# Gancheekim/ATM-VFI

Measured on AMD Instinct MI355X. Metric: interpolated frames/s at 1080p (network_base, bs=1), higher is better.
Workload: dtype f32 (contractions as fp16 hi/lo split x3 MFMA, fp32 accumulate; ~22 significand bits)

## Files before the change

atm-vfi_amd/csrc/api.hip:

```cpp
#include "common.h"

#include <string.h>

#include <vector>

namespace atmvfi {

static thread_local char g_err[512] = "";

void set_error(const char* fmt, ...) {
    va_list ap;
    va_start(ap, fmt);
    vsnprintf(g_err, sizeof(g_err), fmt, ap);
    va_end(ap);
}

int check_launch(const char* what) {
    const hipError_t e = hipGetLastError();
    if (e != hipSuccess) {
        set_error("%s: launch failed: %s", what, hipGetErrorString(e));
        return ATMVFI_ELAUNCH;
    }
    return ATMVFI_OK;
}

#ifdef ATMVFI_RANGE_CHECK
static std::vector<RangeWordSetter>& range_registry() {
    static std::vector<RangeWordSetter> v;
    return v;
}
void range_registry_add(RangeWordSetter s) { range_registry().push_back(s); }
#endif

}

extern "C" int atmvfi_range_word_set(uint32_t* word, void* stream) {
#ifdef ATMVFI_RANGE_CHECK
    for (atmvfi::RangeWordSetter set : atmvfi::range_registry()) {
        const int e = set(reinterpret_cast<unsigned*>(word), (hipStream_t)stream);
        ATMVFI_REQUIRE(e == 0, ATMVFI_ELAUNCH, "range_word_set: hipMemcpyToSymbolAsync failed (%d)", e);
    }
    return ATMVFI_OK;
#else
    (void)word; (void)stream;
    atmvfi::set_error("range_word_set: this is the default build; the operand range check lives in libatmvfi_hip_checked.so (make checked)");
    return ATMVFI_EINVAL;
#endif
}
extern "C" int atmvfi_range_checked(void) {
#ifdef ATMVFI_RANGE_CHECK
    return 1;
#else
    return 0;
#endif
}

extern "C" int atmvfi_version(void) { return (0 << 16) | (26 << 8) | 0; }
extern "C" const char* atmvfi_last_error(void) { return atmvfi::g_err; }
#ifndef ATMVFI_SOURCE_DIGEST
#define ATMVFI_SOURCE_DIGEST "unknown (api.hip compiled outside the Makefile)"
#endif
extern "C" const char* atmvfi_source_digest(void) { return ATMVFI_SOURCE_DIGEST; }
```

atm-vfi_amd/csrc/conv3x3_f16x3.hip:

```cpp
#include "common.h"

#include "conv3_common.h"

#include <stdlib.h>

namespace {

__global__ void pack_split_kernel(int mode, const float* __restrict__ src, _Float16* __restrict__ hi, _Float16* __restrict__ lo,
                                  int Cout, int Cin, int kh, int kw, int rows, int cin_pad, int coutp) {
    fp16_saturate_on();
    const int taps = (mode == ATMVFI_GEMM_DECONV) ? 1 : kh * kw;
    const int cpt = cin_pad >> 5;
    const long long total = (long long)rows * taps * cin_pad;
    for (long long idx = (long long)blockIdx.x * blockDim.x + threadIdx.x; idx < total;
         idx += (long long)gridDim.x * blockDim.x) {
        const int e = (int)(idx & 31);
        const int row = (int)((idx >> 5) % rows);
        const int kstep = (int)((idx >> 5) / rows);
        const int tap = kstep / cpt;
        const int c = (kstep - tap * cpt) * 32 + e;
        float v = 0.f;
        if (c < Cin) {
            if (mode == ATMVFI_GEMM_DECONV) {
                const int q = row / coutp;
                const int co = row - q * coutp;
                if (q < 4 && co < Cout) v = src[(((long long)c * Cout + co) * 2 + (q >> 1)) * 2 + (q & 1)];
            } else if (row < Cout) {
                const int ky = tap / kw, kx = tap - ky * kw;
                v = src[(((long long)row * Cin + c) * kh + ky) * kw + kx];
            }
        }
        const _Float16 h = sat_half(v);
        hi[idx] = h;
        lo[idx] = sat_half((v - (float)h) * LO_SCALE);
    }
}

__global__ void pack_conv3x3_kernel(const float* __restrict__ src, _Float16* __restrict__ hi, _Float16* __restrict__ lo, int Cout, int Cin,
                                    int rows, int cf, int tail) {
    fp16_saturate_on();
    const int nsteps = 9 * (cf >> 5) + (tail ? 3 : 0);
    const long long total = (long long)nsteps * rows * 32;
    for (long long idx = (long long)blockIdx.x * blockDim.x + threadIdx.x; idx < total; idx += (long long)gridDim.x * blockDim.x) {
        const int e = (int)(idx & 31);
        const int row = (int)((idx >> 5) % rows);
        const int step = (int)((idx >> 5) / rows);
        int tap, c;
        if (step < 9 * (cf >> 5)) {
            tap = step % 9;
            c = (step / 9) * 32 + e;
        } else {
            const int t = step - 9 * (cf >> 5);
            tap = 4 * t + (e >> 3);
            c = (e & 7) < tail ? cf + (e & 7) : Cin;
        }
        float v = 0.f;
        if (row < Cout && tap < 9 && c < Cin) v = src[((long long)row * Cin + c) * 9 + tap];
        const _Float16 h = sat_half(v);
        hi[idx] = h;
        lo[idx] = sat_half((v - (float)h) * LO_SCALE);
    }
}

}

static void conv3_layout(int Cin, int& cf, int& tail) {
    const int t = Cin % 32;
    if (t >= 1 && t <= 8) { cf = Cin - t; tail = t; }
    else { cf = atmvfi::round_up(Cin, 32); tail = 0; }
}
static int split_rows(int mode, int Cout) {
    return (mode == ATMVFI_GEMM_DECONV) ? atmvfi::round_up(4 * atmvfi::round_up(Cout, 4), 16) : atmvfi::round_up(Cout, 16);
}

extern "C" int64_t atmvfi_split_weight_halves(int mode, int Cout, int Cin, int kh, int kw) {
    const int taps = (mode == ATMVFI_GEMM_DECONV) ? 1 : kh * kw;
    return (int64_t)split_rows(mode, Cout) * taps * atmvfi::round_up(Cin, 32);
}

extern "C" int atmvfi_pack_weight_split(int mode, const float* src, void* dst_hi, void* dst_lo, int Cout, int Cin, int kh,
                                         int kw, void* stream) {
    ATMVFI_REQUIRE(src && dst_hi && dst_lo && Cout > 0 && Cin > 0 && kh > 0 && kw > 0 && mode >= 0 && mode <= 2, ATMVFI_EINVAL,
                   "pack_weight_split: bad arguments");
    if (mode == ATMVFI_GEMM_DECONV) ATMVFI_REQUIRE(kh == 2 && kw == 2, ATMVFI_EINVAL, "pack_weight_split: deconv must be 2x2");
    const int64_t total = atmvfi_split_weight_halves(mode, Cout, Cin, kh, kw);
    const int blocks = (int)((total + 255) / 256 > 4096 ? 4096 : (total + 255) / 256);
    hipLaunchKernelGGL(pack_split_kernel, dim3(blocks), dim3(256), 0, (hipStream_t)stream, mode, src, (_Float16*)dst_hi,
                       (_Float16*)dst_lo, Cout, Cin, kh, kw, split_rows(mode, Cout), atmvfi::round_up(Cin, 32),
                       atmvfi::round_up(Cout, 4));
    return atmvfi::check_launch("pack_weight_split");
}

extern "C" int atmvfi_conv3x3_f16x3(const float* in, int in_ld, int N, int H, int W, int Cin, const void* w_hi,
                                     const void* w_lo, int Cout, float* out, int out_ld, const float* bias,
                                     const float* prelu, void* out_hi, void* out_lo, int64_t plane_rows,
                                     const float* plane_prelu, int schedule, int wn, void* stream) {
    ATMVFI_REQUIRE(in && w_hi && w_lo && out, ATMVFI_EINVAL, "conv3x3_f16x3: null pointer");
    ATMVFI_REQUIRE(schedule >= -1 && schedule <= 1 && wn >= 0 && wn <= 8, ATMVFI_EINVAL,
                   "conv3x3_f16x3: schedule -1 (auto), 0 (row) or 1 (half), wn 0 (auto) or 1..8; got %d, %d", schedule, wn);
    ATMVFI_REQUIRE(N > 0 && H > 0 && W > 0 && Cin > 0 && Cout > 0, ATMVFI_EINVAL, "conv3x3_f16x3: bad shape");
    ATMVFI_REQUIRE(in_ld % 4 == 0 && in_ld >= atmvfi::round_up(Cin, 4) && out_ld % 4 == 0 && out_ld >= atmvfi::round_up(Cout, 4),
                   ATMVFI_EALIGN, "conv3x3_f16x3: leading dimensions must be multiples of 4 and cover the channels");
    ATMVFI_REQUIRE(atmvfi::aligned16(in) && atmvfi::aligned16(out) && atmvfi::aligned16(w_hi) && atmvfi::aligned16(w_lo) &&
                       (!bias || atmvfi::aligned16(bias)) && (!prelu || atmvfi::aligned16(prelu)),
                   ATMVFI_EALIGN, "conv3x3_f16x3: pointers (incl. bias/prelu) must be 16-byte aligned");
    ATMVFI_REQUIRE((out_hi == nullptr) == (out_lo == nullptr), ATMVFI_EINVAL, "conv3x3_f16x3: plane sink needs both planes");
    if (out_hi) {
        ATMVFI_REQUIRE(plane_rows >= (int64_t)N * H * W, ATMVFI_EINVAL, "conv3x3_f16x3: plane_rows %lld < N*H*W", (long long)plane_rows);
        ATMVFI_REQUIRE(atmvfi::aligned16(out_hi) && atmvfi::aligned16(out_lo) && (!plane_prelu || atmvfi::aligned16(plane_prelu)),
                       ATMVFI_EALIGN, "conv3x3_f16x3: plane sink pointers must be 16-byte aligned");
    }
    Conv3Dev d;
    d.in = in; d.in_ld = in_ld; d.N = N; d.H = H; d.W = W; d.Cin = Cin;
    d.w_hi = (const _Float16*)w_hi; d.w_lo = (const _Float16*)w_lo;
    d.wrows = atmvfi::round_up(Cout, 16);
    conv3_layout(Cin, d.cf, d.tail);
    d.cs = 0;
    d.ktot = 0;
    d.Cout = Cout; d.out = out; d.out_ld = out_ld; d.bias = bias; d.prelu = prelu;
    d.out_hi = (_Float16*)out_hi; d.out_lo = (_Float16*)out_lo; d.plane_rows = plane_rows; d.plane_prelu = plane_prelu;
    d.stamp = nullptr;
    d.nblocks = 0;
    d.tchunk = 0;
    d.legacy_order = 0;
    d.force_schedule = schedule;
// ... 24 lines not shown
```

atm-vfi_amd/csrc/gemm_common.h:

```cpp
#pragma once
#include "common.h"

namespace atmvfi {

struct GemmDev {
    int mode;
    const float* in;
    int in_ld, H, W, Cin;
    long long in_gstride;
    int in_rpg;
    const float* weight;
    int wrows;
    int ktot;
    int cin_pad;
    int cpt;
    int nchunks;
    int Cout;
    int coutp;
    int kw, stride, pad, dil;
    int Ho, Wo;
    long long M;
    float* out;
    int out_ld;
    long long out_gstride;
// ... 3 lines not shown
    const float* prelu;
    const float* in_prelu;
    const float* residual;
    int res_ld;
    const _Float16* w_hi;
    const _Float16* w_lo;
    int cin_pad32;
    int cpt32;
    int nchunks32;
    int ktot32;
    const _Float16* a_hi;
    const _Float16* a_lo;
    const _Float16* a_hi2;
    const _Float16* a_lo2;
    int in_ld2, split_chunks;
    int in_N;
    unsigned long long* stamp;
    int dbg;
    int mchunk;
    int vblocks;
    int nblocks;
    _Float16* out_hi;
    _Float16* out_lo;
    long long out_plane_rows;
    int out_c0, out_gc;
    int force_wn;
    int ksplit;
    float* part;
    long long part_stride;
    int part_ld;
    int fit32;
    int pfit32;
    int terms;
};


__device__ __forceinline__ bool gemm_out_row(const GemmDev& a, long long m, float*& orow, const float*& rrow, long long& prow, int& pc0) {
    pc0 = a.out_c0;
    if (a.mode == ATMVFI_GEMM_DECONV) {
        const int hw = a.H * a.W;
        const int n = (m >> 31) ? (int)(m / hw) : (int)((unsigned)m / (unsigned)hw);
        const int rem = (int)(m - (long long)n * hw);
        const int y = rem / a.W;
        const int x = rem - y * a.W;
        prow = ((long long)n * a.Ho + 2 * y) * a.Wo + 2 * x;
        orow = a.out + prow * a.out_ld;
    } else {
        long long ro = m;
        if (a.out_row_map) ro = a.out_row_map[m];
        if (ro < 0) return false;
        prow = ro;
        long long off = ro * (long long)a.out_ld;
        if (a.out_rpg > 0) {
            const long long grp = ro / a.out_rpg;
            prow = ro - grp * a.out_rpg;
            off = grp * a.out_gstride + prow * (long long)a.out_ld;
            pc0 += (int)grp * a.out_gc;
        }
        orow = a.out + off;
    }
    rrow = a.residual ? a.residual + m * (long long)a.res_ld : nullptr;
    return true;
}
__device__ __forceinline__ void gemm_out_row_at(const GemmDev& a, long long m, long long ro, float*& orow, long long& prow, int& pc0) {
    pc0 = a.out_c0;
    if (a.mode == ATMVFI_GEMM_DECONV) {
        const int hw = a.H * a.W;
// ... 44 lines not shown
    if (c.nvalid >= 4) {
        if (a.bias) c.b = *reinterpret_cast<const f32x4*>(a.bias + c.co);
        if (a.prelu) c.p = *reinterpret_cast<const f32x4*>(a.prelu + c.co);
    } else if (c.nvalid > 0) {
        float bb[4] = {0.f, 0.f, 0.f, 0.f}, pp[4] = {1.f, 1.f, 1.f, 1.f};
        for (int e = 0; e < c.nvalid; ++e) {
            if (a.bias) bb[e] = a.bias[c.co + e];
            if (a.prelu) pp[e] = a.prelu[c.co + e];
        }
        c.b = (f32x4){bb[0], bb[1], bb[2], bb[3]};
        c.p = (f32x4){pp[0], pp[1], pp[2], pp[3]};
    }
    return c;
}

__device__ __forceinline__ void gemm_store4(const GemmDev& a, float* orow, const float* rrow, const ChanVec& c, f32x4 v) {
    if (c.co < 0) return;
    float* optr = orow;
    if (a.mode == ATMVFI_GEMM_DECONV) optr = orow + ((long long)(c.q >> 1) * a.Wo + (c.q & 1)) * a.out_ld;
    v += c.b;
    v.x = v.x > 0.f ? v.x : c.p.x * v.x;
    v.y = v.y > 0.f ? v.y : c.p.y * v.y;
    v.z = v.z > 0.f ? v.z : c.p.z * v.z;
    v.w = v.w > 0.f ? v.w : c.p.w * v.w;
    if (c.nvalid >= 4) {
        if (rrow) v += *reinterpret_cast<const f32x4*>(rrow + c.co);
        *reinterpret_cast<f32x4*>(optr + c.co) = v;
    } else {
        const float vv[4] = {v.x, v.y, v.z, v.w};
        for (int e = 0; e < c.nvalid; ++e) optr[c.co + e] = vv[e] + (rrow ? rrow[c.co + e] : 0.f);
    }
}

template <int BN>
__device__ __forceinline__ void gemm_dma_consts(const GemmDev& a, int n0, float* cst, int wave, int lane) {
    dma_epilogue_consts<BN>(a.bias, a.prelu, n0, cst, wave, lane, [&](int col) {
        int co = col;
        if (a.mode == ATMVFI_GEMM_DECONV) {
            const int q = col / a.coutp;
            co = q < 4 ? col - q * a.coutp : a.Cout;
        }
        return co < a.Cout ? co : -1;
    });
}
constexpr int gemm_const_floats(int BN) { return epilogue_const_floats(BN); }

struct ChanPos {
    int co;
    int q;
    int nvalid;
};
__device__ __forceinline__ ChanPos gemm_chan_pos(const GemmDev& a, int nb) {
    ChanPos c;
    c.q = 0;
    c.co = nb;
    if (a.mode == ATMVFI_GEMM_DECONV) {
        c.q = (nb >= a.coutp) + (nb >= 2 * a.coutp) + (nb >= 3 * a.coutp);
        c.co = nb - c.q * a.coutp;
        if (nb >= 4 * a.coutp) c.co = a.Cout;
    }
    c.nvalid = a.Cout - c.co;
    return c;
}
__device__ __forceinline__ void gemm_finish_store4(const GemmDev& a, float* orow, long long prow, int pc0, const ChanPos& c, f32x4 v,
                                                   const f32x4 b, const f32x4 p, const f32x4 res) {
    v += b;
    v.x = v.x > 0.f ? v.x : p.x * v.x;
    v.y = v.y > 0.f ? v.y : p.y * v.y;
    v.z = v.z > 0.f ? v.z : p.z * v.z;
    v.w = v.w > 0.f ? v.w : p.w * v.w;
    v += res;
// ... 1 lines not shown
        float* optr = orow;
        if (a.mode == ATMVFI_GEMM_DECONV) optr = orow + ((long long)(c.q >> 1) * a.Wo + (c.q & 1)) * a.out_ld;
        if (c.nvalid >= 4) {
            *reinterpret_cast<f32x4*>(optr + c.co) = v;
        } else if (c.nvalid > 0) {
            optr[c.co] = v.x;
            if (c.nvalid > 1) optr[c.co + 1] = v.y;
            if (c.nvalid > 2) optr[c.co + 2] = v.z;
        }
    }
    if (a.out_hi && c.nvalid > 0) {
        if (c.nvalid < 4) {
            v.y = c.nvalid > 1 ? v.y : 0.f;
            v.z = c.nvalid > 2 ? v.z : 0.f;
            v.w = 0.f;
        }
        if (a.mode == ATMVFI_GEMM_DECONV) prow += (long long)(c.q >> 1) * a.Wo + (c.q & 1);
        const RowSink sink{nullptr, 0, a.out_hi, a.out_lo, a.out_plane_rows};
        sink_store4(sink, prow, pc0 + c.co, v);
    }
}
__device__ __forceinline__ f32x4 gemm_load_residual4(const float* rrow, const ChanPos& c) {
    f32x4 r = (f32x4){0.f, 0.f, 0.f, 0.f};
    if (c.nvalid >= 4) {
        r = *reinterpret_cast<const f32x4*>(rrow + c.co);
    } else if (c.nvalid > 0) {
        r.x = rrow[c.co];
        if (c.nvalid > 1) r.y = rrow[c.co + 1];
        if (c.nvalid > 2) r.z = rrow[c.co + 2];
    }
    return r;
}

int launch_gemm_f16x3(const GemmDev& d, int ngemm, hipStream_t stream);
bool try_launch_conv3x3_small(const GemmDev& d, int kh, int* rc, hipStream_t stream);
int launch_gemm_split(const GemmDev& d, int ngemm, hipStream_t stream);
int launch_gemm_pp(const GemmDev& d, int ngemm, hipStream_t stream);
int launch_gemm_duo(const GemmDev& d, int ngemm, hipStream_t stream);

}
```

atm-vfi_amd/csrc/gemm_conv.hip:

```cpp
#include "common.h"
#include "gemm_common.h"

#include <algorithm>

namespace {

using atmvfi::GemmDev;

__device__ __forceinline__ int swz(int row) { return (0x1320 >> (((row >> 2) & 3) << 2)) & 3; }

template <int WM, int WN>
__global__ __launch_bounds__(256) void gemm_mfma_f32(const GemmDev a) {
    fp16_saturate_on();
    constexpr int BM = 64 * WM;
    constexpr int BN = 16 * WN;
    constexpr int NB = (BN * 4 + 255) / 256;
    __shared__ __attribute__((aligned(16))) float lds[2 * (BM + BN) * 16];
    float* As = lds;
    float* Bs = lds + 2 * BM * 16;

    const int t = threadIdx.x;
    const int lane = t & 63;
    const int wave = t >> 6;
    const int kq = t & 3;
// ... 169 lines not shown

int packed_rows(int mode, int Cout) {
    if (mode == ATMVFI_GEMM_DECONV) return atmvfi::round_up(4 * atmvfi::round_up(Cout, 4), 16);
    return atmvfi::round_up(Cout, 16);
}

template <int WM, int WN>
void launch(const GemmDev& d, int ntiles, hipStream_t s) {
    dim3 grid((unsigned)atmvfi::ceil_div64(d.M, 64 * WM), (unsigned)((ntiles + WN - 1) / WN));
    hipLaunchKernelGGL((gemm_mfma_f32<WM, WN>), grid, dim3(256), 0, s, d);
}

}

extern "C" int64_t atmvfi_packed_weight_floats(int mode, int Cout, int Cin, int kh, int kw) {
    const int taps = (mode == ATMVFI_GEMM_DECONV) ? 1 : kh * kw;
    return (int64_t)packed_rows(mode, Cout) * taps * atmvfi::round_up(Cin, 16);
}

extern "C" int atmvfi_pack_weight(int mode, const float* src, float* dst, int Cout, int Cin, int kh, int kw, void* stream) {
    ATMVFI_REQUIRE(src && dst, ATMVFI_EINVAL, "pack_weight: null pointer");
    ATMVFI_REQUIRE(mode >= 0 && mode <= 2 && Cout > 0 && Cin > 0, ATMVFI_EINVAL, "pack_weight: bad mode/shape");
    if (mode == ATMVFI_GEMM_DECONV) ATMVFI_REQUIRE(kh == 2 && kw == 2, ATMVFI_EINVAL, "pack_weight: deconv must be 2x2");
    if (mode == ATMVFI_GEMM_LINEAR) ATMVFI_REQUIRE(kh == 1 && kw == 1, ATMVFI_EINVAL, "pack_weight: linear must be 1x1");
    const int rows = packed_rows(mode, Cout);
    const int cin_pad = atmvfi::round_up(Cin, 16);
    const int64_t total = atmvfi_packed_weight_floats(mode, Cout, Cin, kh, kw);
    const int blocks = (int)std::min<int64_t>((total + 255) / 256, 4096);
    hipLaunchKernelGGL(pack_weight_kernel, dim3(blocks), dim3(256), 0, (hipStream_t)stream, mode, src, dst, Cout, Cin,
                       kh, kw, rows, cin_pad, atmvfi::round_up(Cout, 4));
    return atmvfi::check_launch("pack_weight");
}

extern "C" int atmvfi_gemm(const atmvfi_gemm_params* p, void* stream) {
    ATMVFI_REQUIRE(p, ATMVFI_EINVAL, "gemm: null params");
    const bool planes = p->in_hi || p->in_lo;
    const bool sink = p->out_hi || p->out_lo;
    ATMVFI_REQUIRE((p->in || planes) && p->weight && (p->out || sink), ATMVFI_EINVAL, "gemm: null tensor pointer");
    if (sink) {
        ATMVFI_REQUIRE(p->out_hi && p->out_lo && (p->precision == ATMVFI_PREC_F16X3 || p->precision == ATMVFI_PREC_F16), ATMVFI_EINVAL,
                       "gemm: the plane sink needs both planes and precision f16x3 (or f16)");
        ATMVFI_REQUIRE(atmvfi::aligned16(p->out_hi) && atmvfi::aligned16(p->out_lo) && p->out_plane_c0 >= 0 && p->out_plane_c0 % 4 == 0 &&
                           p->out_plane_gc % 4 == 0, ATMVFI_EALIGN, "gemm: plane sink: 16-byte aligned planes, channel offsets multiples of 4");
        const long long orows = p->mode == ATMVFI_GEMM_DECONV ? (long long)p->N * p->Ho * p->Wo
                                : p->out_rpg > 0 ? (long long)p->out_rpg : (p->mode == ATMVFI_GEMM_CONV ? (long long)p->N * p->Ho * p->Wo : (long long)p->M);
        ATMVFI_REQUIRE(p->out_row_map || p->out_plane_rows >= orows, ATMVFI_EINVAL, "gemm: plane sink rows %lld < output rows %lld",
                       (long long)p->out_plane_rows, orows);
        ATMVFI_REQUIRE(p->out_plane_rows > 0, ATMVFI_EINVAL, "gemm: plane sink needs out_plane_rows");
    }
    if (planes) {
        ATMVFI_REQUIRE(p->in_hi && p->in_lo && (p->precision == ATMVFI_PREC_F16X3 || p->precision == ATMVFI_PREC_F16) && !p->in_prelu,
                       ATMVFI_EINVAL, "gemm: split-plane input needs both planes, precision f16x3 (or f16) and no in_prelu");
        ATMVFI_REQUIRE(atmvfi::aligned16(p->in_hi) && atmvfi::aligned16(p->in_lo) && p->in_rpg == 0, ATMVFI_EALIGN,
                       "gemm: split planes need 16-byte aligned pointers and plain rows");
        const long long mrows = p->mode == ATMVFI_GEMM_LINEAR ? (long long)p->M : (long long)p->N * p->H * p->W;
        ATMVFI_REQUIRE(p->in_ld >= mrows + (p->mode == ATMVFI_GEMM_CONV ? 1 : 0), ATMVFI_EALIGN,
                       "gemm: with split planes in_ld is the plane row count and must cover the rows (+ the zero row in CONV mode): %lld > %d",
                       mrows, p->in_ld);
        if (p->in_hi2 || p->in_lo2) {
            ATMVFI_REQUIRE(p->mode == ATMVFI_GEMM_CONV && p->in_hi2 && p->in_lo2 && atmvfi::aligned16(p->in_hi2) && atmvfi::aligned16(p->in_lo2) &&
                               p->in_ld2 >= mrows + 1 && p->in_split_chunks > 0 && p->in_split_chunks * 32 < p->Cin, ATMVFI_EINVAL,
                           "gemm: a second plane source needs CONV mode, both planes, in_ld2 > N*H*W and 0 < 32 * in_split_chunks < Cin");
        }
    }
    ATMVFI_REQUIRE(p->precision >= ATMVFI_PREC_F32 && p->precision <= ATMVFI_PREC_F16, ATMVFI_EINVAL, "gemm: bad precision %d", p->precision);
    ATMVFI_REQUIRE(p->precision != ATMVFI_PREC_F16 || planes, ATMVFI_EINVAL,
                   "gemm: precision f16 needs split-plane input (in_hi / in_lo): the fp32-input engines have no single-pass instance");
    ATMVFI_REQUIRE(p->precision != ATMVFI_PREC_F16 || p->tile_wn != -1, ATMVFI_EINVAL,
                   "gemm: precision f16 has no instance of the reference schedule (tile_wn = -1): use 0 (auto), -2, -3 or -4");
    ATMVFI_REQUIRE(p->mode >= 0 && p->mode <= 2, ATMVFI_EINVAL, "gemm: bad mode %d", p->mode);
    ATMVFI_REQUIRE(p->Cin > 0 && p->Cout > 0, ATMVFI_EINVAL, "gemm: bad channel counts");
    ATMVFI_REQUIRE(planes || (p->in_ld >= atmvfi::round_up(p->Cin, 4) && p->in_ld % 4 == 0), ATMVFI_EALIGN,
                   "gemm: in_ld %d must be a multiple of 4 and >= Cin rounded to 4 (Cin %d)", p->in_ld, p->Cin);
    ATMVFI_REQUIRE(!p->out || (p->out_ld % 4 == 0 && p->out_ld >= atmvfi::round_up(p->Cout, 4)), ATMVFI_EALIGN,
                   "gemm: out_ld %d must be a multiple of 4 and >= Cout rounded to 4 (Cout %d)", p->out_ld, p->Cout);
    ATMVFI_REQUIRE((planes || atmvfi::aligned16(p->in)) && (!p->out || atmvfi::aligned16(p->out)) && atmvfi::aligned16(p->weight), ATMVFI_EALIGN,
                   "gemm: in/out/weight must be 16-byte aligned");
    ATMVFI_REQUIRE((planes || p->in_gstride % 4 == 0) && p->out_gstride % 4 == 0, ATMVFI_EALIGN, "gemm: group strides must be multiples of 4");
    if (p->residual)
        ATMVFI_REQUIRE(p->res_ld >= p->Cout, ATMVFI_EINVAL, "gemm: res_ld %d < Cout %d", p->res_ld, p->Cout);
    if (p->in_prelu) ATMVFI_REQUIRE(atmvfi::aligned16(p->in_prelu), ATMVFI_EALIGN, "gemm: in_prelu must be 16-byte aligned");
    ATMVFI_REQUIRE((!p->bias || atmvfi::aligned16(p->bias)) && (!p->prelu || atmvfi::aligned16(p->prelu)) &&
                       (!p->residual || (atmvfi::aligned16(p->residual) && p->res_ld % 4 == 0)),
                   ATMVFI_EALIGN, "gemm: bias/prelu/residual must be 16-byte aligned (res_ld a multiple of 4)");

    GemmDev d;
    d.mode = p->mode;
    d.in = p->in; d.in_ld = p->in_ld; d.H = p->H; d.W = p->W; d.Cin = p->Cin;
    d.in_gstride = p->in_gstride; d.in_rpg = p->in_rpg;
    d.weight = p->weight;
    d.cin_pad = atmvfi::round_up(p->Cin, 16);
    d.cpt = d.cin_pad / 16;
    d.Cout = p->Cout; d.coutp = atmvfi::round_up(p->Cout, 4);
    d.kw = 1; d.stride = 1; d.pad = 0; d.dil = 1; d.Ho = p->Ho; d.Wo = p->Wo;
    int taps = 1;
    int ngemm = p->Cout;
    if (p->mode == ATMVFI_GEMM_CONV) {
        ATMVFI_REQUIRE(p->N > 0 && p->H > 0 && p->W > 0, ATMVFI_EINVAL, "conv2d: bad input size");
        ATMVFI_REQUIRE((p->kh == 1 || p->kh == 3) && p->kh == p->kw, ATMVFI_EINVAL, "conv2d: kernel %dx%d unsupported", p->kh, p->kw);
        ATMVFI_REQUIRE(p->stride >= 1 && p->dil >= 1 && p->pad >= 0, ATMVFI_EINVAL, "conv2d: bad stride/dilation/pad");
        const int ho = (p->H + 2 * p->pad - p->dil * (p->kh - 1) - 1) / p->stride + 1;
        const int wo = (p->W + 2 * p->pad - p->dil * (p->kw - 1) - 1) / p->stride + 1;
        ATMVFI_REQUIRE(ho == p->Ho && wo == p->Wo, ATMVFI_EINVAL, "conv2d: Ho/Wo (%d,%d) do not match geometry (%d,%d)", p->Ho, p->Wo, ho, wo);
// ... 19 lines not shown
    d.out = p->out; d.out_ld = p->out_ld; d.out_gstride = p->out_gstride; d.out_rpg = p->out_rpg;
    d.out_row_map = p->out_row_map;
    d.bias = p->bias; d.prelu = p->prelu; d.in_prelu = p->in_prelu; d.residual = p->residual; d.res_ld = p->res_ld;
    ATMVFI_REQUIRE(d.M < (1ll << 40), ATMVFI_EINVAL, "gemm: M too large");
    d.a_hi = (const _Float16*)p->in_hi;
    d.a_lo = (const _Float16*)p->in_lo;
    d.a_hi2 = (const _Float16*)p->in_hi2;
    d.a_lo2 = (const _Float16*)p->in_lo2;
    d.in_ld2 = p->in_ld2;
    d.split_chunks = p->in_hi2 ? p->in_split_chunks : (1 << 30);
    d.in_N = p->N;
    d.out_hi = (_Float16*)p->out_hi;
    d.out_lo = (_Float16*)p->out_lo;
    d.out_plane_rows = p->out_plane_rows;
    d.out_c0 = p->out_plane_c0;
    d.out_gc = p->out_plane_gc;
    ATMVFI_REQUIRE(p->tile_wn >= -4 && p->tile_wn <= 8 && (p->tile_wn >= 0 || planes), ATMVFI_EINVAL,
                   "gemm: tile_wn 0 (auto), 1..8, or (split-plane input) -1 reference schedule / -2 gemm_duo (128-column tiles) / -3 gemm_pp / -4 gemm_duo (64-column tiles), got %d", p->tile_wn);
    d.force_wn = p->tile_wn;
    ATMVFI_REQUIRE(!p->workspace || (atmvfi::aligned16(p->workspace) && p->workspace_floats > 0), ATMVFI_EALIGN,
                   "gemm: the split-K workspace must be 16-byte aligned and non-empty");
    d.ksplit = 0;
    d.part = p->workspace;
    d.part_stride = p->workspace ? p->workspace_floats : 0;
    d.part_ld = 0;
    d.fit32 = 0;
    d.pfit32 = 0;
    d.nblocks = 0;
    d.dbg = 0;
    d.vblocks = 0;
    d.mchunk = 0;
    d.stamp = nullptr;
    d.terms = p->precision == ATMVFI_PREC_F16 ? 1 : 3;
    d.w_hi = (const _Float16*)p->weight_hi;
    d.w_lo = (const _Float16*)p->weight_lo;
    d.cin_pad32 = atmvfi::round_up(p->Cin, 32);
    d.cpt32 = d.cin_pad32 / 32;
    d.nchunks32 = taps * d.cpt32;
    d.ktot32 = taps * d.cin_pad32;
    if (p->precision == ATMVFI_PREC_F16X3 || p->precision == ATMVFI_PREC_F16) {
        ATMVFI_REQUIRE(p->weight_hi && p->weight_lo, ATMVFI_EINVAL, "gemm: precision f16x3 / f16 needs weight_hi/weight_lo");
        ATMVFI_REQUIRE(atmvfi::aligned16(p->weight_hi) && atmvfi::aligned16(p->weight_lo), ATMVFI_EALIGN,
                       "gemm: split weights must be 16-byte aligned");
        if (planes) return atmvfi::launch_gemm_split(d, ngemm, (hipStream_t)stream);
        return atmvfi::launch_gemm_f16x3(d, ngemm, (hipStream_t)stream);
    }

    {
        int rc = 0;
        if (atmvfi::try_launch_conv3x3_small(d, p->kh, &rc, (hipStream_t)stream)) return rc;
    }
    const int ntiles = (ngemm + 15) / 16;
    int best = 1;
    float best_cost = 1e30f;
    for (int wn = 1; wn <= 8; ++wn) {
        const int padded = (ntiles + wn - 1) / wn * wn;
        const float cost = (float)padded * (1.0f + 1.0f / (float)wn);
        if (cost <= best_cost) { best_cost = cost; best = wn; }
    }
    hipStream_t s = (hipStream_t)stream;
    switch (best) {
        case 1: launch<2, 1>(d, ntiles, s); break;
        case 2: launch<2, 2>(d, ntiles, s); break;
        case 3: launch<2, 3>(d, ntiles, s); break;
        case 4: launch<2, 4>(d, ntiles, s); break;
        case 5: launch<2, 5>(d, ntiles, s); break;
        case 6: launch<2, 6>(d, ntiles, s); break;
        case 7: launch<2, 7>(d, ntiles, s); break;
        default: launch<2, 8>(d, ntiles, s); break;
    }
    return atmvfi::check_launch("gemm");
}

extern "C" int atmvfi_conv2d(const atmvfi_gemm_params* p, void* stream) {
    ATMVFI_REQUIRE(p && p->mode == ATMVFI_GEMM_CONV, ATMVFI_EINVAL, "conv2d: params->mode must be ATMVFI_GEMM_CONV");
    return atmvfi_gemm(p, stream);
}
extern "C" int atmvfi_linear(const atmvfi_gemm_params* p, void* stream) {
    ATMVFI_REQUIRE(p && p->mode == ATMVFI_GEMM_LINEAR, ATMVFI_EINVAL, "linear: params->mode must be ATMVFI_GEMM_LINEAR");
    return atmvfi_gemm(p, stream);
}
extern "C" int atmvfi_deconv2x2(const atmvfi_gemm_params* p, void* stream) {
    ATMVFI_REQUIRE(p && p->mode == ATMVFI_GEMM_DECONV, ATMVFI_EINVAL, "deconv2x2: params->mode must be ATMVFI_GEMM_DECONV");
    return atmvfi_gemm(p, stream);
}
```

atm-vfi_amd/csrc/gemm_duo.hip:

```cpp
#include "gemm_plane.h"

namespace {

using atmvfi::GemmDev;

constexpr int BM = 128;
constexpr int stage_bytes(int BN) { return (2 * BM + 2 * BN) * 64; }
constexpr int A_LO = BM * 64, W_HI = 2 * BM * 64;
constexpr int cst_floats(int BN) { return atmvfi::gemm_const_floats(BN) + BM; }

#ifdef ATMVFI_STAMP
static unsigned long long* g_duo_stamp = nullptr;
extern "C" void atmvfi_debug_set_duo_stamp_buffer(void* p) { g_duo_stamp = (unsigned long long*)p; }
#define DUO_SUB(k) do { if (a.stamp) { __builtin_amdgcn_sched_barrier(0); const unsigned long long t_ = __builtin_amdgcn_s_memtime(); sub[k] += t_ - sub_t; sub_t = t_; __builtin_amdgcn_sched_barrier(0); } } while (0)
#else
#define DUO_SUB(k) do { } while (0)
#endif

template <bool CONVM, int BN, bool X3>
__global__ __launch_bounds__(256, 2) void gemm_duo_kernel(const GemmDev a) {
    constexpr int STAGE = stage_bytes(BN), W_LO = W_HI + BN * 64;
    constexpr int MI = BN == 128 ? 4 : 2;
    constexpr int NWN = BN / 64;
    constexpr int WROWS = 16 * MI;
// ... 247 lines not shown
        const f32x4 res = rrow ? atmvfi::gemm_load_residual4(rrow, cp) : (f32x4){0.f, 0.f, 0.f, 0.f};
        atmvfi::gemm_finish_store4(a, orow, prow, pc0, cp, v, vec4(a.bias, 0.f), vec4(a.prelu, 1.f), res);
    }
}

}

template <bool CONVM, int BN, bool X3>
static int launch_duo(const GemmDev& d, int ngemm, hipStream_t s) {
    const size_t lds = (size_t)2 * stage_bytes(BN) + cst_floats(BN) * sizeof(float);
    const hipError_t attr_err = atmvfi::allow_dynamic_lds<gemm_duo_kernel<CONVM, BN, X3>>(lds);
    ATMVFI_REQUIRE(attr_err == hipSuccess, ATMVFI_ELAUNCH, "gemm_duo: hipFuncSetAttribute: %s", hipGetErrorString(attr_err));
    GemmDev dd = d;
    const int prc = atmvfi::plane_gemm_prepare("gemm_duo", dd, ngemm, BM, BN);
    if (prc != ATMVFI_OK) return prc;
#ifdef ATMVFI_STAMP
    dd.stamp = g_duo_stamp;
#endif
    if (dd.ksplit > 1) {
        hipLaunchKernelGGL((gemm_duo_kernel<CONVM, BN, X3>), dim3((unsigned)dd.vblocks, (unsigned)dd.ksplit), dim3(256), lds, s, dd);
        const int rc = atmvfi::check_launch("gemm_duo (split-K)");
        if (rc != ATMVFI_OK) return rc;
        const int ngemm4 = (ngemm + 3) / 4;
        const long long groups = d.M * ngemm4;
        hipLaunchKernelGGL(gemm_splitk_reduce_kernel, dim3((unsigned)std::min<long long>((groups + 255) / 256, 8192)), dim3(256), 0, s, dd, ngemm4);
        return atmvfi::check_launch("gemm_duo (split-K reduce)");
    }
    hipLaunchKernelGGL((gemm_duo_kernel<CONVM, BN, X3>), dim3((unsigned)dd.vblocks), dim3(256), lds, s, dd);
    return atmvfi::check_launch("gemm_duo");
}

int atmvfi::launch_gemm_duo(const GemmDev& d, int ngemm, hipStream_t s) {
    const bool conv = d.mode == ATMVFI_GEMM_CONV;
    if ((ngemm <= 64 && d.force_wn != -2) || d.force_wn == -4) {
        if (d.terms == 1) return conv ? launch_duo<true, 64, false>(d, ngemm, s) : launch_duo<false, 64, false>(d, ngemm, s);
        return conv ? launch_duo<true, 64, true>(d, ngemm, s) : launch_duo<false, 64, true>(d, ngemm, s);
    }
    if (d.terms == 1) return conv ? launch_duo<true, 128, false>(d, ngemm, s) : launch_duo<false, 128, false>(d, ngemm, s);
    return conv ? launch_duo<true, 128, true>(d, ngemm, s) : launch_duo<false, 128, true>(d, ngemm, s);
}
```

atm-vfi_amd/csrc/gemm_plane.h:

```cpp
#pragma once
#include "common.h"
#include "gemm_common.h"

typedef _Float16 f16x8 __attribute__((ext_vector_type(8)));

constexpr float LO_UNSCALE = 1.0f / 1024.0f;

__device__ __forceinline__ int swz64(int row) { return ((row >> 2) & 1) << 1; }
__device__ __forceinline__ void dma16(const unsigned char* src, unsigned char* lds_wave_base) {
    __builtin_amdgcn_global_load_lds((const __attribute__((address_space(1))) void*)src,
                                     (__attribute__((address_space(3))) void*)lds_wave_base, 16, 0, 0);
}
__device__ __forceinline__ void lds_write16f(unsigned addr, const f32x4& v) {
    asm volatile("ds_write_b128 %0, %1" ::"v"(addr), "v"(v) : "memory");
}
template <int OFF>
__device__ __forceinline__ void lds_read16f(f32x4& d, unsigned addr) {
    asm volatile("ds_read_b128 %0, %1 offset:%2" : "=v"(d) : "v"(addr), "n"(OFF) : "memory");
}
template <int N>
__device__ __forceinline__ void wait_vm() { asm volatile("s_waitcnt vmcnt(%0)" ::"n"(N) : "memory"); }

namespace atmvfi {

// ... 268 lines not shown
#pragma unroll
            for (int i = 0; i < MI; ++i)
#pragma unroll
                for (int q = 0; q < 4; ++q) {
                    f32x4 v = finish(i, q);
                    v.y = cp.nvalid > 1 ? v.y : 0.f;
                    v.z = cp.nvalid > 2 ? v.z : 0.f;
                    v.w = cp.nvalid > 3 ? v.w : 0.f;
                    const long long prow = ((long long)dn * a.Ho + 2 * dy) * a.Wo + 2 * dx + qoff;
                    if (ro[i][q] >= 0 && cp.nvalid > 0) sink_store4(sink, prow, pc, v);
                    dx += 4;
                    const bool wrap = dx >= a.W;
                    dx = wrap ? dx - a.W : dx;
                    dy = wrap ? dy + 1 : dy;
                    const bool wrap2 = dy >= a.H;
                    dy = wrap2 ? 0 : dy;
                    dn = wrap2 ? dn + 1 : dn;
                }
        }
    };
    const bool c4 = (a.Cout & 3) == 0;
    const bool fast = (a.mode != ATMVFI_GEMM_DECONV && c4 && (a.out_hi || (a.out && a.out_rpg == 0))) ||
                      (a.mode == ATMVFI_GEMM_DECONV && !a.out && a.out_hi && a.W >= 4 && !a.residual);
    if (fast) {
        if (a.prelu) fast_rows(std::true_type{});
        else fast_rows(std::false_type{});
    } else if (a.residual && !vec_res) {
        store_rows(std::true_type{});
    } else {
        store_rows(std::false_type{});
    }
}

inline int plane_gemm_prepare(const char* engine, GemmDev& d, int ngemm, int BM, int BN) {
    ATMVFI_REQUIRE((long long)d.in_ld * 64 < (1ll << 32) && (long long)d.wrows * 64 < (1ll << 32) &&
                       (!d.a_hi2 || (long long)d.in_ld2 * 64 < (1ll << 32)) && d.M < (1ll << 26), ATMVFI_EINVAL,
                   "%s: plane rows x 64 bytes must fit 32 bits (got %d rows)", engine, d.in_ld);
    if (d.mode == ATMVFI_GEMM_CONV)
        ATMVFI_REQUIRE(d.H < 32768 && d.W < 32768, ATMVFI_EINVAL, "%s: CONV mode packs (y, x) into 16 bits each", engine);
    d.dbg = 0;
    d.pfit32 = d.out_hi && (long long)d.out_plane_rows * 64 < (1ll << 32);
    d.fit32 = d.out && !d.out_row_map && d.out_rpg == 0 && d.mode != ATMVFI_GEMM_DECONV && (d.M + 1) * (long long)d.out_ld * 4 < (1ll << 32) &&
               (!d.residual || (d.M + 1) * (long long)d.res_ld * 4 < (1ll << 32));
    d.nblocks = (ngemm + BN - 1) / BN;
    const long long mgroups = (ceil_div64(d.M, BM) + 7) / 8;
    ATMVFI_REQUIRE(mgroups * 8 * d.nblocks < (1LL << 31), ATMVFI_EINVAL, "%s: grid too large", engine);
    d.vblocks = (int)(mgroups * 8 * d.nblocks);
    return ATMVFI_OK;
}

}
```

atm-vfi_amd/csrc/gemm_pp.hip:

```cpp
#include "gemm_plane.h"

#ifdef ATMVFI_STAMP
static unsigned long long* g_pp_stamp = nullptr;
extern "C" void atmvfi_debug_set_pp_stamp_buffer(void* p) { g_pp_stamp = (unsigned long long*)p; }
#define PP_KSTAMP_BEGIN() unsigned long long kt0_ = 0; do { if (a.stamp) { __builtin_amdgcn_sched_barrier(0); kt0_ = __builtin_amdgcn_s_memtime(); __builtin_amdgcn_sched_barrier(0); } } while (0)
#define PP_KSTAMP_END(idx) do { if (a.stamp) { __builtin_amdgcn_sched_barrier(0); const unsigned long long t_ = __builtin_amdgcn_s_memtime(); if (lane == 0) atomicAdd(&kst[wave * 16 + ((idx) < 15 ? (idx) : 15)], t_ - kt0_); __builtin_amdgcn_sched_barrier(0); } } while (0)
#define PP_STAMP(i) do { if (a.stamp) { tstamp[i] = __builtin_amdgcn_s_memtime(); rstamp[i] = __builtin_amdgcn_s_memrealtime(); } } while (0)
#define PP_SUB(k) do { if (a.stamp) { __builtin_amdgcn_sched_barrier(0); const unsigned long long t_ = __builtin_amdgcn_s_memtime(); sub[k] += t_ - sub_t; sub_t = t_; __builtin_amdgcn_sched_barrier(0); } } while (0)
#else
#define PP_STAMP(i) do { } while (0)
#define PP_SUB(k) do { } while (0)
#define PP_KSTAMP_BEGIN() do { } while (0)
#define PP_KSTAMP_END(idx) do { } while (0)
#endif

namespace {

using atmvfi::GemmDev;

constexpr int BM = 256, BN = 128;
constexpr int STAGE = (2 * BM + 2 * BN) * 64;
constexpr int A_LO = BM * 64, W_HI = 2 * BM * 64, W_LO = W_HI + BN * 64;
constexpr int PIECES = 6;
constexpr int CST_FLOATS = atmvfi::gemm_const_floats(BN) + BM;
// ... 45 lines not shown
            else aoff[i] = (unsigned)m * 64u + ls16;
        }
        int n = tn0 + wave * 16 + (lane >> 2);
        if (n >= a.wrows) n = a.wrows - 1;
        wsoff = (unsigned)n * 64u + ls16;
        pa_hi = reinterpret_cast<const unsigned char*>(a.a_hi);
        pa_lo = reinterpret_cast<const unsigned char*>(a.a_lo);
        pw_hi = reinterpret_cast<const unsigned char*>(a.w_hi);
        pw_lo = reinterpret_cast<const unsigned char*>(a.w_lo);
        cv.ky = cv.kx = cv.chunk = 0;
    };
    setup_issue(m0, n0);
    const long long a_step = (long long)a.in_ld * 64, w_step = (long long)a.wrows * 64;
    int wr_off = 0;
    auto issue_stage = [&]() {
        unsigned char* dst = smem + wr_off + wave * 1024;
        if constexpr (CONVM) {
            atmvfi::plane_conv_issue<A_LO, 8 * 1024>(a, cv, pa_hi, pa_lo, a_step, zero_row, ls16, dst);
        } else {
            dma16(pa_hi + aoff[0], dst);
            dma16(pa_hi + aoff[1], dst + 8 * 1024);
            dma16(pa_lo + aoff[0], dst + A_LO);
            dma16(pa_lo + aoff[1], dst + A_LO + 8 * 1024);
            pa_hi += a_step;
            pa_lo += a_step;
        }
        dma16(pw_hi + wsoff, dst + W_HI);
        dma16(pw_lo + wsoff, dst + W_LO);
        pw_hi += w_step;
        pw_lo += w_step;
        wr_off = wr_off == 2 * STAGE ? 0 : wr_off + STAGE;
    };
    auto dma_tile_consts = [&](int tm0, int tn0, float* dst) {
        atmvfi::gemm_dma_consts<BN>(a, tn0, dst, wave, lane);
        if (a.out_row_map && a.mode == ATMVFI_GEMM_LINEAR) {
            int m = tm0 + (wave & 3) * 64 + lane;
            if (m >= M) m = M - 1;
            __builtin_amdgcn_global_load_lds((const __attribute__((address_space(1))) void*)(a.out_row_map + m),
                                             (__attribute__((address_space(3))) void*)(dst + atmvfi::gemm_const_floats(BN) + (wave & 3) * 64), 4, 0, 0);
        } else {
            atmvfi::gemm_dma_consts<BN>(a, tn0, dst, wave, lane);
        }
    };

    f32x4 acc[4][4];
    RegsIf<X3, f32x4[4][4]> cor;

#ifdef ATMVFI_STAMP
    unsigned long long* kst = reinterpret_cast<unsigned long long*>(smem + 3 * STAGE + 2 * CST_FLOATS * sizeof(float));
    if (tid < 128) kst[tid] = 0;
    __syncthreads();
    unsigned long long tstamp[4], rstamp[4];
    unsigned long long t_loop = 0, t_epi = 0, r_loop = 0, r_epi = 0, t_pro = 0, r_pro = 0;
    int ntile = 0;
    unsigned long long sub[3] = {0, 0, 0}, sub_t = 0;
#endif
    PP_STAMP(0);
    const int nk = a.nchunks32;
    dma_tile_consts(m0, n0, cst_base);
    issue_stage();
    if (nk > 1) {
        issue_stage();
        wait_vm<PIECES>();
    } else {
        wait_vm<0>();
    }
    __builtin_amdgcn_s_barrier();
    if (grp == 1) __builtin_amdgcn_s_barrier();

    f16x8 xh[4], wh[4];
    RegsIf<X3, f16x8[4]> xl, wl;
    const unsigned xfrag = lds_offset(smem) + (unsigned)((64 * wm + r) * 64 + ((g ^ swz64(r)) << 4));
    const unsigned wfrag = lds_offset(smem) + (unsigned)(W_HI + (64 * wn + r) * 64 + ((g ^ swz64(r)) << 4));
    int rd_off = 0;
// ... 98 lines not shown
            bool g1wait = seq == 0;
            for (int kc = 0; kc + 2 < nk; ++kc) {
                PP_KSTAMP_BEGIN();
                kstep(std::integral_constant<int, 0>{}, g1wait);
                PP_KSTAMP_END(kc);
                g1wait = true;
            }
            if (nk >= 2) {
                PP_KSTAMP_BEGIN();
                kstep(std::integral_constant<int, 1>{}, g1wait);
                PP_KSTAMP_END(nk - 2);
                g1wait = true;
            }
            {
                PP_KSTAMP_BEGIN();
                kstep(std::integral_constant<int, 2>{}, g1wait);
                PP_KSTAMP_END(nk - 1);
            }
        }
        PP_STAMP(2);
#ifdef ATMVFI_STAMP
        sub_t = __builtin_amdgcn_s_memtime();
#endif
        if (grp == 0) __builtin_amdgcn_s_barrier();
        if (grp == 1 && has_next) wait_vm<0>();

#pragma unroll
        for (int i = 0; i < 4; ++i)
#pragma unroll
            for (int j = 0; j < 4; ++j) {
                if constexpr (X3) acc[i][j] = acc[i][j] + cor[i][j] * LO_UNSCALE;
                asm volatile("" : "+v"(acc[i][j]));
            }
        {
            const unsigned xb = (unsigned)(rd_off == 0 ? 2 * STAGE : rd_off - STAGE);
            const unsigned tb = lds_offset(smem) + xb + (unsigned)(wave * 1024);
            const unsigned wbase = tb + (unsigned)((r >> 2) * 8192 + (r & 3) * 256 + ((g ^ (r & 3)) << 4));
            const unsigned rq6 = (unsigned)((r >> 2) << 6);
            const unsigned rbase = tb + (unsigned)(g * 256);
            const unsigned rg4 = (unsigned)((r ^ g) << 4);
            unsigned wad[4], rad[4];
#pragma unroll
            for (int k = 0; k < 4; ++k) {
                wad[k] = wbase + (rq6 ^ (unsigned)(k << 6));
                rad[k] = rbase + (rg4 ^ (unsigned)(k << 6));
            }
            static_for<0, 4>([&](auto ic) {
                constexpr int i = decltype(ic)::value;
                static_for<0, 4>([&](auto jc) {
                    constexpr int j = decltype(jc)::value;
                    lds_write16f(wad[j], acc[i][j]);
                });
                static_for<0, 4>([&](auto qc) {
                    constexpr int q = decltype(qc)::value;
                    lds_read16f<q * 8192>(acc[i][q], rad[q]);
                });
            });
            asm volatile("s_waitcnt lgkmcnt(0)" ::: "memory");
#pragma unroll
            for (int i = 0; i < 4; ++i)
#pragma unroll
                for (int q = 0; q < 4; ++q) asm volatile("" : "+v"(acc[i][q]));
        }
        PP_SUB(0);
        atmvfi::plane_gemm_epilogue<CONVM, 4, BM, BN>(a, acc, cst, m0, n0, M, wm, wn, r, g, [&] { PP_SUB(1); });
        PP_SUB(2);
        PP_STAMP(3);
#ifdef ATMVFI_STAMP
        if (a.stamp) {
            if (seq == 0) { t_pro = tstamp[1] - tstamp[0]; r_pro = rstamp[1] - rstamp[0]; }
            t_loop += tstamp[2] - tstamp[1]; r_loop += rstamp[2] - rstamp[1];
            t_epi += tstamp[3] - tstamp[2]; r_epi += rstamp[3] - rstamp[2];
            ++ntile;
        }
#endif
        if (!has_next) break;
        if (grp == 1) __builtin_amdgcn_s_barrier();
        vb = nxt;
        m0 = nm0;
        n0 = nn0;
        ++seq;
    }
#ifdef ATMVFI_STAMP
    if (a.stamp && lane == 0) {
        unsigned long long* o = a.stamp + ((long long)blockIdx.x * 8 + wave) * 8;
        o[0] = t_pro; o[1] = t_loop / ntile; o[2] = t_epi / ntile;
        o[3] = (unsigned long long)nk;
        o[4] = r_loop / ntile; o[5] = sub[0] / ntile; o[6] = sub[1] / ntile;
        o[7] = sub[2] / ntile;
    }
    __syncthreads();
    if (a.stamp && tid < 128) a.stamp[(long long)gridDim.x * 64 + (long long)blockIdx.x * 128 + tid] = kst[tid] / (ntile ? ntile : 1);
#endif
}

}

template <bool CONVM, bool X3>
static int launch_pp(const GemmDev& d, int ngemm, hipStream_t s) {
#ifdef ATMVFI_STAMP
    const size_t lds = (size_t)3 * STAGE + 2 * CST_FLOATS * sizeof(float) + 1024;
#else
    const size_t lds = (size_t)3 * STAGE + 2 * CST_FLOATS * sizeof(float);
#endif
    const hipError_t attr_err = atmvfi::allow_dynamic_lds<gemm_pp_kernel<CONVM, X3>>(lds);
    ATMVFI_REQUIRE(attr_err == hipSuccess, ATMVFI_ELAUNCH, "gemm_pp: hipFuncSetAttribute: %s", hipGetErrorString(attr_err));
    GemmDev dd = d;
    const int rc = atmvfi::plane_gemm_prepare("gemm_pp", dd, ngemm, BM, BN);
    if (rc != ATMVFI_OK) return rc;
#ifdef ATMVFI_STAMP
    dd.stamp = g_pp_stamp;
#endif
    const int grid = d.nchunks32 >= 2 ? std::min(dd.vblocks, atmvfi::cu_count()) : dd.vblocks;
    hipLaunchKernelGGL((gemm_pp_kernel<CONVM, X3>), dim3((unsigned)grid), dim3(512), lds, s, dd);
    return atmvfi::check_launch("gemm_pp");
}

int atmvfi::launch_gemm_pp(const GemmDev& d, int ngemm, hipStream_t s) {
    if (d.terms == 1) return d.mode == ATMVFI_GEMM_CONV ? launch_pp<true, false>(d, ngemm, s) : launch_pp<false, false>(d, ngemm, s);
    return d.mode == ATMVFI_GEMM_CONV ? launch_pp<true, true>(d, ngemm, s) : launch_pp<false, true>(d, ngemm, s);
}
```

atm-vfi_amd/csrc/gemm_split.hip:

```cpp
#include "gemm_plane.h"

#if defined(ATMVFI_REFSCHED) || defined(ATMVFI_STAMP) || defined(ATMVFI_ABLATE)
#define ATMVFI_HAVE_REFSCHED 1
#endif

#ifdef ATMVFI_STAMP
static unsigned long long* g_split_stamp = nullptr;
extern "C" void atmvfi_debug_set_split_stamp_buffer(void* p) { g_split_stamp = (unsigned long long*)p; }
#define SPLIT_STAMP(i) do { if (a.stamp) { tstamp[i] = __builtin_amdgcn_s_memtime(); rstamp[i] = __builtin_amdgcn_s_memrealtime(); } } while (0)
#else
#define SPLIT_STAMP(i) do { } while (0)
#endif

namespace {

using atmvfi::GemmDev;

#ifdef ATMVFI_ABLATE
#define SABL(bit) ((a.dbg & (bit)) != 0)
#else
#define SABL(bit) false
#endif

#ifdef ATMVFI_HAVE_REFSCHED
// ... 340 lines not shown
#endif
#ifdef ATMVFI_STAMP
    dd.stamp = g_split_stamp;
#endif
    dd.nblocks = (ngemm + BN - 1) / BN;
    const long long mgroups = (atmvfi::ceil_div64(d.M, BM) + 7) / 8;
    ATMVFI_REQUIRE(mgroups * 8 * dd.nblocks < (1LL << 31), ATMVFI_EINVAL, "gemm_split: grid too large");
    hipLaunchKernelGGL(kern, dim3((unsigned)(mgroups * 8 * dd.nblocks)), dim3(64 * WGM * WGN), lds, s, dd);
    return atmvfi::check_launch("gemm_split");
}
#endif

}

static int gemm_splitk_plan(long long M, int ngemm, int nk) {
    const long long cus = atmvfi::cu_count();
    const long long tiles = atmvfi::ceil_div64(M, 128) * ((ngemm + 63) / 64);
    if (nk < 16 || tiles * 2 > cus) return 1;
    const int S = (int)std::min<long long>(std::min<long long>(2 * cus / tiles, nk / 8), 8);
    if (S < 2) return 1;
    const double per_step = tiles * S > cus ? 0.75 : 0.6;
    const double traffic_us = 2.0 * S * (double)M * atmvfi::round_up(ngemm, 64) * 4.0 / 3.0e6;
    const double t_unsplit = 6.4 + 0.6 * nk;
    const double t_split = 6.4 + per_step * ((nk + S - 1) / S) + 5.0 + traffic_us;
    return t_split < 0.85 * t_unsplit ? S : 1;
}

extern "C" int64_t atmvfi_gemm_workspace_floats(int64_t M, int ngemm, int ksteps) {
    if (M <= 0 || ngemm <= 0 || ksteps <= 0) return 0;
    const int S = gemm_splitk_plan(M, ngemm, ksteps);
    return S > 1 ? (int64_t)S * M * atmvfi::round_up(ngemm, 64) : 0;
}

int atmvfi::launch_gemm_split(const GemmDev& d, int ngemm, hipStream_t s) {
    if (d.force_wn == -2 || d.force_wn == -4) return launch_gemm_duo(d, ngemm, s);
    if (d.force_wn == -3) return launch_gemm_pp(d, ngemm, s);
    if (d.force_wn == 0 && d.part) {
        const int S = gemm_splitk_plan(d.M, ngemm, d.nchunks32);
        const int ld = round_up(ngemm, 64);
        if (S > 1 && (long long)S * d.M * ld <= d.part_stride) {
            GemmDev ds = d;
            ds.ksplit = S;
            ds.part_ld = ld;
            ds.part_stride = d.M * ld;
            ds.force_wn = -4;
            return launch_gemm_duo(ds, ngemm, s);
        }
    }
    if (d.force_wn == 0) {
        if (ngemm <= 64) return launch_gemm_duo(d, ngemm, s);
        if (ceil_div64(d.M, 128) * ((ngemm + 63) / 64) <= 2 * (long long)cu_count()) {
            GemmDev d64 = d;
            d64.force_wn = -4;
            return launch_gemm_duo(d64, ngemm, s);
        }
        const long long cus = cu_count(), ntile = (ngemm + 127) / 128;
        const long long pp_rounds = ceil_div64(ceil_div64(d.M, 256) * ntile, cus);
        const long long duo_per_cu = ceil_div64(ceil_div64(d.M, 128) * ntile, cus);
        const double duo_rounds = (0.5 * (double)duo_per_cu + ((duo_per_cu & 1) ? 0.1 : 0.0)) * 1.08 * (d.nchunks32 >= 64 ? 1.15 : 1.0);
        return duo_rounds < (double)pp_rounds ? launch_gemm_duo(d, ngemm, s) : launch_gemm_pp(d, ngemm, s);
    }
    if (d.force_wn != -1) return launch_gemm_pp(d, ngemm, s);
#ifdef ATMVFI_HAVE_REFSCHED
    return d.mode == ATMVFI_GEMM_CONV ? launch_split<4, 2, true>(d, ngemm, s) : launch_split<4, 2, false>(d, ngemm, s);
#else
    ATMVFI_REQUIRE(false, ATMVFI_EINVAL, "gemm: tile_wn = -1 (the reference schedule) is not in the product library: load tools/lib/libatmvfi_hip_ref.so (make -C atm-vfi_amd/csrc ref)");
#endif
}

extern "C" int atmvfi_split_planes_at(const float* in, int in_ld, int64_t M, int C, const float* prelu, void* hi, void* lo, int plane_rows,
                                      int c0, int pad_to, void* stream) {
    ATMVFI_REQUIRE(in && hi && lo && M > 0 && C > 0, ATMVFI_EINVAL, "split_planes: bad arguments");
    ATMVFI_REQUIRE(plane_rows >= M && in_ld >= C, ATMVFI_EALIGN, "split_planes: plane rows %d must cover M and in_ld %d must cover C %d", plane_rows, in_ld, C);
    ATMVFI_REQUIRE(atmvfi::aligned16(hi) && atmvfi::aligned16(lo), ATMVFI_EALIGN, "split_planes: planes must be 16-byte aligned");
    ATMVFI_REQUIRE(c0 >= 0 && c0 % 8 == 0 && (pad_to == 8 || pad_to == 32) && (pad_to == 8 || c0 % 32 == 0), ATMVFI_EINVAL,
                   "split_planes: channel offset %d must be a multiple of 8 (of 32 when padding to 32), pad_to 8 or 32", c0);
    const long long n = (long long)M * ((C + pad_to - 1) / pad_to * (pad_to / 8));
    hipLaunchKernelGGL(split_planes_kernel, dim3((unsigned)((n + 255) / 256)), dim3(256), 0, (hipStream_t)stream, in, in_ld, (long long)M, C,
                       prelu, (_Float16*)hi, (_Float16*)lo, (long long)plane_rows, c0, pad_to);
    return atmvfi::check_launch("split_planes");
}
extern "C" int atmvfi_split_planes(const float* in, int in_ld, int64_t M, int C, const float* prelu, void* hi, void* lo, int plane_rows,
                                   void* stream) {
    return atmvfi_split_planes_at(in, in_ld, M, C, prelu, hi, lo, plane_rows, 0, 32, stream);
}

extern "C" int atmvfi_head1x1_planes(const void* in_hi, const void* in_lo, int64_t plane_rows, int64_t rows, int Cin, const float* weight,
                                     const float* bias, int Cout, float* out, int out_ld, void* stream) {
    ATMVFI_REQUIRE(in_hi && in_lo && weight && out, ATMVFI_EINVAL, "head1x1_planes: null pointer");
    ATMVFI_REQUIRE(rows > 0 && plane_rows >= rows && Cin > 0 && Cout >= 1 && Cout <= 8 && out_ld >= Cout, ATMVFI_EINVAL,
                   "head1x1_planes: rows %lld (plane rows %lld), Cin %d, 1 <= Cout %d <= 8 <= ... out_ld %d", (long long)rows,
                   (long long)plane_rows, Cin, Cout, out_ld);
    ATMVFI_REQUIRE(atmvfi::aligned16(in_hi) && atmvfi::aligned16(in_lo), ATMVFI_EALIGN, "head1x1_planes: planes must be 16-byte aligned");
// ... 10 lines not shown
```

atm-vfi_amd/csrc/plan_dispatch.inc:

```
#define ATMVFI_PLAN_NFN 75
static const char* const kPlanFnNames[ATMVFI_PLAN_NFN] = {
    "atmvfi_conv2d",
    "atmvfi_conv3x3_f16x3",
    "atmvfi_conv3x3_planes",
    "atmvfi_conv3x3_planes2",
    "atmvfi_conv3x3_planes3",
    "atmvfi_conv3x3_planes4",
    "atmvfi_conv3x3_planes_readout",
    "atmvfi_conv3x3_planes_readout2",
    "atmvfi_deconv2x2",
    "atmvfi_dwconv3x3_gelu",
    "atmvfi_ensemble_select",
    "atmvfi_f32_to_yuv420p10",
    "atmvfi_final_residual",
    "atmvfi_flow_warp",
    "atmvfi_flow_warp_ex",
    "atmvfi_flow_warp_nhwc",
    "atmvfi_flow_warp_tiled",
    "atmvfi_flow_warp_up2",
    "atmvfi_flow_warp_up2_tiled",
    "atmvfi_frame_borders",
    "atmvfi_frame_compose",
    "atmvfi_frame_difference",
    "atmvfi_frame_f32_to_u8",
    "atmvfi_frame_half",
    "atmvfi_frame_rot180",
    "atmvfi_frame_signature",
    "atmvfi_frame_u8_to_f32",
    "atmvfi_frame_u8_window",
    "atmvfi_gemm",
    "atmvfi_head1x1_planes",
    "atmvfi_image_pyramid",
    "atmvfi_image_pyramid_pack",
    "atmvfi_l1_mean",
    "atmvfi_layernorm",
    "atmvfi_linear",
    "atmvfi_motion_head",
    "atmvfi_motion_head_planes",
    "atmvfi_pack_dw_weight",
    "atmvfi_pack_frames",
    "atmvfi_pack_weight",
    "atmvfi_pack_weight_conv3x3",
    "atmvfi_pack_weight_split",
    "atmvfi_pool_blocks",
    "atmvfi_range_word_set",
    "atmvfi_refine_tail",
    "atmvfi_resize_bilinear_ac",
    "atmvfi_rgb16_decode",
    "atmvfi_rgb16_encode",
    "atmvfi_rgb_to_yuv420",
    "atmvfi_shutter_accumulate",
    "atmvfi_shutter_resolve",
    "atmvfi_split_planes",
    "atmvfi_split_planes_at",
    "atmvfi_ssim_psnr",
    "atmvfi_stem_fused",
    "atmvfi_synth_up2",
    "atmvfi_tta_merge",
    "atmvfi_warp_blend",
    "atmvfi_warp_blend_planes",
    "atmvfi_warp_blend_tiled",
    "atmvfi_window_attention",
    "atmvfi_window_attention_f16x3",
    "atmvfi_window_attn_cross_motion",
    "atmvfi_window_attn_self",
    "atmvfi_yuv420_to_rgb",
    "atmvfi_yuv420_window",
    "atmvfi_yuv420p10_to_f32",
    "atmvfi_yuv_borders",
    "atmvfi_yuv_compose",
    "atmvfi_yuv_pack",
    "atmvfi_yuv_sub_decode",
    "atmvfi_yuv_sub_encode",
    "atmvfi_yuv_surface_decode",
    "atmvfi_yuv_surface_encode",
    "atmvfi_yuv_unpack",
};
static const int kPlanFnArgs[ATMVFI_PLAN_NFN] = {1, 19, 21, 25, 27, 28, 15, 16, 1, 13, 13, 10, 8, 10, 9, 14, 10, 8, 8, 7, 15, 12, 9, 5, 5, 11, 9, 15, 1, 10, 8, 9, 7, 14, 1, 12, 17, 3, 6, 7, 5, 8, 8, 1, 10, 13, 15, 10, 13, 13, 7, 8, 10, 18, 21, 1, 11, 19, 23, 23, 13, 13, 9, 8, 14, 18, 14, 9, 24, 5, 25, 17, 24, 16, 6};
static int plan_call(const atmvfi_plan_op* op, void* stream) {
    const atmvfi_plan_arg* a = op->a;
    switch (op->fn) {
    case 0: return atmvfi_conv2d((const atmvfi_gemm_params*)(uintptr_t)a[0].u, stream);
    case 1: return atmvfi_conv3x3_f16x3((const float*)(uintptr_t)a[0].u, (int)a[1].i, (int)a[2].i, (int)a[3].i, (int)a[4].i, (int)a[5].i, (const void*)(uintptr_t)a[6].u, (const void*)(uintptr_t)a[7].u, (int)a[8].i, (float*)(uintptr_t)a[9].u, (int)a[10].i, (const float*)(uintptr_t)a[11].u, (const float*)(uintptr_t)a[12].u, (void*)(uintptr_t)a[13].u, (void*)(uintptr_t)a[14].u, (int64_t)a[15].i, (const float*)(uintptr_t)a[16].u, (int)a[17].i, (int)a[18].i, stream);
    case 2: return atmvfi_conv3x3_planes((const void*)(uintptr_t)a[0].u, (const void*)(uintptr_t)a[1].u, (int64_t)a[2].i, (int)a[3].i, (int)a[4].i, (int)a[5].i, (int)a[6].i, (const void*)(uintptr_t)a[7].u, (const void*)(uintptr_t)a[8].u, (int)a[9].i, (float*)(uintptr_t)a[10].u, (int)a[11].i, (const float*)(uintptr_t)a[12].u, (const float*)(uintptr_t)a[13].u, (void*)(uintptr_t)a[14].u, (void*)(uintptr_t)a[15].u, (int64_t)a[16].i, (int)a[17].i, (const float*)(uintptr_t)a[18].u, (int)a[19].i, (int)a[20].i, stream);
    case 3: return atmvfi_conv3x3_planes2((const void*)(uintptr_t)a[0].u, (const void*)(uintptr_t)a[1].u, (int64_t)a[2].i, (int)a[3].i, (int)a[4].i, (int)a[5].i, (int)a[6].i, (const void*)(uintptr_t)a[7].u, (const void*)(uintptr_t)a[8].u, (int)a[9].i, (float*)(uintptr_t)a[10].u, (int)a[11].i, (const float*)(uintptr_t)a[12].u, (const float*)(uintptr_t)a[13].u, (void*)(uintptr_t)a[14].u, (void*)(uintptr_t)a[15].u, (int64_t)a[16].i, (int)a[17].i, (const float*)(uintptr_t)a[18].u, (void*)(uintptr_t)a[19].u, (void*)(uintptr_t)a[20].u, (int64_t)a[21].i, (int)a[22].i, (int)a[23].i, (int)a[24].i, stream);
    case 4: return atmvfi_conv3x3_planes3((const void*)(uintptr_t)a[0].u, (const void*)(uintptr_t)a[1].u, (int64_t)a[2].i, (int)a[3].i, (int)a[4].i, (int)a[5].i, (int)a[6].i, (const void*)(uintptr_t)a[7].u, (const void*)(uintptr_t)a[8].u, (int)a[9].i, (float*)(uintptr_t)a[10].u, (int)a[11].i, (const float*)(uintptr_t)a[12].u, (const float*)(uintptr_t)a[13].u, (void*)(uintptr_t)a[14].u, (void*)(uintptr_t)a[15].u, (int64_t)a[16].i, (int)a[17].i, (const float*)(uintptr_t)a[18].u, (void*)(uintptr_t)a[19].u, (void*)(uintptr_t)a[20].u, (int64_t)a[21].i, (int)a[22].i, (int)a[23].i, (int)a[24].i, (float*)(uintptr_t)a[25].u, (int64_t)a[26].i, stream);
    case 5: return atmvfi_conv3x3_planes4((const void*)(uintptr_t)a[0].u, (const void*)(uintptr_t)a[1].u, (int64_t)a[2].i, (int)a[3].i, (int)a[4].i, (int)a[5].i, (int)a[6].i, (const void*)(uintptr_t)a[7].u, (const void*)(uintptr_t)a[8].u, (int)a[9].i, (float*)(uintptr_t)a[10].u, (int)a[11].i, (const float*)(uintptr_t)a[12].u, (const float*)(uintptr_t)a[13].u, (void*)(uintptr_t)a[14].u, (void*)(uintptr_t)a[15].u, (int64_t)a[16].i, (int)a[17].i, (const float*)(uintptr_t)a[18].u, (void*)(uintptr_t)a[19].u, (void*)(uintptr_t)a[20].u, (int64_t)a[21].i, (int)a[22].i, (int)a[23].i, (int)a[24].i, (float*)(uintptr_t)a[25].u, (int64_t)a[26].i, (int)a[27].i, stream);
    case 6: return atmvfi_conv3x3_planes_readout((const void*)(uintptr_t)a[0].u, (const void*)(uintptr_t)a[1].u, (int64_t)a[2].i, (int)a[3].i, (int)a[4].i, (int)a[5].i, (int)a[6].i, (const void*)(uintptr_t)a[7].u, (const void*)(uintptr_t)a[8].u, (int)a[9].i, (const float*)(uintptr_t)a[10].u, (const float*)(uintptr_t)a[11].u, (const void*)(uintptr_t)a[12].u, (float*)(uintptr_t)a[13].u, (int64_t)a[14].i, stream);
    case 7: return atmvfi_conv3x3_planes_readout2((const void*)(uintptr_t)a[0].u, (const void*)(uintptr_t)a[1].u, (int64_t)a[2].i, (int)a[3].i, (int)a[4].i, (int)a[5].i, (int)a[6].i, (const void*)(uintptr_t)a[7].u, (const void*)(uintptr_t)a[8].u, (int)a[9].i, (const float*)(uintptr_t)a[10].u, (const float*)(uintptr_t)a[11].u, (const void*)(uintptr_t)a[12].u, (float*)(uintptr_t)a[13].u, (int64_t)a[14].i, (int)a[15].i, stream);
    case 8: return atmvfi_deconv2x2((const atmvfi_gemm_params*)(uintptr_t)a[0].u, stream);
    case 9: return atmvfi_dwconv3x3_gelu((const float*)(uintptr_t)a[0].u, (int)a[1].i, (float*)(uintptr_t)a[2].u, (int)a[3].i, (const float*)(uintptr_t)a[4].u, (const float*)(uintptr_t)a[5].u, (int)a[6].i, (int)a[7].i, (int)a[8].i, (int)a[9].i, (void*)(uintptr_t)a[10].u, (void*)(uintptr_t)a[11].u, (int)a[12].i, stream);
    case 10: return atmvfi_ensemble_select((const float*)(uintptr_t)a[0].u, (const float*)(uintptr_t)a[1].u, (const float*)(uintptr_t)a[2].u, (const float*)(uintptr_t)a[3].u, (const float*)(uintptr_t)a[4].u, (const float*)(uintptr_t)a[5].u, (const float*)(uintptr_t)a[6].u, (const float*)(uintptr_t)a[7].u, (const float*)(uintptr_t)a[8].u, (float*)(uintptr_t)a[9].u, (float*)(uintptr_t)a[10].u, (int)a[11].i, (int64_t)a[12].i, stream);
    case 11: return atmvfi_f32_to_yuv420p10((const float*)(uintptr_t)a[0].u, (int)a[1].i, (int)a[2].i, (int)a[3].i, (int)a[4].i, (int)a[5].i, (int)a[6].i, (int)a[7].i, (int)a[8].i, (void*)(uintptr_t)a[9].u, stream);
    case 12: return atmvfi_final_residual((const float*)(uintptr_t)a[0].u, (const float*)(uintptr_t)a[1].u, (int)a[2].i, (float*)(uintptr_t)a[3].u, (float*)(uintptr_t)a[4].u, (int)a[5].i, (int)a[6].i, (int)a[7].i, stream);
    case 13: return atmvfi_flow_warp((const float*)(uintptr_t)a[0].u, (const float*)(uintptr_t)a[1].u, (int64_t)a[2].i, (int)a[3].i, (int)a[4].i, (float*)(uintptr_t)a[5].u, (int)a[6].i, (int)a[7].i, (int)a[8].i, (int)a[9].i, stream);
    case 14: return atmvfi_flow_warp_ex((const float*)(uintptr_t)a[0].u, (const float*)(uintptr_t)a[1].u, (float*)(uintptr_t)a[2].u, (uint8_t*)(uintptr_t)a[3].u, (int)a[4].i, (int)a[5].i, (int)a[6].i, (int)a[7].i, (int)a[8].i, stream);
    case 15: return atmvfi_flow_warp_nhwc((const float*)(uintptr_t)a[0].u, (int)a[1].i, (int64_t)a[2].i, (const float*)(uintptr_t)a[3].u, (int64_t)a[4].i, (int)a[5].i, (int)a[6].i, (float*)(uintptr_t)a[7].u, (int)a[8].i, (int64_t)a[9].i, (int)a[10].i, (int)a[11].i, (int)a[12].i, (int)a[13].i, stream);
    case 16: return atmvfi_flow_warp_tiled((const float*)(uintptr_t)a[0].u, (const float*)(uintptr_t)a[1].u, (int64_t)a[2].i, (int)a[3].i, (int)a[4].i, (float*)(uintptr_t)a[5].u, (int)a[6].i, (int)a[7].i, (int)a[8].i, (int)a[9].i, stream);
    case 17: return atmvfi_flow_warp_up2((const float*)(uintptr_t)a[0].u, (const float*)(uintptr_t)a[1].u, (float*)(uintptr_t)a[2].u, (float*)(uintptr_t)a[3].u, (int)a[4].i, (int)a[5].i, (int)a[6].i, (int)a[7].i, stream);
    case 18: return atmvfi_flow_warp_up2_tiled((const float*)(uintptr_t)a[0].u, (const float*)(uintptr_t)a[1].u, (float*)(uintptr_t)a[2].u, (float*)(uintptr_t)a[3].u, (int)a[4].i, (int)a[5].i, (int)a[6].i, (int)a[7].i, stream);
    case 19: return atmvfi_frame_borders((const void*)(uintptr_t)a[0].u, (int)a[1].i, (int)a[2].i, (int)a[3].i, (int32_t*)(uintptr_t)a[4].u, (int32_t*)(uintptr_t)a[5].u, (int64_t)a[6].i, stream);
    case 20: return atmvfi_frame_compose((void*)(uintptr_t)a[0].u, (const void*)(uintptr_t)a[1].u, (int)a[2].i, (int)a[3].i, (int)a[4].i, (int)a[5].i, (int)a[6].i, (int)a[7].i, (const float*)(uintptr_t)a[8].u, (int)a[9].i, (int)a[10].i, (int)a[11].i, (int)a[12].i, (const void*)(uintptr_t)a[13].u, (int)a[14].i, stream);
    case 21: return atmvfi_frame_difference((const void*)(uintptr_t)a[0].u, (const void*)(uintptr_t)a[1].u, (int)a[2].i, (int)a[3].i, (int)a[4].i, (int)a[5].i, (int)a[6].i, (int)a[7].i, (int)a[8].i, (int32_t*)(uintptr_t)a[9].u, (int32_t*)(uintptr_t)a[10].u, (int64_t)a[11].i, stream);
    case 22: return atmvfi_frame_f32_to_u8((const float*)(uintptr_t)a[0].u, (int)a[1].i, (int)a[2].i, (int)a[3].i, (int)a[4].i, (void*)(uintptr_t)a[5].u, (int)a[6].i, (int)a[7].i, (int)a[8].i, stream);
    case 23: return atmvfi_frame_half((const float*)(uintptr_t)a[0].u, (float*)(uintptr_t)a[1].u, (int)a[2].i, (int)a[3].i, (int)a[4].i, stream);
    case 24: return atmvfi_frame_rot180((const float*)(uintptr_t)a[0].u, (float*)(uintptr_t)a[1].u, (int)a[2].i, (int)a[3].i, (int)a[4].i, stream);
    case 25: return atmvfi_frame_signature((const void*)(uintptr_t)a[0].u, (int)a[1].i, (int)a[2].i, (int)a[3].i, (int)a[4].i, (int)a[5].i, (int)a[6].i, (int)a[7].i, (int32_t*)(uintptr_t)a[8].u, (int32_t*)(uintptr_t)a[9].u, (int64_t)a[10].i, stream);
    case 26: return atmvfi_frame_u8_to_f32((const void*)(uintptr_t)a[0].u, (int)a[1].i, (int)a[2].i, (int)a[3].i, (float*)(uintptr_t)a[4].u, (int)a[5].i, (int)a[6].i, (int)a[7].i, (int)a[8].i, stream);
    case 27: return atmvfi_frame_u8_window((const void*)(uintptr_t)a[0].u, (int)a[1].i, (int)a[2].i, (int)a[3].i, (int)a[4].i, (int)a[5].i, (int)a[6].i, (int)a[7].i, (int)a[8].i, (float*)(uintptr_t)a[9].u, (int)a[10].i, (int)a[11].i, (int)a[12].i, (int)a[13].i, (void*)(uintptr_t)a[14].u, stream);
    case 28: return atmvfi_gemm((const atmvfi_gemm_params*)(uintptr_t)a[0].u, stream);
    case 29: return atmvfi_head1x1_planes((const void*)(uintptr_t)a[0].u, (const void*)(uintptr_t)a[1].u, (int64_t)a[2].i, (int64_t)a[3].i, (int)a[4].i, (const float*)(uintptr_t)a[5].u, (const float*)(uintptr_t)a[6].u, (int)a[7].i, (float*)(uintptr_t)a[8].u, (int)a[9].i, stream);
    case 30: return atmvfi_image_pyramid((const float*)(uintptr_t)a[0].u, (const float*)(uintptr_t)a[1].u, (float*)(uintptr_t)a[2].u, (float*)(uintptr_t)a[3].u, (float*)(uintptr_t)a[4].u, (int)a[5].i, (int)a[6].i, (int)a[7].i, stream);
    case 31: return atmvfi_image_pyramid_pack((const float*)(uintptr_t)a[0].u, (const float*)(uintptr_t)a[1].u, (float*)(uintptr_t)a[2].u, (float*)(uintptr_t)a[3].u, (float*)(uintptr_t)a[4].u, (float*)(uintptr_t)a[5].u, (int)a[6].i, (int)a[7].i, (int)a[8].i, stream);
    case 32: return atmvfi_l1_mean((const float*)(uintptr_t)a[0].u, (const float*)(uintptr_t)a[1].u, (float*)(uintptr_t)a[2].u, (int)a[3].i, (int64_t)a[4].i, (float*)(uintptr_t)a[5].u, (int64_t)a[6].i, stream);
    case 33: return atmvfi_layernorm((const float*)(uintptr_t)a[0].u, (int)a[1].i, (int64_t)a[2].i, (int)a[3].i, (const int32_t*)(uintptr_t)a[4].u, (float*)(uintptr_t)a[5].u, (int)a[6].i, (const float*)(uintptr_t)a[7].u, (const float*)(uintptr_t)a[8].u, (int64_t)a[9].i, (int)a[10].i, (void*)(uintptr_t)a[11].u, (void*)(uintptr_t)a[12].u, (int)a[13].i, stream);
    case 34: return atmvfi_linear((const atmvfi_gemm_params*)(uintptr_t)a[0].u, stream);
    case 35: return atmvfi_motion_head((const float*)(uintptr_t)a[0].u, (const int32_t*)(uintptr_t)a[1].u, (const float*)(uintptr_t)a[2].u, (const float*)(uintptr_t)a[3].u, (const float*)(uintptr_t)a[4].u, (const float*)(uintptr_t)a[5].u, (float*)(uintptr_t)a[6].u, (int)a[7].i, (int64_t)a[8].i, (int)a[9].i, (int64_t)a[10].i, (int)a[11].i, stream);
    case 36: return atmvfi_motion_head_planes((const float*)(uintptr_t)a[0].u, (const int32_t*)(uintptr_t)a[1].u, (const float*)(uintptr_t)a[2].u, (const float*)(uintptr_t)a[3].u, (const float*)(uintptr_t)a[4].u, (const float*)(uintptr_t)a[5].u, (float*)(uintptr_t)a[6].u, (int)a[7].i, (int64_t)a[8].i, (int)a[9].i, (int64_t)a[10].i, (int)a[11].i, (void*)(uintptr_t)a[12].u, (void*)(uintptr_t)a[13].u, (int64_t)a[14].i, (int)a[15].i, (int)a[16].i, stream);
    case 37: return atmvfi_pack_dw_weight((const float*)(uintptr_t)a[0].u, (float*)(uintptr_t)a[1].u, (int)a[2].i, stream);
    case 38: return atmvfi_pack_frames((const float*)(uintptr_t)a[0].u, (const float*)(uintptr_t)a[1].u, (float*)(uintptr_t)a[2].u, (int)a[3].i, (int)a[4].i, (int)a[5].i, stream);
    case 39: return atmvfi_pack_weight((int)a[0].i, (const float*)(uintptr_t)a[1].u, (float*)(uintptr_t)a[2].u, (int)a[3].i, (int)a[4].i, (int)a[5].i, (int)a[6].i, stream);
    case 40: return atmvfi_pack_weight_conv3x3((const float*)(uintptr_t)a[0].u, (void*)(uintptr_t)a[1].u, (void*)(uintptr_t)a[2].u, (int)a[3].i, (int)a[4].i, stream);
    case 41: return atmvfi_pack_weight_split((int)a[0].i, (const float*)(uintptr_t)a[1].u, (void*)(uintptr_t)a[2].u, (void*)(uintptr_t)a[3].u, (int)a[4].i, (int)a[5].i, (int)a[6].i, (int)a[7].i, stream);
    case 42: return atmvfi_pool_blocks((void*)(uintptr_t)a[0].u, (int64_t)a[1].i, (int)a[2].i, (const int32_t*)(uintptr_t)a[3].u, (int)a[4].i, (int64_t)a[5].i, (void*)(uintptr_t)a[6].u, (int)a[7].i, stream);
    case 43: return atmvfi_range_word_set((uint32_t*)(uintptr_t)a[0].u, stream);
    case 44: return atmvfi_refine_tail((const float*)(uintptr_t)a[0].u, (int64_t)a[1].i, (const float*)(uintptr_t)a[2].u, (const float*)(uintptr_t)a[3].u, (const float*)(uintptr_t)a[4].u, (float*)(uintptr_t)a[5].u, (float*)(uintptr_t)a[6].u, (int)a[7].i, (int)a[8].i, (int)a[9].i, stream);
    case 45: return atmvfi_resize_bilinear_ac((const float*)(uintptr_t)a[0].u, (int64_t)a[1].i, (int64_t)a[2].i, (int64_t)a[3].i, (int64_t)a[4].i, (float*)(uintptr_t)a[5].u, (int)a[6].i, (int)a[7].i, (int)a[8].i, (int)a[9].i, (int)a[10].i, (int)a[11].i, (float)a[12].f, stream);
    case 46: return atmvfi_rgb16_decode((const void*)(uintptr_t)a[0].u, (int)a[1].i, (int)a[2].i, (int)a[3].i, (int)a[4].i, (int)a[5].i, (int)a[6].i, (int)a[7].i, (int)a[8].i, (float*)(uintptr_t)a[9].u, (int)a[10].i, (int)a[11].i, (int)a[12].i, (int)a[13].i, (void*)(uintptr_t)a[14].u, stream);
    case 47: return atmvfi_rgb16_encode((const float*)(uintptr_t)a[0].u, (int)a[1].i, (int)a[2].i, (int)a[3].i, (int)a[4].i, (void*)(uintptr_t)a[5].u, (int)a[6].i, (int)a[7].i, (int)a[8].i, (int)a[9].i, stream);
    case 48: return atmvfi_rgb_to_yuv420((const void*)(uintptr_t)a[0].u, (int)a[1].i, (const float*)(uintptr_t)a[2].u, (int)a[3].i, (int)a[4].i, (int)a[5].i, (int)a[6].i, (int)a[7].i, (int)a[8].i, (int)a[9].i, (int)a[10].i, (int)a[11].i, (void*)(uintptr_t)a[12].u, stream);
    case 49: return atmvfi_shutter_accumulate((int32_t*)(uintptr_t)a[0].u, (int)a[1].i, (int)a[2].i, (const float*)(uintptr_t)a[3].u, (int)a[4].i, (int)a[5].i, (int)a[6].i, (int)a[7].i, (const uint8_t*)(uintptr_t)a[8].u, (int)a[9].i, (int)a[10].i, (int)a[11].i, (int)a[12].i, stream);
    case 50: return atmvfi_shutter_resolve((const int32_t*)(uintptr_t)a[0].u, (int)a[1].i, (int)a[2].i, (int)a[3].i, (int)a[4].i, (uint8_t*)(uintptr_t)a[5].u, (int)a[6].i, stream);
    case 51: return atmvfi_split_planes((const float*)(uintptr_t)a[0].u, (int)a[1].i, (int64_t)a[2].i, (int)a[3].i, (const float*)(uintptr_t)a[4].u, (void*)(uintptr_t)a[5].u, (void*)(uintptr_t)a[6].u, (int)a[7].i, stream);
    case 52: return atmvfi_split_planes_at((const float*)(uintptr_t)a[0].u, (int)a[1].i, (int64_t)a[2].i, (int)a[3].i, (const float*)(uintptr_t)a[4].u, (void*)(uintptr_t)a[5].u, (void*)(uintptr_t)a[6].u, (int)a[7].i, (int)a[8].i, (int)a[9].i, stream);
    case 53: return atmvfi_ssim_psnr((const void*)(uintptr_t)a[0].u, (int64_t)a[1].i, (int64_t)a[2].i, (int64_t)a[3].i, (int64_t)a[4].i, (const float*)(uintptr_t)a[5].u, (int64_t)a[6].i, (int64_t)a[7].i, (int64_t)a[8].i, (int64_t)a[9].i, (int)a[10].i, (int)a[11].i, (int)a[12].i, (float)a[13].f, (int)a[14].i, (double*)(uintptr_t)a[15].u, (float*)(uintptr_t)a[16].u, (int64_t)a[17].i, stream);
    case 54: return atmvfi_stem_fused((const float*)(uintptr_t)a[0].u, (int)a[1].i, (int)a[2].i, (int)a[3].i, (int)a[4].i, (int)a[5].i, (const void*)(uintptr_t)a[6].u, (const void*)(uintptr_t)a[7].u, (const float*)(uintptr_t)a[8].u, (const float*)(uintptr_t)a[9].u, (const void*)(uintptr_t)a[10].u, (const void*)(uintptr_t)a[11].u, (const float*)(uintptr_t)a[12].u, (const float*)(uintptr_t)a[13].u, (const void*)(uintptr_t)a[14].u, (const void*)(uintptr_t)a[15].u, (const float*)(uintptr_t)a[16].u, (const float*)(uintptr_t)a[17].u, (void*)(uintptr_t)a[18].u, (void*)(uintptr_t)a[19].u, (int64_t)a[20].i, stream);
    case 55: return atmvfi_synth_up2((const atmvfi_synth_up2_params*)(uintptr_t)a[0].u, stream);
    case 56: return atmvfi_tta_merge((const float*)(uintptr_t)a[0].u, (const float*)(uintptr_t)a[1].u, (float*)(uintptr_t)a[2].u, (void*)(uintptr_t)a[3].u, (int)a[4].i, (int)a[5].i, (int)a[6].i, (int)a[7].i, (int)a[8].i, (int)a[9].i, (int)a[10].i, stream);
    case 57: return atmvfi_warp_blend((const float*)(uintptr_t)a[0].u, (const float*)(uintptr_t)a[1].u, (const float*)(uintptr_t)a[2].u, (int)a[3].i, (int64_t)a[4].i, (float*)(uintptr_t)a[5].u, (float*)(uintptr_t)a[6].u, (float*)(uintptr_t)a[7].u, (float*)(uintptr_t)a[8].u, (float*)(uintptr_t)a[9].u, (float*)(uintptr_t)a[10].u, (float*)(uintptr_t)a[11].u, (const float*)(uintptr_t)a[12].u, (const float*)(uintptr_t)a[13].u, (float*)(uintptr_t)a[14].u, (int)a[15].i, (int)a[16].i, (int)a[17].i, (int)a[18].i, stream);
    case 58: return atmvfi_warp_blend_planes((const float*)(uintptr_t)a[0].u, (const float*)(uintptr_t)a[1].u, (const float*)(uintptr_t)a[2].u, (int)a[3].i, (int64_t)a[4].i, (float*)(uintptr_t)a[5].u, (float*)(uintptr_t)a[6].u, (float*)(uintptr_t)a[7].u, (float*)(uintptr_t)a[8].u, (float*)(uintptr_t)a[9].u, (float*)(uintptr_t)a[10].u, (float*)(uintptr_t)a[11].u, (const float*)(uintptr_t)a[12].u, (const float*)(uintptr_t)a[13].u, (float*)(uintptr_t)a[14].u, (int)a[15].i, (void*)(uintptr_t)a[16].u, (void*)(uintptr_t)a[17].u, (int64_t)a[18].i, (int)a[19].i, (int)a[20].i, (int)a[21].i, (int)a[22].i, stream);
    case 59: return atmvfi_warp_blend_tiled((const float*)(uintptr_t)a[0].u, (const float*)(uintptr_t)a[1].u, (const float*)(uintptr_t)a[2].u, (int)a[3].i, (int64_t)a[4].i, (float*)(uintptr_t)a[5].u, (float*)(uintptr_t)a[6].u, (float*)(uintptr_t)a[7].u, (float*)(uintptr_t)a[8].u, (float*)(uintptr_t)a[9].u, (float*)(uintptr_t)a[10].u, (float*)(uintptr_t)a[11].u, (const float*)(uintptr_t)a[12].u, (const float*)(uintptr_t)a[13].u, (float*)(uintptr_t)a[14].u, (int)a[15].i, (void*)(uintptr_t)a[16].u, (void*)(uintptr_t)a[17].u, (int64_t)a[18].i, (int)a[19].i, (int)a[20].i, (int)a[21].i, (int)a[22].i, stream);
    case 60: return atmvfi_window_attention((const float*)(uintptr_t)a[0].u, (float*)(uintptr_t)a[1].u, (float*)(uintptr_t)a[2].u, (const int32_t*)(uintptr_t)a[3].u, (int)a[4].i, (int)a[5].i, (int)a[6].i, (int)a[7].i, (int)a[8].i, (int)a[9].i, (void*)(uintptr_t)a[10].u, (void*)(uintptr_t)a[11].u, (int)a[12].i, stream);
    case 61: return atmvfi_window_attention_f16x3((const float*)(uintptr_t)a[0].u, (float*)(uintptr_t)a[1].u, (float*)(uintptr_t)a[2].u, (const int32_t*)(uintptr_t)a[3].u, (int)a[4].i, (int)a[5].i, (int)a[6].i, (int)a[7].i, (int)a[8].i, (int)a[9].i, (void*)(uintptr_t)a[10].u, (void*)(uintptr_t)a[11].u, (int)a[12].i, stream);
    case 62: return atmvfi_window_attn_cross_motion((const float*)(uintptr_t)a[0].u, (float*)(uintptr_t)a[1].u, (float*)(uintptr_t)a[2].u, (const int32_t*)(uintptr_t)a[3].u, (int)a[4].i, (int)a[5].i, (int)a[6].i, (int)a[7].i, (int)a[8].i, stream);
    case 63: return atmvfi_window_attn_self((const float*)(uintptr_t)a[0].u, (float*)(uintptr_t)a[1].u, (const int32_t*)(uintptr_t)a[2].u, (int)a[3].i, (int)a[4].i, (int)a[5].i, (int)a[6].i, (int)a[7].i, stream);
    case 64: return atmvfi_yuv420_to_rgb((const void*)(uintptr_t)a[0].u, (int)a[1].i, (int)a[2].i, (int)a[3].i, (int)a[4].i, (int)a[5].i, (int)a[6].i, (void*)(uintptr_t)a[7].u, (int)a[8].i, (float*)(uintptr_t)a[9].u, (int)a[10].i, (int)a[11].i, (int)a[12].i, (int)a[13].i, stream);
    case 65: return atmvfi_yuv420_window((const void*)(uintptr_t)a[0].u, (int)a[1].i, (int)a[2].i, (int)a[3].i, (int)a[4].i, (int)a[5].i, (int)a[6].i, (int)a[7].i, (int)a[8].i, (int)a[9].i, (int)a[10].i, (int)a[11].i, (float*)(uintptr_t)a[12].u, (int)a[13].i, (int)a[14].i, (int)a[15].i, (int)a[16].i, (void*)(uintptr_t)a[17].u, stream);
    case 66: return atmvfi_yuv420p10_to_f32((const void*)(uintptr_t)a[0].u, (int)a[1].i, (int)a[2].i, (int)a[3].i, (int)a[4].i, (int)a[5].i, (int)a[6].i, (int)a[7].i, (int)a[8].i, (float*)(uintptr_t)a[9].u, (int)a[10].i, (int)a[11].i, (int)a[12].i, (int)a[13].i, stream);
    case 67: return atmvfi_yuv_borders((const void*)(uintptr_t)a[0].u, (int)a[1].i, (int)a[2].i, (int)a[3].i, (int)a[4].i, (int64_t)a[5].i, (int32_t*)(uintptr_t)a[6].u, (int32_t*)(uintptr_t)a[7].u, (int64_t)a[8].i, stream);
    case 68: return atmvfi_yuv_compose((void*)(uintptr_t)a[0].u, (const void*)(uintptr_t)a[1].u, (int)a[2].i, (int)a[3].i, (int)a[4].i, (int)a[5].i, (int)a[6].i, (int)a[7].i, (int)a[8].i, (int)a[9].i, (int)a[10].i, (int64_t)a[11].i, (int64_t)a[12].i, (int64_t)a[13].i, (int)a[14].i, (int)a[15].i, (int)a[16].i, (int)a[17].i, (const float*)(uintptr_t)a[18].u, (int)a[19].i, (int)a[20].i, (int)a[21].i, (int)a[22].i, (const void*)(uintptr_t)a[23].u, stream);
    case 69: return atmvfi_yuv_pack((const void*)(uintptr_t)a[0].u, (int)a[1].i, (int)a[2].i, (int)a[3].i, (void*)(uintptr_t)a[4].u, stream);
    case 70: return atmvfi_yuv_sub_decode((const void*)(uintptr_t)a[0].u, (int)a[1].i, (int)a[2].i, (int)a[3].i, (int)a[4].i, (int)a[5].i, (int)a[6].i, (int)a[7].i, (int)a[8].i, (int)a[9].i, (int64_t)a[10].i, (int64_t)a[11].i, (int64_t)a[12].i, (int)a[13].i, (int)a[14].i, (int)a[15].i, (int)a[16].i, (int)a[17].i, (void*)(uintptr_t)a[18].u, (int)a[19].i, (float*)(uintptr_t)a[20].u, (int)a[21].i, (int)a[22].i, (int)a[23].i, (int)a[24].i, stream);
    case 71: return atmvfi_yuv_sub_encode((const void*)(uintptr_t)a[0].u, (int)a[1].i, (const float*)(uintptr_t)a[2].u, (int)a[3].i, (int)a[4].i, (int)a[5].i, (int)a[6].i, (int)a[7].i, (int)a[8].i, (int)a[9].i, (int)a[10].i, (int)a[11].i, (int)a[12].i, (int)a[13].i, (int)a[14].i, (int)a[15].i, (void*)(uintptr_t)a[16].u, stream);
    case 72: return atmvfi_yuv_surface_decode((const void*)(uintptr_t)a[0].u, (int)a[1].i, (int)a[2].i, (int)a[3].i, (int)a[4].i, (int)a[5].i, (int)a[6].i, (int)a[7].i, (int)a[8].i, (int64_t)a[9].i, (int64_t)a[10].i, (int64_t)a[11].i, (int)a[12].i, (int)a[13].i, (int)a[14].i, (int)a[15].i, (int)a[16].i, (void*)(uintptr_t)a[17].u, (int)a[18].i, (float*)(uintptr_t)a[19].u, (int)a[20].i, (int)a[21].i, (int)a[22].i, (int)a[23].i, stream);
    case 73: return atmvfi_yuv_surface_encode((const void*)(uintptr_t)a[0].u, (int)a[1].i, (const float*)(uintptr_t)a[2].u, (int)a[3].i, (int)a[4].i, (int)a[5].i, (int)a[6].i, (int)a[7].i, (int)a[8].i, (int)a[9].i, (int)a[10].i, (int)a[11].i, (int)a[12].i, (int)a[13].i, (int)a[14].i, (void*)(uintptr_t)a[15].u, stream);
    case 74: return atmvfi_yuv_unpack((const void*)(uintptr_t)a[0].u, (int)a[1].i, (int)a[2].i, (int)a[3].i, (int64_t)a[4].i, (void*)(uintptr_t)a[5].u, stream);
    default: break;
    }
    atmvfi::set_error("plan_run: unknown function id %d", op->fn);
    return ATMVFI_EINVAL;
}
```

atm-vfi_amd/hip_ops.py:

```python
from __future__ import annotations

import ctypes
import os
from dataclasses import dataclass
from typing import List, Optional

import torch

from .pixfmt import DeepRGB, Packed, Surface, _not_420, _origin_error, as_surface

_HERE = os.path.dirname(os.path.abspath(__file__))
LIB_PATH = os.path.join(_HERE, "libatmvfi_hip.so")
CHECKED_LIB_PATH = os.path.join(_HERE, "libatmvfi_hip_checked.so")

GEMM_CONV, GEMM_LINEAR, GEMM_DECONV = 0, 1, 2

c_f = ctypes.c_void_p
c_i = ctypes.c_int
C_SLOTS = ctypes.POINTER(ctypes.c_int32)
c_l = ctypes.c_int64


class HipLibraryMissing(RuntimeError):
    pass


class GemmParams(ctypes.Structure):
    _fields_ = [
        ("mode", ctypes.c_int32),
        ("in_", c_f), ("in_ld", ctypes.c_int32), ("N", ctypes.c_int32), ("H", ctypes.c_int32),
        ("W", ctypes.c_int32), ("Cin", ctypes.c_int32),
        ("in_gstride", ctypes.c_int64), ("in_rpg", ctypes.c_int32),
        ("weight", c_f),
        ("Cout", ctypes.c_int32), ("kh", ctypes.c_int32), ("kw", ctypes.c_int32), ("stride", ctypes.c_int32),
        ("pad", ctypes.c_int32), ("dil", ctypes.c_int32),
        ("Ho", ctypes.c_int32), ("Wo", ctypes.c_int32),
        ("M", ctypes.c_int64),
        ("out", c_f), ("out_ld", ctypes.c_int32),
        ("out_gstride", ctypes.c_int64), ("out_rpg", ctypes.c_int32),
        ("out_row_map", c_f),
        ("bias", c_f), ("prelu", c_f), ("in_prelu", c_f), ("residual", c_f),
        ("res_ld", ctypes.c_int32),
        ("precision", ctypes.c_int32), ("weight_hi", c_f), ("weight_lo", c_f),
        ("in_hi", c_f), ("in_lo", c_f),
        ("out_hi", c_f), ("out_lo", c_f), ("out_plane_rows", ctypes.c_int64), ("out_plane_c0", ctypes.c_int32),
        ("out_plane_gc", ctypes.c_int32), ("tile_wn", ctypes.c_int32),
        ("in_hi2", c_f), ("in_lo2", c_f), ("in_ld2", ctypes.c_int32), ("in_split_chunks", ctypes.c_int32),
        ("workspace", c_f), ("workspace_floats", ctypes.c_int64),
    ]


class PlanArg(ctypes.Union):
    _fields_ = [("u", ctypes.c_uint64), ("i", ctypes.c_int64), ("f", ctypes.c_double)]


PLAN_MAX_ARGS = 28


class PlanOp(ctypes.Structure):
    _fields_ = [("fn", ctypes.c_int32), ("nargs", ctypes.c_int32), ("a", PlanArg * PLAN_MAX_ARGS)]


class PlanPatch(ctypes.Structure):
    _fields_ = [("op", ctypes.c_int32), ("arg", ctypes.c_int32), ("slot", ctypes.c_int32), ("reserved", ctypes.c_int32),
                ("offset", ctypes.c_int64)]


SIGNATURES = {
    "atmvfi_version": (c_i, []),
    "atmvfi_last_error": (ctypes.c_char_p, []),
    "atmvfi_source_digest": (ctypes.c_char_p, []),
    "atmvfi_range_word_set": (c_i, [c_f, c_f]),
    "atmvfi_range_checked": (c_i, []),
    "atmvfi_gemm": (c_i, [ctypes.POINTER(GemmParams), c_f]),
    "atmvfi_gemm_workspace_floats": (c_l, [c_l, c_i, c_i]),
    "atmvfi_split_planes": (c_i, [c_f, c_i, c_l, c_i, c_f, c_f, c_f, c_i, c_f]),
    "atmvfi_split_planes_at": (c_i, [c_f, c_i, c_l, c_i, c_f, c_f, c_f, c_i, c_i, c_i, c_f]),
    "atmvfi_conv2d": (c_i, [ctypes.POINTER(GemmParams), c_f]),
    "atmvfi_linear": (c_i, [ctypes.POINTER(GemmParams), c_f]),
    "atmvfi_deconv2x2": (c_i, [ctypes.POINTER(GemmParams), c_f]),
    "atmvfi_packed_weight_floats": (c_l, [c_i, c_i, c_i, c_i, c_i]),
    "atmvfi_pack_weight": (c_i, [c_i, c_f, c_f, c_i, c_i, c_i, c_i, c_f]),
    "atmvfi_split_weight_halves": (c_l, [c_i, c_i, c_i, c_i, c_i]),
    "atmvfi_pack_weight_split": (c_i, [c_i, c_f, c_f, c_f, c_i, c_i, c_i, c_i, c_f]),
    "atmvfi_conv3x3_weight_halves": (c_l, [c_i, c_i]),
    "atmvfi_pack_weight_conv3x3": (c_i, [c_f, c_f, c_f, c_i, c_i, c_f]),
    "atmvfi_conv3x3_f16x3": (c_i, [c_f, c_i, c_i, c_i, c_i, c_i, c_f, c_f, c_i, c_f, c_i, c_f, c_f, c_f, c_f, c_l, c_f, c_i, c_i, c_f]),
    "atmvfi_conv3x3_planes": (c_i, [c_f, c_f, c_l, c_i, c_i, c_i, c_i, c_f, c_f, c_i, c_f, c_i, c_f, c_f, c_f, c_f, c_l, c_i, c_f, c_i, c_i, c_f]),
    "atmvfi_flow_warp_up2": (c_i, [c_f, c_f, c_f, c_f, c_i, c_i, c_i, c_i, c_f]),
    "atmvfi_flow_warp_up2_tiled": (c_i, [c_f, c_f, c_f, c_f, c_i, c_i, c_i, c_i, c_f]),
    "atmvfi_image_pyramid": (c_i, [c_f, c_f, c_f, c_f, c_f, c_i, c_i, c_i, c_f]),
    "atmvfi_image_pyramid_pack": (c_i, [c_f, c_f, c_f, c_f, c_f, c_f, c_i, c_i, c_i, c_f]),
    "atmvfi_head1x1_planes": (c_i, [c_f, c_f, c_l, c_l, c_i, c_f, c_f, c_i, c_f, c_i, c_f]),
    "atmvfi_conv3x3_planes2": (c_i, [c_f, c_f, c_l, c_i, c_i, c_i, c_i, c_f, c_f, c_i, c_f, c_i, c_f, c_f, c_f, c_f, c_l, c_i, c_f, c_f, c_f, c_l, c_i, c_i, c_i, c_f]),
    "atmvfi_conv3x3_planes3": (c_i, [c_f, c_f, c_l, c_i, c_i, c_i, c_i, c_f, c_f, c_i, c_f, c_i, c_f, c_f, c_f, c_f, c_l, c_i, c_f, c_f, c_f, c_l, c_i, c_i, c_i, c_f, c_l, c_f]),
    "atmvfi_conv3x3_planes_workspace_floats": (c_l, [c_i, c_i, c_i, c_i, c_i]),
    "atmvfi_conv3x3_planes_readout": (c_i, [c_f, c_f, c_l, c_i, c_i, c_i, c_i, c_f, c_f, c_i, c_f, c_f, c_f, c_f, c_l, c_f]),
    "atmvfi_conv3x3_planes4": (c_i, [c_f, c_f, c_l, c_i, c_i, c_i, c_i, c_f, c_f, c_i, c_f, c_i, c_f, c_f, c_f, c_f, c_l, c_i, c_f, c_f, c_f, c_l, c_i, c_i, c_i, c_f, c_l, c_i, c_f]),
    "atmvfi_conv3x3_planes_readout2": (c_i, [c_f, c_f, c_l, c_i, c_i, c_i, c_i, c_f, c_f, c_i, c_f, c_f, c_f, c_f, c_l, c_i, c_f]),
    "atmvfi_refine_tail": (c_i, [c_f, c_l, c_f, c_f, c_f, c_f, c_f, c_i, c_i, c_i, c_f]),
    "atmvfi_layernorm": (c_i, [c_f, c_i, c_l, c_i, c_f, c_f, c_i, c_f, c_f, c_l, c_i, c_f, c_f, c_i, c_f]),
    "atmvfi_dwconv3x3_gelu": (c_i, [c_f, c_i, c_f, c_i, c_f, c_f, c_i, c_i, c_i, c_i, c_f, c_f, c_i, c_f]),
    "atmvfi_pack_dw_weight": (c_i, [c_f, c_f, c_i, c_f]),
    "atmvfi_window_attention": (c_i, [c_f, c_f, c_f, c_f, c_i, c_i, c_i, c_i, c_i, c_i, c_f, c_f, c_i, c_f]),
    "atmvfi_window_attention_f16x3": (c_i, [c_f, c_f, c_f, c_f, c_i, c_i, c_i, c_i, c_i, c_i, c_f, c_f, c_i, c_f]),
    "atmvfi_window_attn_cross_motion": (c_i, [c_f, c_f, c_f, c_f, c_i, c_i, c_i, c_i, c_i, c_f]),
    "atmvfi_window_attn_self": (c_i, [c_f, c_f, c_f, c_i, c_i, c_i, c_i, c_i, c_f]),
    "atmvfi_motion_head": (c_i, [c_f, c_f, c_f, c_f, c_f, c_f, c_f, c_i, c_l, c_i, c_l, c_i, c_f]),
    "atmvfi_motion_head_planes": (c_i, [c_f, c_f, c_f, c_f, c_f, c_f, c_f, c_i, c_l, c_i, c_l, c_i, c_f, c_f, c_l, c_i, c_i, c_f]),
    "atmvfi_flow_warp": (c_i, [c_f, c_f, c_l, c_i, c_i, c_f, c_i, c_i, c_i, c_i, c_f]),
    "atmvfi_flow_warp_tiled": (c_i, [c_f, c_f, c_l, c_i, c_i, c_f, c_i, c_i, c_i, c_i, c_f]),
    "atmvfi_flow_warp_ex": (c_i, [c_f, c_f, c_f, c_f, c_i, c_i, c_i, c_i, c_i, c_f]),
    "atmvfi_flow_warp_nhwc": (c_i, [c_f, c_i, c_l, c_f, c_l, c_i, c_i, c_f, c_i, c_l, c_i, c_i, c_i, c_i, c_f]),
    "atmvfi_warp_blend": (c_i, [c_f, c_f, c_f, c_i, c_l, c_f, c_f, c_f, c_f, c_f, c_f, c_f, c_f, c_f, c_f, c_i,
                                c_i, c_i, c_i, c_f]),
    "atmvfi_warp_blend_planes": (c_i, [c_f, c_f, c_f, c_i, c_l, c_f, c_f, c_f, c_f, c_f, c_f, c_f, c_f, c_f, c_f, c_i,
                                       c_f, c_f, c_l, c_i, c_i, c_i, c_i, c_f]),
# ... 56 lines not shown
    _fields_ = ([(n, ctypes.c_void_p) for n in ("it_sum", "it0", "it1", "flow0", "flow1", "m1", "store0", "store1", "slots0", "slots1", "dst_f32",
                                                 "dst_u8", "f0_out", "f1_out", "m_out", "workspace")]
                + [(n, ctypes.c_int32) for n in ("B", "h", "w", "S0", "S1", "pad_top", "pad_left", "hh", "ww", "bgr", "path", "reserved")])


def load_library(path: str = LIB_PATH, optional=()) -> ctypes.CDLL:
    if not os.path.exists(path):
        raise HipLibraryMissing(
            f"{path} not found: build it with `python -c 'import __graft_entry__ as g; g.build()'` "
            "(hipcc --offload-arch=gfx950).  There is no CPU fallback.")
    lib = ctypes.CDLL(path)
    for name, (res, args) in SIGNATURES.items():
        if name in optional and not hasattr(lib, name):
            continue
        fn = getattr(lib, name)
        fn.restype = res
        fn.argtypes = args
    return lib


@dataclass
class PackedWeight:
    mode: int
    cout: int
    cin: int
    kh: int
    kw: int
    orig: torch.Tensor
    packed: Optional[torch.Tensor]
    hi: Optional[torch.Tensor] = None
    lo: Optional[torch.Tensor] = None
    hi3: Optional[torch.Tensor] = None
    lo3: Optional[torch.Tensor] = None


@dataclass
class StemWeights:
    c0: int
    c1: int
    w1h: torch.Tensor
    w1l: torch.Tensor
    b1: torch.Tensor
    p1: torch.Tensor
    w2h: torch.Tensor
    w2l: torch.Tensor
    b2: torch.Tensor
    p2: torch.Tensor
    w3h: torch.Tensor
    w3l: torch.Tensor
    b3: torch.Tensor
    p3: torch.Tensor


class Planes:

    def __init__(self, t: torch.Tensor, c: int, rows: Optional[int] = None):
        if t.dtype != torch.float16 or t.dim() != 4 or t.shape[0] != 2 or t.shape[3] != 32 or not t.is_contiguous() or c > t.shape[1] * 32 \
                or c <= (t.shape[1] - 1) * 32:
            raise ValueError(f"Planes: expected contiguous fp16 [2, ceil(C/32), rows, 32], got {tuple(t.shape)} {t.dtype} C={c}")
        if not t.is_cuda:
            raise TypeError("Planes: tensor must live on the GPU")
        if rows is not None and not 0 < rows <= t.shape[2]:
            raise ValueError(f"Planes: {rows} valid rows do not fit the {t.shape[2]} allocated ones")
        self.t, self.c = t, c
        self._rows = t.shape[2] if rows is None else rows

# ... 299 lines not shown
            rc = self.lib.atmvfi_plan_run(self.c_ops, len(self.ops_list), self.c_patches, len(self.patches), sl, len(self.slots),
                                          ctypes.byref(self.failed), stream)
        if rc != 0:
            raise RuntimeError(f"plan_run failed ({rc}) at op {self.failed.value}: {self.lib.atmvfi_last_error().decode()}")

        def build(x):
            if isinstance(x, tuple) and len(x) == 2 and x[0] == "slot":
                return outs[x[1] - base]
            if isinstance(x, dict):
                return {kk: build(v) for kk, v in x.items()}
            if isinstance(x, list):
                return [build(v) for v in x]
            return x
        return build(self.template)


class HipOps:

    def __init__(self, device: torch.device, checked: bool = False, lib_path: Optional[str] = None, lib_optional=()):
        self.checked = bool(checked)
        self.lib = load_library(lib_path, lib_optional) if lib_path else load_library(CHECKED_LIB_PATH) if self.checked else load_library()
        self.device = device
        self.range_word: Optional[torch.Tensor] = None
        if self.checked:
            if self.lib.atmvfi_range_checked() != 1:
                raise HipLibraryMissing(f"{CHECKED_LIB_PATH} is not a checked build (make -C atm-vfi_amd/csrc checked)")
            self.range_word = torch.zeros(1, dtype=torch.int32, device=device)
        self.profile: Optional[List] = None
        self.precision = "f16x3"
        self.plane_terms = 3
        self.attention_f16x3 = True
        self.conv3_instance = None
        self.gemm_tile_wn = 0
        self.warp_tiles = True
        self.recording: Optional[LaunchPlan] = None
        self.gemm_workspace = None

    def begin_plan(self, inputs) -> LaunchPlan:
        if self.profile is not None:
            raise PlanUnsupported("per-launch profiling is on")
        self.recording = LaunchPlan(self.lib, inputs)
        return self.recording

    def end_plan(self, result) -> LaunchPlan:
        plan, self.recording = self.recording, None
        return plan.finish(result)

    def abort_plan(self):
        self.recording = None

    def _stream(self):
        return ctypes.c_void_p(torch.cuda.current_stream(self.device).cuda_stream)

    def begin_forward(self):
        if self.checked:
            self._check(self.lib.atmvfi_range_word_set(self.range_word.data_ptr(), self._stream()), "range_word_set")

    def _check(self, rc: int, name: str):
        if rc != 0:
            raise RuntimeError(f"{name} failed ({rc}): {self.lib.atmvfi_last_error().decode()}")

    def _run(self, name: str, meta: dict, fn, *args):
        if self.recording is not None:
            self.recording.add_op(fn, args)
        if self.profile is None:
            self._check(fn(*args), name)
# ... 5 lines not shown
        self._check(fn(*args), name)
        e.record(st)
        self.profile.append((name, meta, s, e))

    def empty(self, *shape) -> torch.Tensor:
        t = torch.empty(*shape, dtype=torch.float32, device=self.device)
        if self.recording is not None:
            self.recording.add_output(t)
        return t

    def to_device_int(self, t: torch.Tensor) -> torch.Tensor:
        return t.to(device=self.device, dtype=torch.int32).contiguous()

    def pack_weight(self, mode: int, w: torch.Tensor) -> PackedWeight:
        _chk(w, "pack_weight")
        w = w.detach().contiguous()
        if mode == GEMM_DECONV:
            cin, cout, kh, kw = w.shape
        elif mode == GEMM_LINEAR:
            cout, cin = w.shape[0], w.shape[1]
            kh = kw = 1
        else:
            cout, cin, kh, kw = w.shape
        n = self.lib.atmvfi_packed_weight_floats(mode, cout, cin, kh, kw)
        dst = self.empty(n)
        self._check(self.lib.atmvfi_pack_weight(mode, _ptr(w), _ptr(dst), cout, cin, kh, kw, self._stream()), "pack_weight")
        pw = PackedWeight(mode, cout, cin, kh, kw, w, dst)
        if cin >= 16:
            nh = self.lib.atmvfi_split_weight_halves(mode, cout, cin, kh, kw)
            pw.hi = torch.empty(nh, dtype=torch.float16, device=self.device)
            pw.lo = torch.empty(nh, dtype=torch.float16, device=self.device)
            self._check(self.lib.atmvfi_pack_weight_split(mode, _ptr(w), _ptr(pw.hi), _ptr(pw.lo), cout, cin, kh, kw, self._stream()),
                        "pack_weight_split")
            if mode == GEMM_CONV and kh == 3 and kw == 3:
                n3 = self.lib.atmvfi_conv3x3_weight_halves(cout, cin)
                pw.hi3 = torch.empty(n3, dtype=torch.float16, device=self.device)
                pw.lo3 = torch.empty(n3, dtype=torch.float16, device=self.device)
                self._check(self.lib.atmvfi_pack_weight_conv3x3(_ptr(w), _ptr(pw.hi3), _ptr(pw.lo3), cout, cin, self._stream()),
                            "pack_weight_conv3x3")
        return pw

    def pack_dw_weight(self, w: torch.Tensor) -> torch.Tensor:
        _chk(w, "pack_dw_weight")
        w = w.detach().contiguous()
        c = w.shape[0]
        dst = self.empty(9 * c)
        self._check(self.lib.atmvfi_pack_dw_weight(_ptr(w), _ptr(dst), c, self._stream()), "pack_dw_weight")
        return dst

    def _plane_prec(self, p: "GemmParams"):
        if self.plane_terms not in (1, 3):
            raise ValueError(f"plane_terms must be 3 (f16x3) or 1 (f16), got {self.plane_terms!r}")
        if self.plane_terms == 1 and p.precision == 1 and p.in_hi:
            p.precision = 2

    def _prec(self, w: PackedWeight):
        if self.precision == "f16x3" and w.hi is not None:
            return 1, w.hi.data_ptr(), w.lo.data_ptr()
        return 0, None, None

    def pad_channels(self, v: torch.Tensor, mult: int = 32) -> torch.Tensor:
        c = v.shape[0]
        out = torch.zeros((c + mult - 1) // mult * mult, dtype=torch.float32, device=self.device)
        out[:c] = v.detach()
        return out

# ... 255 lines not shown
        else:
            ld, n, h, wd, cin = nhwc_view(x, "deconv.in")
        cout = w.cout
        if out is None:
            if sink is None:
                raise ValueError("deconv: no output")
            old, on, oh, ow = 0, n, 2 * h, 2 * wd
        else:
            old, on, oh, ow, oc = nhwc_view(out, "deconv.out")
            if oc != cout:
                raise ValueError(f"deconv: out has {oc} channels, weight {cout}")
        if cin != w.cin or on != n or w.mode != GEMM_DECONV or oh != 2 * h or ow != 2 * wd:
            raise ValueError(f"deconv: shape mismatch in {(n, h, wd, cin)} w ({w.cin},{w.cout}) out {(on, oh, ow, cout)}")
        p = GemmParams(mode=GEMM_DECONV, in_=None if x is None else x.data_ptr(), in_ld=ld, N=n, H=h, W=wd, Cin=cin, in_gstride=0, in_rpg=0,
                       weight=w.packed.data_ptr(), Cout=cout, kh=2, kw=2, stride=2, pad=0, dil=1, Ho=oh, Wo=ow,
                       M=n * h * wd, out=None if out is None else out.data_ptr(), out_ld=old, out_gstride=0, out_rpg=0, out_row_map=None,
                       bias=_ptr(bias), prelu=_ptr(prelu), in_prelu=_ptr(in_prelu), residual=None, res_ld=0)
        p.precision, p.weight_hi, p.weight_lo = self._prec(w)
        p.tile_wn = self.gemm_tile_wn
        self._gemm_sink(p, sink, n * oh * ow, cout, sink_c0, 0, 1, "deconv")
        use_planes = planes is not None and p.precision == 1
        if x is None and not use_planes:
            raise ValueError("deconv: plane input needs the f16x3 engine")
        if use_planes:
            if planes.rows < n * h * wd or planes.c != cin:
                raise ValueError("deconv: planes do not match the input rows")
            p.in_, p.in_ld, p.in_prelu = None, planes.ld_rows, None
            p.in_hi, p.in_lo = planes.t[0].data_ptr(), planes.t[1].data_ptr()
        meta = {"flops": 2.0 * n * h * wd * 4 * cout * cin, "bytes": 4.0 * (n * h * wd * cin + n * oh * ow * cout + 4 * cout * cin),
                "shape": f"M{n * h * wd} N{4 * cout} K{cin}"}
        ws = self._gemm_splitk(p, n * h * wd, 4 * ((cout + 3) // 4 * 4), (cin + 31) // 32) if use_planes else None
        p._srcs = (x, out, bias, prelu, in_prelu, ws)
        self._plane_prec(p)
        self._run("deconv2x2_split" if use_planes else "deconv2x2_f16x3" if p.precision else "deconv2x2", meta, self.lib.atmvfi_deconv2x2,
                  ctypes.byref(p), self._stream())

    split_planes_ok = True
    pyramid_packs = True
    motion_head_sink = True

    def split_planes(self, x, out: Planes, prelu=None, c0: Optional[int] = None):
        ld, m, c, gs, _ = rows_view(x, "split_planes.in")
        if gs != 0 or m != out.rows or (c0 is None and c != out.c) or (c0 is not None and (c0 % 8 or c0 + c > out.chunks * 32)):
            raise ValueError("split_planes: expected a plain [rows,C] view matching the planes")
        if prelu is not None and prelu.numel() < c:
            raise ValueError("split_planes: prelu needs one slope per channel")
        meta = {"bytes": 4.0 * m * c + 4.0 * m * ((c + 31) // 32 * 32 if c0 is None else (c + 7) // 8 * 8)}
        if c0 is None:
            self._run("split_planes", meta, self.lib.atmvfi_split_planes, _ptr(x), ld, m, c, _ptr(prelu), _ptr(out.t[0]),
                      _ptr(out.t[1]), out.ld_rows, self._stream())
        else:
            self._run("split_planes", meta, self.lib.atmvfi_split_planes_at, _ptr(x), ld, m, c, _ptr(prelu), _ptr(out.t[0]),
                      _ptr(out.t[1]), out.ld_rows, c0, 8, self._stream())

    def linear(self, x, w: PackedWeight, out, bias=None, residual=None, out_row_map=None, sink: Optional[Planes] = None,
               sink_c0: int = 0, sink_gc: int = 0):
        planes = x if isinstance(x, Planes) else None
        if planes is not None:
            if self.precision != "f16x3" or w.hi is None:
                raise ValueError("linear: split-plane input needs the f16x3 engine and split weights")
            ld, m, cin, gs, rpg = planes.ld_rows, planes.rows, planes.c, 0, 0
        else:
            ld, m, cin, gs, rpg = rows_view(x, "linear.in")
        old, mo, cout, ogs, orpg = rows_view(out, "linear.out")
        if cin != w.cin or cout != w.cout or w.kh != 1 or w.mode == GEMM_DECONV:
            raise ValueError(f"linear: shape mismatch in {tuple(x.shape)} w ({w.cout},{w.cin}) out {tuple(out.shape)}")
        if out_row_map is None and mo != m:
            raise ValueError("linear: row count mismatch")
        if out_row_map is not None and (out_row_map.numel() != m or out_row_map.dtype != torch.int32 or not out_row_map.is_cuda):
# ... 851 lines not shown
```

atm-vfi_amd/network.py:

```python
from __future__ import annotations

import math
import operator
from typing import Dict, List, Optional, Tuple

import torch
import torch.nn as nn

from . import scaled
from . import schema as S
from .hip_ops import GEMM_CONV, GEMM_DECONV, GEMM_LINEAR, HipOps, PackedWeight, Planes, PlanUnsupported
from .windows import WindowGeometry, build_window_geometry


_VERSION_OF = operator.attrgetter("_version")
_DATA_PTR_OF = torch.Tensor.data_ptr


_PARAM_EPOCH = [0]


class _ParamWatch:

    def __setattr__(self, name, value):
# ... 689 lines not shown
    def enable_frame_cache(self, flag: bool = True):
        self._frame_cache_on = bool(flag)
        self._frame_cache = None

    def f16x3_deviation(self, im0: torch.Tensor, im1: torch.Tensor) -> float:
        keep = "f16x3-checked" if self._checked else self._precision
        try:
            self.set_precision("f32")
            ref = self.forward(im0, im1)["I_t"].clone()
            self.set_precision("f16x3")
            got = self.forward(im0, im1)["I_t"]
            return float((got - ref).abs().max())
        finally:
            self.set_precision(keep)

    def enable_plans(self, flag: bool = True):
        self.use_plans = bool(flag)
        self._plan_stats = self._new_plan_stats()
        if not flag:
            self._drop_plans()

    PLAN_KINDS = ("forward", "pooled_frame", "pooled_pair")

    @classmethod
    def _new_plan_stats(cls) -> Dict[str, Dict[str, int]]:
        return {kind: {"eager": 0, "recorded": 0, "replayed": 0, "refused": 0} for kind in cls.PLAN_KINDS}

    def plan_stats(self) -> Dict[str, Dict[str, int]]:
        return {kind: dict(c) for kind, c in self._plan_stats.items()}

    def _mode_fields(self, ops) -> Tuple:
        return (self.global_motion, self.ensemble_global_motion, self._precision, self._checked, getattr(ops, "attention_f16x3", None),
                self.local_motion_args["window_size"], self.global_motion_args["window_size"], getattr(ops, "warp_tiles", None),
                getattr(ops, "conv3_instance", None), getattr(ops, "gemm_tile_wn", None))

    def _pool_validity_key(self, ops, glob: bool, target) -> Tuple:
        return (self._prepared_sig, glob, self._precision, self._checked, getattr(ops, "attention_f16x3", None), self._rows_fit_planes, target)

    def _mode_key(self, ops, im0, im1) -> Tuple:
        return (tuple(im0.shape), tuple(im1.shape), str(im0.device)) + self._mode_fields(ops) + (self._workspace_key(im0),)

    def _sync_plan_sig(self):
        if self._plan_sig is not self._prepared_sig:
            self._drop_plans()
            self._plan_sig = self._prepared_sig

    def forward(self, im0: torch.Tensor, im1: torch.Tensor, reuse_first: bool = False):
        self._reuse_first = bool(reuse_first)
        st = self._plan_stats["forward"]
        if not im0.is_cuda or self._frame_cache_on or self._checked:
            st["eager"] += 1
            return self._forward_eager(im0, im1)
        if self.use_graphs:
            st["eager"] += 1
            return self._forward_graph(im0, im1)
        ops = self._ops_obj
        pl = self._plist
        if (not self.use_plans or not isinstance(ops, HipOps) or ops.profile is not None
                or pl is None or pl[0].device != im0.device or torch.cuda.is_current_stream_capturing()):
            st["eager"] += 1
            return self._forward_eager(im0, im1)
        self._prepare(ops)
        self._sync_plan_sig()
        key = self._mode_key(ops, im0, im1)
        ent = self._plans.get(key, 0)
        if ent is False:
            st["eager"] += 1
# ... 576 lines not shown
```

include/atmvfi.h:

```cpp
#ifndef ATMVFI_H
#define ATMVFI_H

#include <stdint.h>

#ifdef __cplusplus
extern "C" {
#endif

#define ATMVFI_OK        0
#define ATMVFI_EINVAL   -1
#define ATMVFI_EALIGN   -2
#define ATMVFI_ELAUNCH  -3

int         atmvfi_version(void);
const char* atmvfi_last_error(void);
const char* atmvfi_source_digest(void);
int atmvfi_range_word_set(uint32_t* word, void* stream);
int atmvfi_range_checked(void);

#define ATMVFI_GEMM_CONV   0
#define ATMVFI_GEMM_LINEAR 1
#define ATMVFI_GEMM_DECONV 2

typedef struct atmvfi_gemm_params {
    int32_t mode;
    const float* in;
    int32_t in_ld, N, H, W, Cin;
    int64_t in_gstride; int32_t in_rpg;
    const float* weight;
    int32_t Cout, kh, kw, stride, pad, dil;
    int32_t Ho, Wo;
    int64_t M;
    float* out;
    int32_t out_ld;
    int64_t out_gstride; int32_t out_rpg;
    const int32_t* out_row_map;
    const float* bias;
    const float* prelu;
    const float* in_prelu;
    const float* residual;
    int32_t res_ld;
    int32_t precision;
    const void* weight_hi;
    const void* weight_lo;
    const void* in_hi;
    const void* in_lo;
    void* out_hi;
    void* out_lo;
    int64_t out_plane_rows;
    int32_t out_plane_c0, out_plane_gc;
    int32_t tile_wn;
    const void* in_hi2;
    const void* in_lo2;
    int32_t in_ld2, in_split_chunks;
    float* workspace;
    int64_t workspace_floats;
} atmvfi_gemm_params;

#define ATMVFI_PREC_F32   0
#define ATMVFI_PREC_F16X3 1
#define ATMVFI_PREC_F16   2

int atmvfi_gemm(const atmvfi_gemm_params* p, void* stream);
int64_t atmvfi_gemm_workspace_floats(int64_t M, int ngemm, int ksteps);

int atmvfi_head1x1_planes(const void* in_hi, const void* in_lo, int64_t plane_rows, int64_t rows, int Cin, const float* weight,
                          const float* bias, int Cout, float* out, int out_ld, void* stream);

int atmvfi_split_planes(const float* in, int in_ld, int64_t M, int C, const float* prelu, void* hi, void* lo, int plane_rows, void* stream);
int atmvfi_split_planes_at(const float* in, int in_ld, int64_t M, int C, const float* prelu, void* hi, void* lo, int plane_rows, int c0,
                           int pad_to, void* stream);

int atmvfi_conv2d(const atmvfi_gemm_params* p, void* stream);
int atmvfi_linear(const atmvfi_gemm_params* p, void* stream);
int atmvfi_deconv2x2(const atmvfi_gemm_params* p, void* stream);

int64_t atmvfi_packed_weight_floats(int mode, int Cout, int Cin, int kh, int kw);
int atmvfi_pack_weight(int mode, const float* src, float* dst, int Cout, int Cin, int kh, int kw, void* stream);

int64_t atmvfi_split_weight_halves(int mode, int Cout, int Cin, int kh, int kw);
int atmvfi_pack_weight_split(int mode, const float* src, void* dst_hi, void* dst_lo, int Cout, int Cin, int kh, int kw,
                             void* stream);
int64_t atmvfi_conv3x3_weight_halves(int Cout, int Cin);
int atmvfi_pack_weight_conv3x3(const float* src, void* dst_hi, void* dst_lo, int Cout, int Cin, void* stream);
int atmvfi_conv3x3_f16x3(const float* in, int in_ld, int N, int H, int W, int Cin, const void* w_hi, const void* w_lo,
                         int Cout, float* out, int out_ld, const float* bias, const float* prelu, void* out_hi, void* out_lo,
                         int64_t plane_rows, const float* plane_prelu, int schedule, int wn, void* stream);
int atmvfi_conv3x3_planes(const void* in_hi, const void* in_lo, int64_t in_rows, int N, int H, int W, int Cin, const void* w_hi,
                          const void* w_lo, int Cout, float* out, int out_ld, const float* bias, const float* prelu, void* out_hi,
                          void* out_lo, int64_t plane_rows, int out_c0, const float* plane_prelu, int out_cmin, int wn, void* stream);
int atmvfi_conv3x3_planes2(const void* in_hi, const void* in_lo, int64_t in_rows, int N, int H, int W, int Cin, const void* w_hi,
                           const void* w_lo, int Cout, float* out, int out_ld, const float* bias, const float* prelu, void* out_hi,
                           void* out_lo, int64_t plane_rows, int out_c0, const float* plane_prelu, void* out_hi2, void* out_lo2,
                           int64_t plane_rows2, int out_c02, int out_cmin, int wn, void* stream);
int64_t atmvfi_conv3x3_planes_workspace_floats(int N, int H, int W, int Cin, int Cout);
int atmvfi_conv3x3_planes3(const void* in_hi, const void* in_lo, int64_t in_rows, int N, int H, int W, int Cin, const void* w_hi,
                           const void* w_lo, int Cout, float* out, int out_ld, const float* bias, const float* prelu, void* out_hi,
                           void* out_lo, int64_t plane_rows, int out_c0, const float* plane_prelu, void* out_hi2, void* out_lo2,
                           int64_t plane_rows2, int out_c02, int out_cmin, int wn, float* workspace, int64_t workspace_floats, void* stream);
int atmvfi_conv3x3_planes4(const void* in_hi, const void* in_lo, int64_t in_rows, int N, int H, int W, int Cin, const void* w_hi,
                           const void* w_lo, int Cout, float* out, int out_ld, const float* bias, const float* prelu, void* out_hi,
                           void* out_lo, int64_t plane_rows, int out_c0, const float* plane_prelu, void* out_hi2, void* out_lo2,
                           int64_t plane_rows2, int out_c02, int out_cmin, int wn, float* workspace, int64_t workspace_floats, int terms,
                           void* stream);
int atmvfi_layernorm(const float* in, int in_ld, int64_t in_gstride, int in_rpg,
                     const int32_t* src_row_map, float* out, int out_ld,
                     const float* gamma, const float* beta, int64_t rows, int C,
                     void* out_hi, void* out_lo, int plane_rows, void* stream);
// ... 206 lines not shown
```

Before: 51.97.

## Interleave deconv weight columns so the gemm_pp epilogue writes split planes directly

```diff
diff --git a/atm-vfi_amd/csrc/api.hip b/atm-vfi_amd/csrc/api.hip
--- a/atm-vfi_amd/csrc/api.hip
+++ b/atm-vfi_amd/csrc/api.hip
@@ -55,7 +55,7 @@
 #endif
 }
 
-extern "C" int atmvfi_version(void) { return (0 << 16) | (26 << 8) | 0; }
+extern "C" int atmvfi_version(void) { return (0 << 16) | (27 << 8) | 0; }
 extern "C" const char* atmvfi_last_error(void) { return atmvfi::g_err; }
 #ifndef ATMVFI_SOURCE_DIGEST
 #define ATMVFI_SOURCE_DIGEST "unknown (api.hip compiled outside the Makefile)"
diff --git a/atm-vfi_amd/csrc/conv3x3_f16x3.hip b/atm-vfi_amd/csrc/conv3x3_f16x3.hip
--- a/atm-vfi_amd/csrc/conv3x3_f16x3.hip
+++ b/atm-vfi_amd/csrc/conv3x3_f16x3.hip
@@ -1,6 +1,7 @@
 #include "common.h"
 
 #include "conv3_common.h"
+#include "gemm_common.h"
 
 #include <stdlib.h>
 
@@ -30,6 +31,25 @@
                 v = src[(((long long)row * Cin + c) * kh + ky) * kw + kx];
             }
         }
+        const _Float16 h = sat_half(v);
+        hi[idx] = h;
+        lo[idx] = sat_half((v - (float)h) * LO_SCALE);
+    }
+}
+
+__global__ void pack_split_deconv_il_kernel(const float* __restrict__ src, _Float16* __restrict__ hi, _Float16* __restrict__ lo, int Cout,
+                                            int Cin, int nc, int cin_pad) {
+    fp16_saturate_on();
+    const int rows = nc * 128;
+    const long long total = (long long)rows * cin_pad;
+    for (long long idx = (long long)blockIdx.x * blockDim.x + threadIdx.x; idx < total; idx += (long long)gridDim.x * blockDim.x) {
+        const int e = (int)(idx & 31);
+        const int row = (int)((idx >> 5) % rows);
+        const int c = (int)((idx >> 5) / rows) * 32 + e;
+        int q, co;
+        atmvfi::deconv_il_column(nc, row, q, co);
+        float v = 0.f;
+        if (c < Cin && co < Cout) v = src[(((long long)c * Cout + co) * 2 + (q >> 1)) * 2 + (q & 1)];
         const _Float16 h = sat_half(v);
         hi[idx] = h;
         lo[idx] = sat_half((v - (float)h) * LO_SCALE);
@@ -91,6 +111,19 @@
     return atmvfi::check_launch("pack_weight_split");
 }
 
+extern "C" int64_t atmvfi_split_weight_halves_deconv_il(int Cout, int Cin) {
+    return (int64_t)atmvfi::deconv_il_chunks(Cout) * 128 * atmvfi::round_up(Cin, 32);
+}
+
+extern "C" int atmvfi_pack_weight_split_deconv_il(const float* src, void* dst_hi, void* dst_lo, int Cout, int Cin, void* stream) {
+    ATMVFI_REQUIRE(src && dst_hi && dst_lo && Cout > 0 && Cin > 0, ATMVFI_EINVAL, "pack_weight_split_deconv_il: bad arguments");
+    const int64_t total = atmvfi_split_weight_halves_deconv_il(Cout, Cin);
+    const int blocks = (int)((total + 255) / 256 > 4096 ? 4096 : (total + 255) / 256);
+    hipLaunchKernelGGL(pack_split_deconv_il_kernel, dim3(blocks), dim3(256), 0, (hipStream_t)stream, src, (_Float16*)dst_hi,
+                       (_Float16*)dst_lo, Cout, Cin, atmvfi::deconv_il_chunks(Cout), atmvfi::round_up(Cin, 32));
+    return atmvfi::check_launch("pack_weight_split_deconv_il");
+}
+
 extern "C" int atmvfi_conv3x3_f16x3(const float* in, int in_ld, int N, int H, int W, int Cin, const void* w_hi,
                                      const void* w_lo, int Cout, float* out, int out_ld, const float* bias,
                                      const float* prelu, void* out_hi, void* out_lo, int64_t plane_rows,
diff --git a/atm-vfi_amd/csrc/gemm_common.h b/atm-vfi_amd/csrc/gemm_common.h
--- a/atm-vfi_amd/csrc/gemm_common.h
+++ b/atm-vfi_amd/csrc/gemm_common.h
@@ -59,7 +59,16 @@
     int fit32;
     int pfit32;
     int terms;
+    int direct, nc32;
 };
+
+__host__ __device__ inline int deconv_il_channel(int p) { return (p & 0x13) | ((p & 4) << 1) | ((p & 8) >> 1); }
+__host__ __device__ inline int deconv_il_chunks(int Cout) { return (Cout + 31) / 32; }
+__host__ __device__ inline void deconv_il_column(int nc, int n, int& q, int& co) {
+    const int unit = n >> 6, dy = unit / nc;
+    q = 2 * dy + ((n >> 5) & 1);
+    co = (unit - dy * nc) * 32 + deconv_il_channel(n & 31);
+}
 
 
 __device__ __forceinline__ bool gemm_out_row(const GemmDev& a, long long m, float*& orow, const float*& rrow, long long& prow, int& pc0) {
@@ -170,11 +179,15 @@
     }
 }
 
-template <int BN>
+template <int BN, bool IL = false>
 __device__ __forceinline__ void gemm_dma_consts(const GemmDev& a, int n0, float* cst, int wave, int lane) {
     dma_epilogue_consts<BN>(a.bias, a.prelu, n0, cst, wave, lane, [&](int col) {
         int co = col;
-        if (a.mode == ATMVFI_GEMM_DECONV) {
+        if (IL && a.direct) {
+            int q;
+            deconv_il_column(a.nc32, col, q, co);
+            if (q >= 4) co = a.Cout;
+        } else if (a.mode == ATMVFI_GEMM_DECONV) {
             const int q = col / a.coutp;
             co = q < 4 ? col - q * a.coutp : a.Cout;
         }
@@ -242,6 +255,7 @@
     return r;
 }
 
+bool gemm_split_picks_pp(const GemmDev& d, int ngemm);
 int launch_gemm_f16x3(const GemmDev& d, int ngemm, hipStream_t stream);
 bool try_launch_conv3x3_small(const GemmDev& d, int kh, int* rc, hipStream_t stream);
 int launch_gemm_split(const GemmDev& d, int ngemm, hipStream_t stream);
diff --git a/atm-vfi_amd/csrc/gemm_conv.hip b/atm-vfi_amd/csrc/gemm_conv.hip
--- a/atm-vfi_amd/csrc/gemm_conv.hip
+++ b/atm-vfi_amd/csrc/gemm_conv.hip
@@ -225,7 +225,7 @@
     return atmvfi::check_launch("pack_weight");
 }
 
-extern "C" int atmvfi_gemm(const atmvfi_gemm_params* p, void* stream) {
+static int gemm_run(const atmvfi_gemm_params* p, void* stream, int* direct_query) {
     ATMVFI_REQUIRE(p, ATMVFI_EINVAL, "gemm: null params");
     const bool planes = p->in_hi || p->in_lo;
     const bool sink = p->out_hi || p->out_lo;
@@ -262,6 +262,8 @@
     ATMVFI_REQUIRE(p->precision != ATMVFI_PREC_F16 || p->tile_wn != -1, ATMVFI_EINVAL,
                    "gemm: precision f16 has no instance of the reference schedule (tile_wn = -1): use 0 (auto), -2, -3 or -4");
     ATMVFI_REQUIRE(p->mode >= 0 && p->mode <= 2, ATMVFI_EINVAL, "gemm: bad mode %d", p->mode);
+    ATMVFI_REQUIRE(p->weight_order == ATMVFI_WEIGHTS_STANDARD || p->weight_order == ATMVFI_WEIGHTS_DECONV_IL, ATMVFI_EINVAL,
+                   "gemm: bad weight_order %d", p->weight_order);
     ATMVFI_REQUIRE(p->Cin > 0 && p->Cout > 0, ATMVFI_EINVAL, "gemm: bad channel counts");
     ATMVFI_REQUIRE(planes || (p->in_ld >= atmvfi::round_up(p->Cin, 4) && p->in_ld % 4 == 0), ATMVFI_EALIGN,
                    "gemm: in_ld %d must be a multiple of 4 and >= Cin rounded to 4 (Cin %d)", p->in_ld, p->Cin);
@@ -347,6 +349,8 @@
     d.mchunk = 0;
     d.stamp = nullptr;
     d.terms = p->precision == ATMVFI_PREC_F16 ? 1 : 3;
+    d.direct = 0;
+    d.nc32 = atmvfi::deconv_il_chunks(p->Cout);
     d.w_hi = (const _Float16*)p->weight_hi;
     d.w_lo = (const _Float16*)p->weight_lo;
     d.cin_pad32 = atmvfi::round_up(p->Cin, 32);
@@ -357,9 +361,29 @@
         ATMVFI_REQUIRE(p->weight_hi && p->weight_lo, ATMVFI_EINVAL, "gemm: precision f16x3 / f16 needs weight_hi/weight_lo");
         ATMVFI_REQUIRE(atmvfi::aligned16(p->weight_hi) && atmvfi::aligned16(p->weight_lo), ATMVFI_EALIGN,
                        "gemm: split weights must be 16-byte aligned");
-        if (planes) return atmvfi::launch_gemm_split(d, ngemm, (hipStream_t)stream);
+        if (planes) {
+            const bool direct_ok = p->mode == ATMVFI_GEMM_DECONV && !d.out && d.out_hi && !d.residual && p->W % 16 == 0 && d.out_c0 % 32 == 0 &&
+                                   d.out_plane_rows * 64 < (1ll << 32) && d.M < (1ll << 26) && atmvfi::gemm_split_picks_pp(d, ngemm);
+            if (direct_query) {
+                *direct_query = direct_ok ? 1 : 0;
+                return ATMVFI_OK;
+            }
+            if (p->weight_order == ATMVFI_WEIGHTS_DECONV_IL) {
+                ATMVFI_REQUIRE(direct_ok, ATMVFI_EINVAL,
+                               "gemm: weight_order DECONV_IL needs a launch that atmvfi_deconv_direct_ok accepts (DECONV, plane sink only at a "
+                               "multiple of 32 channels, W %% 16 == 0, the gemm_pp engine)");
+                d.direct = 1;
+                d.wrows = d.nc32 * 128;
+                return atmvfi::launch_gemm_pp(d, d.wrows, (hipStream_t)stream);
+            }
+            return atmvfi::launch_gemm_split(d, ngemm, (hipStream_t)stream);
+        }
+        if (direct_query) return ATMVFI_OK;
+        ATMVFI_REQUIRE(p->weight_order == ATMVFI_WEIGHTS_STANDARD, ATMVFI_EINVAL, "gemm: weight_order DECONV_IL needs split-plane input");
         return atmvfi::launch_gemm_f16x3(d, ngemm, (hipStream_t)stream);
     }
+    if (direct_query) return ATMVFI_OK;
+    ATMVFI_REQUIRE(p->weight_order == ATMVFI_WEIGHTS_STANDARD, ATMVFI_EINVAL, "gemm: weight_order DECONV_IL needs precision f16x3 (or f16)");
 
     {
         int rc = 0;
@@ -387,6 +411,20 @@
     return atmvfi::check_launch("gemm");
 }
 
+extern "C" int atmvfi_gemm(const atmvfi_gemm_params* p, void* stream) { return gemm_run(p, stream, nullptr); }
+
+extern "C" int atmvfi_deconv_direct_ok(const atmvfi_gemm_params* p) {
+    int ok = 0;
+    return gemm_run(p, nullptr, &ok) == ATMVFI_OK ? ok : 0;
+}
+
+extern "C" int atmvfi_deconv_il_column(int Cout, int n) {
+    if (Cout <= 0 || n < 0 || n >= atmvfi::deconv_il_chunks(Cout) * 128) return -1;
+    int q, co;
+    atmvfi::deconv_il_column(atmvfi::deconv_il_chunks(Cout), n, q, co);
+    return co < Cout ? q * atmvfi::round_up(Cout, 4) + co : -1;
+}
+
 extern "C" int atmvfi_conv2d(const atmvfi_gemm_params* p, void* stream) {
     ATMVFI_REQUIRE(p && p->mode == ATMVFI_GEMM_CONV, ATMVFI_EINVAL, "conv2d: params->mode must be ATMVFI_GEMM_CONV");
     return atmvfi_gemm(p, stream);
diff --git a/atm-vfi_amd/csrc/gemm_duo.hip b/atm-vfi_amd/csrc/gemm_duo.hip
--- a/atm-vfi_amd/csrc/gemm_duo.hip
+++ b/atm-vfi_amd/csrc/gemm_duo.hip
@@ -303,6 +303,7 @@
 
 int atmvfi::launch_gemm_duo(const GemmDev& d, int ngemm, hipStream_t s) {
     const bool conv = d.mode == ATMVFI_GEMM_CONV;
+    ATMVFI_REQUIRE(!d.direct, ATMVFI_EINVAL, "gemm_duo: chunk-interleaved DECONV rows are a gemm_pp form");
     if ((ngemm <= 64 && d.force_wn != -2) || d.force_wn == -4) {
         if (d.terms == 1) return conv ? launch_duo<true, 64, false>(d, ngemm, s) : launch_duo<false, 64, false>(d, ngemm, s);
         return conv ? launch_duo<true, 64, true>(d, ngemm, s) : launch_duo<false, 64, true>(d, ngemm, s);
diff --git a/atm-vfi_amd/csrc/gemm_plane.h b/atm-vfi_amd/csrc/gemm_plane.h
--- a/atm-vfi_amd/csrc/gemm_plane.h
+++ b/atm-vfi_amd/csrc/gemm_plane.h
@@ -324,6 +324,106 @@
     }
 }
 
+template <int MI>
+__device__ __forceinline__ void plane_deconv_direct(const GemmDev a, f32x4 (&acc)[MI][4], const float* cst, int BN, int m0, int n0, int M,
+                                                    int wm, int wn, int r, int g, int lane) {
+    typedef unsigned u32x4 __attribute__((ext_vector_type(4)));
+    typedef unsigned u32x2 __attribute__((ext_vector_type(2)));
+    const float* cw = cst + 64 * wn;
+    const int unit = (n0 >> 6) + wn;
+    const int dy = unit >= a.nc32 ? 1 : 0;
+    const int chunk = unit - dy * a.nc32;
+    const int cabs = (a.out_c0 >> 5) + chunk;
+    unsigned char* ph = reinterpret_cast<unsigned char*>(a.out_hi + (long long)cabs * a.out_plane_rows * 32);
+    unsigned char* pl = reinterpret_cast<unsigned char*>(a.out_lo + (long long)cabs * a.out_plane_rows * 32);
+    const int cleft = a.coutp - 32 * chunk;
+    const unsigned lane_off = (unsigned)(r * 128 + g * 16);
+    int w = a.W;
+    asm volatile("" : "+s"(w));
+    const int mb = m0 + 16 * MI * wm;
+    unsigned yy = (unsigned)mb / (unsigned)w;
+    unsigned x0 = (unsigned)mb - yy * (unsigned)w;
+    auto body = [&](auto act_tag, auto full_tag) {
+        constexpr int ACT = decltype(act_tag)::value;
+        constexpr bool FULL = decltype(full_tag)::value;
+        f32x4 bv[4], sv[4];
+#pragma unroll
+        for (int j = 0; j < 4; ++j) {
+            bv[j] = *reinterpret_cast<const f32x4*>(cw + 16 * j + 4 * g);
+            if constexpr (ACT != 0) sv[j] = *reinterpret_cast<const f32x4*>(cw + BN + 16 * j + 4 * g);
+            else sv[j] = (f32x4){1.f, 1.f, 1.f, 1.f};
+        }
+        auto act = [&](f32x4 v, const f32x4 s) -> f32x4 {
+            if constexpr (ACT == 1) {
+                v.x = v.x > 0.f ? v.x : s.x * v.x;
+                v.y = v.y > 0.f ? v.y : s.y * v.y;
+                v.z = v.z > 0.f ? v.z : s.z * v.z;
+                v.w = v.w > 0.f ? v.w : s.w * v.w;
+            } else if constexpr (ACT == 2) {
+                const f32x4 t = s * v;
+                f32x4 o;
+                asm("v_max_f32 %0, %1, %2" : "=v"(o.x) : "v"(v.x), "v"(t.x));
+                asm("v_max_f32 %0, %1, %2" : "=v"(o.y) : "v"(v.y), "v"(t.y));
+                asm("v_max_f32 %0, %1, %2" : "=v"(o.z) : "v"(v.z), "v"(t.z));
+                asm("v_max_f32 %0, %1, %2" : "=v"(o.w) : "v"(v.w), "v"(t.w));
+                v = o;
+            }
+            return v;
+        };
+        auto bits = [](f16x2 v) { return __builtin_bit_cast(unsigned, v); };
+#pragma unroll
+        for (int i = 0; i < MI; ++i) {
+            if (mb + 16 * i < M) {
+                const unsigned row0 = (2u * yy + (unsigned)dy) * (unsigned)a.Wo + 2u * x0;
+#pragma unroll
+                for (int dx = 0; dx < 2; ++dx) {
+                    const f32x4 u0 = act(acc[i][2 * dx] + bv[2 * dx], sv[2 * dx]);
+                    const f32x4 u1 = act(acc[i][2 * dx + 1] + bv[2 * dx + 1], sv[2 * dx + 1]);
+                    f16x2 h00, l00, h01, l01, h10, l10, h11, l11;
+                    split_pair((f32x2){u0.x, u0.y}, h00, l00);
+                    split_pair((f32x2){u0.z, u0.w}, h01, l01);
+                    split_pair((f32x2){u1.x, u1.y}, h10, l10);
+                    split_pair((f32x2){u1.z, u1.w}, h11, l11);
+                    const auto sh0 = __builtin_amdgcn_permlane32_swap(bits(h00), bits(h10), false, false);
+                    const auto sh1 = __builtin_amdgcn_permlane32_swap(bits(h01), bits(h11), false, false);
+                    const auto sl0 = __builtin_amdgcn_permlane32_swap(bits(l00), bits(l10), false, false);
+                    const auto sl1 = __builtin_amdgcn_permlane32_swap(bits(l01), bits(l11), false, false);
+                    const u32x4 h4 = {sh0[0], sh1[0], sh0[1], sh1[1]}, l4 = {sl0[0], sl1[0], sl0[1], sl1[1]};
+                    const unsigned long long sbase = (unsigned long long)(row0 + (unsigned)dx) << 6;
+                    unsigned char* qh = ph + sbase + lane_off;
+                    unsigned char* ql = pl + sbase + lane_off;
+                    if constexpr (FULL) {
+                        *reinterpret_cast<u32x4*>(qh) = h4;
+                        *reinterpret_cast<u32x4*>(ql) = l4;
+                    } else if (cleft - 8 * g >= 8) {
+                        *reinterpret_cast<u32x4*>(qh) = h4;
+                        *reinterpret_cast<u32x4*>(ql) = l4;
+                    } else if (cleft - 8 * g > 0) {
+                        *reinterpret_cast<u32x2*>(qh) = (u32x2){h4[0], h4[1]};
+                        *reinterpret_cast<u32x2*>(ql) = (u32x2){l4[0], l4[1]};
+                    }
+                }
+            }
+            x0 += 16u;
+            if (x0 >= (unsigned)w) { x0 -= (unsigned)w; ++yy; }
+        }
+    };
+    typedef std::integral_constant<int, 0> ActNone;
+    typedef std::integral_constant<int, 1> ActSelect;
+    typedef std::integral_constant<int, 2> ActMax;
+    const float slope = cw[BN + lane];
+    const bool pmax = __builtin_amdgcn_ballot_w64(!(slope > 0.f && slope <= 1.f)) == 0ull;
+    if (cleft >= 32) {
+        if (!a.prelu) body(ActNone{}, std::true_type{});
+        else if (pmax) body(ActMax{}, std::true_type{});
+        else body(ActSelect{}, std::true_type{});
+    } else {
+        if (!a.prelu) body(ActNone{}, std::false_type{});
+        else if (pmax) body(ActMax{}, std::false_type{});
+        else body(ActSelect{}, std::false_type{});
+    }
+}
+
 inline int plane_gemm_prepare(const char* engine, GemmDev& d, int ngemm, int BM, int BN) {
     ATMVFI_REQUIRE((long long)d.in_ld * 64 < (1ll << 32) && (long long)d.wrows * 64 < (1ll << 32) &&
                        (!d.a_hi2 || (long long)d.in_ld2 * 64 < (1ll << 32)) && d.M < (1ll << 26), ATMVFI_EINVAL,
diff --git a/atm-vfi_amd/csrc/gemm_pp.hip b/atm-vfi_amd/csrc/gemm_pp.hip
--- a/atm-vfi_amd/csrc/gemm_pp.hip
+++ b/atm-vfi_amd/csrc/gemm_pp.hip
@@ -101,14 +101,14 @@
         wr_off = wr_off == 2 * STAGE ? 0 : wr_off + STAGE;
     };
     auto dma_tile_consts = [&](int tm0, int tn0, float* dst) {
-        atmvfi::gemm_dma_consts<BN>(a, tn0, dst, wave, lane);
+        atmvfi::gemm_dma_consts<BN, !CONVM>(a, tn0, dst, wave, lane);
         if (a.out_row_map && a.mode == ATMVFI_GEMM_LINEAR) {
             int m = tm0 + (wave & 3) * 64 + lane;
             if (m >= M) m = M - 1;
             __builtin_amdgcn_global_load_lds((const __attribute__((address_space(1))) void*)(a.out_row_map + m),
                                              (__attribute__((address_space(3))) void*)(dst + atmvfi::gemm_const_floats(BN) + (wave & 3) * 64), 4, 0, 0);
         } else {
-            atmvfi::gemm_dma_consts<BN>(a, tn0, dst, wave, lane);
+            atmvfi::gemm_dma_consts<BN, !CONVM>(a, tn0, dst, wave, lane);
         }
     };
 
@@ -273,38 +273,46 @@
                 if constexpr (X3) acc[i][j] = acc[i][j] + cor[i][j] * LO_UNSCALE;
                 asm volatile("" : "+v"(acc[i][j]));
             }
-        {
-            const unsigned xb = (unsigned)(rd_off == 0 ? 2 * STAGE : rd_off - STAGE);
-            const unsigned tb = lds_offset(smem) + xb + (unsigned)(wave * 1024);
-            const unsigned wbase = tb + (unsigned)((r >> 2) * 8192 + (r & 3) * 256 + ((g ^ (r & 3)) << 4));
-            const unsigned rq6 = (unsigned)((r >> 2) << 6);
-            const unsigned rbase = tb + (unsigned)(g * 256);
-            const unsigned rg4 = (unsigned)((r ^ g) << 4);
-            unsigned wad[4], rad[4];
-#pragma unroll
-            for (int k = 0; k < 4; ++k) {
-                wad[k] = wbase + (rq6 ^ (unsigned)(k << 6));
-                rad[k] = rbase + (rg4 ^ (unsigned)(k << 6));
-            }
-            static_for<0, 4>([&](auto ic) {
-                constexpr int i = decltype(ic)::value;
-                static_for<0, 4>([&](auto jc) {
-                    constexpr int j = decltype(jc)::value;
-                    lds_write16f(wad[j], acc[i][j]);
+        bool direct = false;
+        if constexpr (!CONVM) direct = a.direct != 0;
+        if (direct) {
+            PP_SUB(0);
+            atmvfi::plane_deconv_direct<4>(a, acc, cst, BN, m0, n0, M, wm, wn, r, g, lane);
+            PP_SUB(1);
+        } else {
+            {
+                const unsigned xb = (unsigned)(rd_off == 0 ? 2 * STAGE : rd_off - STAGE);
+                const unsigned tb = lds_offset(smem) + xb + (unsigned)(wave * 1024);
+                const unsigned wbase = tb + (unsigned)((r >> 2) * 8192 + (r & 3) * 256 + ((g ^ (r & 3)) << 4));
+                const unsigned rq6 = (unsigned)((r >> 2) << 6);
+                const unsigned rbase = tb + (unsigned)(g * 256);
+                const unsigned rg4 = (unsigned)((r ^ g) << 4);
+                unsigned wad[4], rad[4];
+#pragma unroll
+                for (int k = 0; k < 4; ++k) {
+                    wad[k] = wbase + (rq6 ^ (unsigned)(k << 6));
+                    rad[k] = rbase + (rg4 ^ (unsigned)(k << 6));
+                }
+                static_for<0, 4>([&](auto ic) {
+                    constexpr int i = decltype(ic)::value;
+                    static_for<0, 4>([&](auto jc) {
+                        constexpr int j = decltype(jc)::value;
+                        lds_write16f(wad[j], acc[i][j]);
+                    });
+                    static_for<0, 4>([&](auto qc) {
+                        constexpr int q = decltype(qc)::value;
+                        lds_read16f<q * 8192>(acc[i][q], rad[q]);
+                    });
                 });
-                static_for<0, 4>([&](auto qc) {
-                    constexpr int q = decltype(qc)::value;
-                    lds_read16f<q * 8192>(acc[i][q], rad[q]);
-                });
-            });
-            asm volatile("s_waitcnt lgkmcnt(0)" ::: "memory");
-#pragma unroll
-            for (int i = 0; i < 4; ++i)
-#pragma unroll
-                for (int q = 0; q < 4; ++q) asm volatile("" : "+v"(acc[i][q]));
-        }
-        PP_SUB(0);
-        atmvfi::plane_gemm_epilogue<CONVM, 4, BM, BN>(a, acc, cst, m0, n0, M, wm, wn, r, g, [&] { PP_SUB(1); });
+                asm volatile("s_waitcnt lgkmcnt(0)" ::: "memory");
+#pragma unroll
+                for (int i = 0; i < 4; ++i)
+#pragma unroll
+                    for (int q = 0; q < 4; ++q) asm volatile("" : "+v"(acc[i][q]));
+            }
+            PP_SUB(0);
+            atmvfi::plane_gemm_epilogue<CONVM, 4, BM, BN>(a, acc, cst, m0, n0, M, wm, wn, r, g, [&] { PP_SUB(1); });
+        }
         PP_SUB(2);
         PP_STAMP(3);
 #ifdef ATMVFI_STAMP
@@ -349,6 +357,10 @@
     GemmDev dd = d;
     const int rc = atmvfi::plane_gemm_prepare("gemm_pp", dd, ngemm, BM, BN);
     if (rc != ATMVFI_OK) return rc;
+    ATMVFI_REQUIRE(!dd.direct || (!CONVM && dd.mode == ATMVFI_GEMM_DECONV && !dd.out && dd.out_hi && dd.out_lo && !dd.residual && dd.pfit32 &&
+                                  dd.W % 16 == 0 && dd.out_c0 % 32 == 0 && ngemm == dd.nc32 * 128 && dd.wrows == ngemm &&
+                                  dd.nc32 == atmvfi::deconv_il_chunks(dd.Cout)),
+                   ATMVFI_EINVAL, "gemm_pp: the direct DECONV sink needs W %% 16 == 0, a plane-only sink at a multiple of 32 channels and NC * 128 columns");
 #ifdef ATMVFI_STAMP
     dd.stamp = g_pp_stamp;
 #endif
diff --git a/atm-vfi_amd/csrc/gemm_split.hip b/atm-vfi_amd/csrc/gemm_split.hip
--- a/atm-vfi_amd/csrc/gemm_split.hip
+++ b/atm-vfi_amd/csrc/gemm_split.hip
@@ -396,13 +396,34 @@
     return S > 1 ? (int64_t)S * M * atmvfi::round_up(ngemm, 64) : 0;
 }
 
+static int gemm_splitk_ranges(const atmvfi::GemmDev& d, int ngemm) {
+    if (!d.part) return 1;
+    const int S = gemm_splitk_plan(d.M, ngemm, d.nchunks32);
+    return (S > 1 && (long long)S * d.M * atmvfi::round_up(ngemm, 64) <= d.part_stride) ? S : 1;
+}
+static bool gemm_underfilled(const atmvfi::GemmDev& d, int ngemm) {
+    return atmvfi::ceil_div64(d.M, 128) * ((ngemm + 63) / 64) <= 2 * (long long)atmvfi::cu_count();
+}
+static bool gemm_duo_rounds_win(const atmvfi::GemmDev& d, int ngemm) {
+    const long long cus = atmvfi::cu_count(), ntile = (ngemm + 127) / 128;
+    const long long pp_rounds = atmvfi::ceil_div64(atmvfi::ceil_div64(d.M, 256) * ntile, cus);
+    const long long duo_per_cu = atmvfi::ceil_div64(atmvfi::ceil_div64(d.M, 128) * ntile, cus);
+    const double duo_rounds = (0.5 * (double)duo_per_cu + ((duo_per_cu & 1) ? 0.1 : 0.0)) * 1.08 * (d.nchunks32 >= 64 ? 1.15 : 1.0);
+    return duo_rounds < (double)pp_rounds;
+}
+bool atmvfi::gemm_split_picks_pp(const GemmDev& d, int ngemm) {
+    if (d.force_wn == -3) return true;
+    if (d.force_wn != 0) return false;
+    return gemm_splitk_ranges(d, ngemm) == 1 && ngemm > 64 && !gemm_underfilled(d, ngemm) && !gemm_duo_rounds_win(d, ngemm);
+}
+
 int atmvfi::launch_gemm_split(const GemmDev& d, int ngemm, hipStream_t s) {
     if (d.force_wn == -2 || d.force_wn == -4) return launch_gemm_duo(d, ngemm, s);
     if (d.force_wn == -3) return launch_gemm_pp(d, ngemm, s);
-    if (d.force_wn == 0 && d.part) {
-        const int S = gemm_splitk_plan(d.M, ngemm, d.nchunks32);
-        const int ld = round_up(ngemm, 64);
-        if (S > 1 && (long long)S * d.M * ld <= d.part_stride) {
+    if (d.force_wn == 0) {
+        const int S = gemm_splitk_ranges(d, ngemm);
+        if (S > 1) {
+            const int ld = round_up(ngemm, 64);
             GemmDev ds = d;
             ds.ksplit = S;
             ds.part_ld = ld;
@@ -410,19 +431,13 @@
             ds.force_wn = -4;
             return launch_gemm_duo(ds, ngemm, s);
         }
-    }
-    if (d.force_wn == 0) {
         if (ngemm <= 64) return launch_gemm_duo(d, ngemm, s);
-        if (ceil_div64(d.M, 128) * ((ngemm + 63) / 64) <= 2 * (long long)cu_count()) {
+        if (gemm_underfilled(d, ngemm)) {
             GemmDev d64 = d;
             d64.force_wn = -4;
             return launch_gemm_duo(d64, ngemm, s);
         }
-        const long long cus = cu_count(), ntile = (ngemm + 127) / 128;
-        const long long pp_rounds = ceil_div64(ceil_div64(d.M, 256) * ntile, cus);
-        const long long duo_per_cu = ceil_div64(ceil_div64(d.M, 128) * ntile, cus);
-        const double duo_rounds = (0.5 * (double)duo_per_cu + ((duo_per_cu & 1) ? 0.1 : 0.0)) * 1.08 * (d.nchunks32 >= 64 ? 1.15 : 1.0);
-        return duo_rounds < (double)pp_rounds ? launch_gemm_duo(d, ngemm, s) : launch_gemm_pp(d, ngemm, s);
+        return gemm_duo_rounds_win(d, ngemm) ? launch_gemm_duo(d, ngemm, s) : launch_gemm_pp(d, ngemm, s);
     }
     if (d.force_wn != -1) return launch_gemm_pp(d, ngemm, s);
 #ifdef ATMVFI_HAVE_REFSCHED
diff --git a/atm-vfi_amd/csrc/plan_dispatch.inc b/atm-vfi_amd/csrc/plan_dispatch.inc
--- a/atm-vfi_amd/csrc/plan_dispatch.inc
+++ b/atm-vfi_amd/csrc/plan_dispatch.inc
@@ -1,4 +1,4 @@
-#define ATMVFI_PLAN_NFN 75
+#define ATMVFI_PLAN_NFN 76
 static const char* const kPlanFnNames[ATMVFI_PLAN_NFN] = {
     "atmvfi_conv2d",
     "atmvfi_conv3x3_f16x3",
@@ -42,6 +42,7 @@
     "atmvfi_pack_weight",
     "atmvfi_pack_weight_conv3x3",
     "atmvfi_pack_weight_split",
+    "atmvfi_pack_weight_split_deconv_il",
     "atmvfi_pool_blocks",
     "atmvfi_range_word_set",
     "atmvfi_refine_tail",
@@ -76,7 +77,7 @@
     "atmvfi_yuv_surface_encode",
     "atmvfi_yuv_unpack",
 };
-static const int kPlanFnArgs[ATMVFI_PLAN_NFN] = {1, 19, 21, 25, 27, 28, 15, 16, 1, 13, 13, 10, 8, 10, 9, 14, 10, 8, 8, 7, 15, 12, 9, 5, 5, 11, 9, 15, 1, 10, 8, 9, 7, 14, 1, 12, 17, 3, 6, 7, 5, 8, 8, 1, 10, 13, 15, 10, 13, 13, 7, 8, 10, 18, 21, 1, 11, 19, 23, 23, 13, 13, 9, 8, 14, 18, 14, 9, 24, 5, 25, 17, 24, 16, 6};
+static const int kPlanFnArgs[ATMVFI_PLAN_NFN] = {1, 19, 21, 25, 27, 28, 15, 16, 1, 13, 13, 10, 8, 10, 9, 14, 10, 8, 8, 7, 15, 12, 9, 5, 5, 11, 9, 15, 1, 10, 8, 9, 7, 14, 1, 12, 17, 3, 6, 7, 5, 8, 5, 8, 1, 10, 13, 15, 10, 13, 13, 7, 8, 10, 18, 21, 1, 11, 19, 23, 23, 13, 13, 9, 8, 14, 18, 14, 9, 24, 5, 25, 17, 24, 16, 6};
 static int plan_call(const atmvfi_plan_op* op, void* stream) {
     const atmvfi_plan_arg* a = op->a;
     switch (op->fn) {
@@ -122,39 +123,40 @@
     case 39: return atmvfi_pack_weight((int)a[0].i, (const float*)(uintptr_t)a[1].u, (float*)(uintptr_t)a[2].u, (int)a[3].i, (int)a[4].i, (int)a[5].i, (int)a[6].i, stream);
     case 40: return atmvfi_pack_weight_conv3x3((const float*)(uintptr_t)a[0].u, (void*)(uintptr_t)a[1].u, (void*)(uintptr_t)a[2].u, (int)a[3].i, (int)a[4].i, stream);
     case 41: return atmvfi_pack_weight_split((int)a[0].i, (const float*)(uintptr_t)a[1].u, (void*)(uintptr_t)a[2].u, (void*)(uintptr_t)a[3].u, (int)a[4].i, (int)a[5].i, (int)a[6].i, (int)a[7].i, stream);
-    case 42: return atmvfi_pool_blocks((void*)(uintptr_t)a[0].u, (int64_t)a[1].i, (int)a[2].i, (const int32_t*)(uintptr_t)a[3].u, (int)a[4].i, (int64_t)a[5].i, (void*)(uintptr_t)a[6].u, (int)a[7].i, stream);
-    case 43: return atmvfi_range_word_set((uint32_t*)(uintptr_t)a[0].u, stream);
-    case 44: return atmvfi_refine_tail((const float*)(uintptr_t)a[0].u, (int64_t)a[1].i, (const float*)(uintptr_t)a[2].u, (const float*)(uintptr_t)a[3].u, (const float*)(uintptr_t)a[4].u, (float*)(uintptr_t)a[5].u, (float*)(uintptr_t)a[6].u, (int)a[7].i, (int)a[8].i, (int)a[9].i, stream);
-    case 45: return atmvfi_resize_bilinear_ac((const float*)(uintptr_t)a[0].u, (int64_t)a[1].i, (int64_t)a[2].i, (int64_t)a[3].i, (int64_t)a[4].i, (float*)(uintptr_t)a[5].u, (int)a[6].i, (int)a[7].i, (int)a[8].i, (int)a[9].i, (int)a[10].i, (int)a[11].i, (float)a[12].f, stream);
-    case 46: return atmvfi_rgb16_decode((const void*)(uintptr_t)a[0].u, (int)a[1].i, (int)a[2].i, (int)a[3].i, (int)a[4].i, (int)a[5].i, (int)a[6].i, (int)a[7].i, (int)a[8].i, (float*)(uintptr_t)a[9].u, (int)a[10].i, (int)a[11].i, (int)a[12].i, (int)a[13].i, (void*)(uintptr_t)a[14].u, stream);
-    case 47: return atmvfi_rgb16_encode((const float*)(uintptr_t)a[0].u, (int)a[1].i, (int)a[2].i, (int)a[3].i, (int)a[4].i, (void*)(uintptr_t)a[5].u, (int)a[6].i, (int)a[7].i, (int)a[8].i, (int)a[9].i, stream);
-    case 48: return atmvfi_rgb_to_yuv420((const void*)(uintptr_t)a[0].u, (int)a[1].i, (const float*)(uintptr_t)a[2].u, (int)a[3].i, (int)a[4].i, (int)a[5].i, (int)a[6].i, (int)a[7].i, (int)a[8].i, (int)a[9].i, (int)a[10].i, (int)a[11].i, (void*)(uintptr_t)a[12].u, stream);
-    case 49: return atmvfi_shutter_accumulate((int32_t*)(uintptr_t)a[0].u, (int)a[1].i, (int)a[2].i, (const float*)(uintptr_t)a[3].u, (int)a[4].i, (int)a[5].i, (int)a[6].i, (int)a[7].i, (const uint8_t*)(uintptr_t)a[8].u, (int)a[9].i, (int)a[10].i, (int)a[11].i, (int)a[12].i, stream);
-    case 50: return atmvfi_shutter_resolve((const int32_t*)(uintptr_t)a[0].u, (int)a[1].i, (int)a[2].i, (int)a[3].i, (int)a[4].i, (uint8_t*)(uintptr_t)a[5].u, (int)a[6].i, stream);
-    case 51: return atmvfi_split_planes((const float*)(uintptr_t)a[0].u, (int)a[1].i, (int64_t)a[2].i, (int)a[3].i, (const float*)(uintptr_t)a[4].u, (void*)(uintptr_t)a[5].u, (void*)(uintptr_t)a[6].u, (int)a[7].i, stream);
-    case 52: return atmvfi_split_planes_at((const float*)(uintptr_t)a[0].u, (int)a[1].i, (int64_t)a[2].i, (int)a[3].i, (const float*)(uintptr_t)a[4].u, (void*)(uintptr_t)a[5].u, (void*)(uintptr_t)a[6].u, (int)a[7].i, (int)a[8].i, (int)a[9].i, stream);
-    case 53: return atmvfi_ssim_psnr((const void*)(uintptr_t)a[0].u, (int64_t)a[1].i, (int64_t)a[2].i, (int64_t)a[3].i, (int64_t)a[4].i, (const float*)(uintptr_t)a[5].u, (int64_t)a[6].i, (int64_t)a[7].i, (int64_t)a[8].i, (int64_t)a[9].i, (int)a[10].i, (int)a[11].i, (int)a[12].i, (float)a[13].f, (int)a[14].i, (double*)(uintptr_t)a[15].u, (float*)(uintptr_t)a[16].u, (int64_t)a[17].i, stream);
-    case 54: return atmvfi_stem_fused((const float*)(uintptr_t)a[0].u, (int)a[1].i, (int)a[2].i, (int)a[3].i, (int)a[4].i, (int)a[5].i, (const void*)(uintptr_t)a[6].u, (const void*)(uintptr_t)a[7].u, (const float*)(uintptr_t)a[8].u, (const float*)(uintptr_t)a[9].u, (const void*)(uintptr_t)a[10].u, (const void*)(uintptr_t)a[11].u, (const float*)(uintptr_t)a[12].u, (const float*)(uintptr_t)a[13].u, (const void*)(uintptr_t)a[14].u, (const void*)(uintptr_t)a[15].u, (const float*)(uintptr_t)a[16].u, (const float*)(uintptr_t)a[17].u, (void*)(uintptr_t)a[18].u, (void*)(uintptr_t)a[19].u, (int64_t)a[20].i, stream);
-    case 55: return atmvfi_synth_up2((const atmvfi_synth_up2_params*)(uintptr_t)a[0].u, stream);
-    case 56: return atmvfi_tta_merge((const float*)(uintptr_t)a[0].u, (const float*)(uintptr_t)a[1].u, (float*)(uintptr_t)a[2].u, (void*)(uintptr_t)a[3].u, (int)a[4].i, (int)a[5].i, (int)a[6].i, (int)a[7].i, (int)a[8].i, (int)a[9].i, (int)a[10].i, stream);
-    case 57: return atmvfi_warp_blend((const float*)(uintptr_t)a[0].u, (const float*)(uintptr_t)a[1].u, (const float*)(uintptr_t)a[2].u, (int)a[3].i, (int64_t)a[4].i, (float*)(uintptr_t)a[5].u, (float*)(uintptr_t)a[6].u, (float*)(uintptr_t)a[7].u, (float*)(uintptr_t)a[8].u, (float*)(uintptr_t)a[9].u, (float*)(uintptr_t)a[10].u, (float*)(uintptr_t)a[11].u, (const float*)(uintptr_t)a[12].u, (const float*)(uintptr_t)a[13].u, (float*)(uintptr_t)a[14].u, (int)a[15].i, (int)a[16].i, (int)a[17].i, (int)a[18].i, stream);
-    case 58: return atmvfi_warp_blend_planes((const float*)(uintptr_t)a[0].u, (const float*)(uintptr_t)a[1].u, (const float*)(uintptr_t)a[2].u, (int)a[3].i, (int64_t)a[4].i, (float*)(uintptr_t)a[5].u, (float*)(uintptr_t)a[6].u, (float*)(uintptr_t)a[7].u, (float*)(uintptr_t)a[8].u, (float*)(uintptr_t)a[9].u, (float*)(uintptr_t)a[10].u, (float*)(uintptr_t)a[11].u, (const float*)(uintptr_t)a[12].u, (const float*)(uintptr_t)a[13].u, (float*)(uintptr_t)a[14].u, (int)a[15].i, (void*)(uintptr_t)a[16].u, (void*)(uintptr_t)a[17].u, (int64_t)a[18].i, (int)a[19].i, (int)a[20].i, (int)a[21].i, (int)a[22].i, stream);
-    case 59: return atmvfi_warp_blend_tiled((const float*)(uintptr_t)a[0].u, (const float*)(uintptr_t)a[1].u, (const float*)(uintptr_t)a[2].u, (int)a[3].i, (int64_t)a[4].i, (float*)(uintptr_t)a[5].u, (float*)(uintptr_t)a[6].u, (float*)(uintptr_t)a[7].u, (float*)(uintptr_t)a[8].u, (float*)(uintptr_t)a[9].u, (float*)(uintptr_t)a[10].u, (float*)(uintptr_t)a[11].u, (const float*)(uintptr_t)a[12].u, (const float*)(uintptr_t)a[13].u, (float*)(uintptr_t)a[14].u, (int)a[15].i, (void*)(uintptr_t)a[16].u, (void*)(uintptr_t)a[17].u, (int64_t)a[18].i, (int)a[19].i, (int)a[20].i, (int)a[21].i, (int)a[22].i, stream);
-    case 60: return atmvfi_window_attention((const float*)(uintptr_t)a[0].u, (float*)(uintptr_t)a[1].u, (float*)(uintptr_t)a[2].u, (const int32_t*)(uintptr_t)a[3].u, (int)a[4].i, (int)a[5].i, (int)a[6].i, (int)a[7].i, (int)a[8].i, (int)a[9].i, (void*)(uintptr_t)a[10].u, (void*)(uintptr_t)a[11].u, (int)a[12].i, stream);
-    case 61: return atmvfi_window_attention_f16x3((const float*)(uintptr_t)a[0].u, (float*)(uintptr_t)a[1].u, (float*)(uintptr_t)a[2].u, (const int32_t*)(uintptr_t)a[3].u, (int)a[4].i, (int)a[5].i, (int)a[6].i, (int)a[7].i, (int)a[8].i, (int)a[9].i, (void*)(uintptr_t)a[10].u, (void*)(uintptr_t)a[11].u, (int)a[12].i, stream);
-    case 62: return atmvfi_window_attn_cross_motion((const float*)(uintptr_t)a[0].u, (float*)(uintptr_t)a[1].u, (float*)(uintptr_t)a[2].u, (const int32_t*)(uintptr_t)a[3].u, (int)a[4].i, (int)a[5].i, (int)a[6].i, (int)a[7].i, (int)a[8].i, stream);
-    case 63: return atmvfi_window_attn_self((const float*)(uintptr_t)a[0].u, (float*)(uintptr_t)a[1].u, (const int32_t*)(uintptr_t)a[2].u, (int)a[3].i, (int)a[4].i, (int)a[5].i, (int)a[6].i, (int)a[7].i, stream);
-    case 64: return atmvfi_yuv420_to_rgb((const void*)(uintptr_t)a[0].u, (int)a[1].i, (int)a[2].i, (int)a[3].i, (int)a[4].i, (int)a[5].i, (int)a[6].i, (void*)(uintptr_t)a[7].u, (int)a[8].i, (float*)(uintptr_t)a[9].u, (int)a[10].i, (int)a[11].i, (int)a[12].i, (int)a[13].i, stream);
-    case 65: return atmvfi_yuv420_window((const void*)(uintptr_t)a[0].u, (int)a[1].i, (int)a[2].i, (int)a[3].i, (int)a[4].i, (int)a[5].i, (int)a[6].i, (int)a[7].i, (int)a[8].i, (int)a[9].i, (int)a[10].i, (int)a[11].i, (float*)(uintptr_t)a[12].u, (int)a[13].i, (int)a[14].i, (int)a[15].i, (int)a[16].i, (void*)(uintptr_t)a[17].u, stream);
-    case 66: return atmvfi_yuv420p10_to_f32((const void*)(uintptr_t)a[0].u, (int)a[1].i, (int)a[2].i, (int)a[3].i, (int)a[4].i, (int)a[5].i, (int)a[6].i, (int)a[7].i, (int)a[8].i, (float*)(uintptr_t)a[9].u, (int)a[10].i, (int)a[11].i, (int)a[12].i, (int)a[13].i, stream);
-    case 67: return atmvfi_yuv_borders((const void*)(uintptr_t)a[0].u, (int)a[1].i, (int)a[2].i, (int)a[3].i, (int)a[4].i, (int64_t)a[5].i, (int32_t*)(uintptr_t)a[6].u, (int32_t*)(uintptr_t)a[7].u, (int64_t)a[8].i, stream);
-    case 68: return atmvfi_yuv_compose((void*)(uintptr_t)a[0].u, (const void*)(uintptr_t)a[1].u, (int)a[2].i, (int)a[3].i, (int)a[4].i, (int)a[5].i, (int)a[6].i, (int)a[7].i, (int)a[8].i, (int)a[9].i, (int)a[10].i, (int64_t)a[11].i, (int64_t)a[12].i, (int64_t)a[13].i, (int)a[14].i, (int)a[15].i, (int)a[16].i, (int)a[17].i, (const float*)(uintptr_t)a[18].u, (int)a[19].i, (int)a[20].i, (int)a[21].i, (int)a[22].i, (const void*)(uintptr_t)a[23].u, stream);
-    case 69: return atmvfi_yuv_pack((const void*)(uintptr_t)a[0].u, (int)a[1].i, (int)a[2].i, (int)a[3].i, (void*)(uintptr_t)a[4].u, stream);
-    case 70: return atmvfi_yuv_sub_decode((const void*)(uintptr_t)a[0].u, (int)a[1].i, (int)a[2].i, (int)a[3].i, (int)a[4].i, (int)a[5].i, (int)a[6].i, (int)a[7].i, (int)a[8].i, (int)a[9].i, (int64_t)a[10].i, (int64_t)a[11].i, (int64_t)a[12].i, (int)a[13].i, (int)a[14].i, (int)a[15].i, (int)a[16].i, (int)a[17].i, (void*)(uintptr_t)a[18].u, (int)a[19].i, (float*)(uintptr_t)a[20].u, (int)a[21].i, (int)a[22].i, (int)a[23].i, (int)a[24].i, stream);
-    case 71: return atmvfi_yuv_sub_encode((const void*)(uintptr_t)a[0].u, (int)a[1].i, (const float*)(uintptr_t)a[2].u, (int)a[3].i, (int)a[4].i, (int)a[5].i, (int)a[6].i, (int)a[7].i, (int)a[8].i, (int)a[9].i, (int)a[10].i, (int)a[11].i, (int)a[12].i, (int)a[13].i, (int)a[14].i, (int)a[15].i, (void*)(uintptr_t)a[16].u, stream);
-    case 72: return atmvfi_yuv_surface_decode((const void*)(uintptr_t)a[0].u, (int)a[1].i, (int)a[2].i, (int)a[3].i, (int)a[4].i, (int)a[5].i, (int)a[6].i, (int)a[7].i, (int)a[8].i, (int64_t)a[9].i, (int64_t)a[10].i, (int64_t)a[11].i, (int)a[12].i, (int)a[13].i, (int)a[14].i, (int)a[15].i, (int)a[16].i, (void*)(uintptr_t)a[17].u, (int)a[18].i, (float*)(uintptr_t)a[19].u, (int)a[20].i, (int)a[21].i, (int)a[22].i, (int)a[23].i, stream);
-    case 73: return atmvfi_yuv_surface_encode((const void*)(uintptr_t)a[0].u, (int)a[1].i, (const float*)(uintptr_t)a[2].u, (int)a[3].i, (int)a[4].i, (int)a[5].i, (int)a[6].i, (int)a[7].i, (int)a[8].i, (int)a[9].i, (int)a[10].i, (int)a[11].i, (int)a[12].i, (int)a[13].i, (int)a[14].i, (void*)(uintptr_t)a[15].u, stream);
-    case 74: return atmvfi_yuv_unpack((const void*)(uintptr_t)a[0].u, (int)a[1].i, (int)a[2].i, (int)a[3].i, (int64_t)a[4].i, (void*)(uintptr_t)a[5].u, stream);
+    case 42: return atmvfi_pack_weight_split_deconv_il((const float*)(uintptr_t)a[0].u, (void*)(uintptr_t)a[1].u, (void*)(uintptr_t)a[2].u, (int)a[3].i, (int)a[4].i, stream);
+    case 43: return atmvfi_pool_blocks((void*)(uintptr_t)a[0].u, (int64_t)a[1].i, (int)a[2].i, (const int32_t*)(uintptr_t)a[3].u, (int)a[4].i, (int64_t)a[5].i, (void*)(uintptr_t)a[6].u, (int)a[7].i, stream);
+    case 44: return atmvfi_range_word_set((uint32_t*)(uintptr_t)a[0].u, stream);
+    case 45: return atmvfi_refine_tail((const float*)(uintptr_t)a[0].u, (int64_t)a[1].i, (const float*)(uintptr_t)a[2].u, (const float*)(uintptr_t)a[3].u, (const float*)(uintptr_t)a[4].u, (float*)(uintptr_t)a[5].u, (float*)(uintptr_t)a[6].u, (int)a[7].i, (int)a[8].i, (int)a[9].i, stream);
+    case 46: return atmvfi_resize_bilinear_ac((const float*)(uintptr_t)a[0].u, (int64_t)a[1].i, (int64_t)a[2].i, (int64_t)a[3].i, (int64_t)a[4].i, (float*)(uintptr_t)a[5].u, (int)a[6].i, (int)a[7].i, (int)a[8].i, (int)a[9].i, (int)a[10].i, (int)a[11].i, (float)a[12].f, stream);
+    case 47: return atmvfi_rgb16_decode((const void*)(uintptr_t)a[0].u, (int)a[1].i, (int)a[2].i, (int)a[3].i, (int)a[4].i, (int)a[5].i, (int)a[6].i, (int)a[7].i, (int)a[8].i, (float*)(uintptr_t)a[9].u, (int)a[10].i, (int)a[11].i, (int)a[12].i, (int)a[13].i, (void*)(uintptr_t)a[14].u, stream);
+    case 48: return atmvfi_rgb16_encode((const float*)(uintptr_t)a[0].u, (int)a[1].i, (int)a[2].i, (int)a[3].i, (int)a[4].i, (void*)(uintptr_t)a[5].u, (int)a[6].i, (int)a[7].i, (int)a[8].i, (int)a[9].i, stream);
+    case 49: return atmvfi_rgb_to_yuv420((const void*)(uintptr_t)a[0].u, (int)a[1].i, (const float*)(uintptr_t)a[2].u, (int)a[3].i, (int)a[4].i, (int)a[5].i, (int)a[6].i, (int)a[7].i, (int)a[8].i, (int)a[9].i, (int)a[10].i, (int)a[11].i, (void*)(uintptr_t)a[12].u, stream);
+    case 50: return atmvfi_shutter_accumulate((int32_t*)(uintptr_t)a[0].u, (int)a[1].i, (int)a[2].i, (const float*)(uintptr_t)a[3].u, (int)a[4].i, (int)a[5].i, (int)a[6].i, (int)a[7].i, (const uint8_t*)(uintptr_t)a[8].u, (int)a[9].i, (int)a[10].i, (int)a[11].i, (int)a[12].i, stream);
+    case 51: return atmvfi_shutter_resolve((const int32_t*)(uintptr_t)a[0].u, (int)a[1].i, (int)a[2].i, (int)a[3].i, (int)a[4].i, (uint8_t*)(uintptr_t)a[5].u, (int)a[6].i, stream);
+    case 52: return atmvfi_split_planes((const float*)(uintptr_t)a[0].u, (int)a[1].i, (int64_t)a[2].i, (int)a[3].i, (const float*)(uintptr_t)a[4].u, (void*)(uintptr_t)a[5].u, (void*)(uintptr_t)a[6].u, (int)a[7].i, stream);
+    case 53: return atmvfi_split_planes_at((const float*)(uintptr_t)a[0].u, (int)a[1].i, (int64_t)a[2].i, (int)a[3].i, (const float*)(uintptr_t)a[4].u, (void*)(uintptr_t)a[5].u, (void*)(uintptr_t)a[6].u, (int)a[7].i, (int)a[8].i, (int)a[9].i, stream);
+    case 54: return atmvfi_ssim_psnr((const void*)(uintptr_t)a[0].u, (int64_t)a[1].i, (int64_t)a[2].i, (int64_t)a[3].i, (int64_t)a[4].i, (const float*)(uintptr_t)a[5].u, (int64_t)a[6].i, (int64_t)a[7].i, (int64_t)a[8].i, (int64_t)a[9].i, (int)a[10].i, (int)a[11].i, (int)a[12].i, (float)a[13].f, (int)a[14].i, (double*)(uintptr_t)a[15].u, (float*)(uintptr_t)a[16].u, (int64_t)a[17].i, stream);
+    case 55: return atmvfi_stem_fused((const float*)(uintptr_t)a[0].u, (int)a[1].i, (int)a[2].i, (int)a[3].i, (int)a[4].i, (int)a[5].i, (const void*)(uintptr_t)a[6].u, (const void*)(uintptr_t)a[7].u, (const float*)(uintptr_t)a[8].u, (const float*)(uintptr_t)a[9].u, (const void*)(uintptr_t)a[10].u, (const void*)(uintptr_t)a[11].u, (const float*)(uintptr_t)a[12].u, (const float*)(uintptr_t)a[13].u, (const void*)(uintptr_t)a[14].u, (const void*)(uintptr_t)a[15].u, (const float*)(uintptr_t)a[16].u, (const float*)(uintptr_t)a[17].u, (void*)(uintptr_t)a[18].u, (void*)(uintptr_t)a[19].u, (int64_t)a[20].i, stream);
+    case 56: return atmvfi_synth_up2((const atmvfi_synth_up2_params*)(uintptr_t)a[0].u, stream);
+    case 57: return atmvfi_tta_merge((const float*)(uintptr_t)a[0].u, (const float*)(uintptr_t)a[1].u, (float*)(uintptr_t)a[2].u, (void*)(uintptr_t)a[3].u, (int)a[4].i, (int)a[5].i, (int)a[6].i, (int)a[7].i, (int)a[8].i, (int)a[9].i, (int)a[10].i, stream);
+    case 58: return atmvfi_warp_blend((const float*)(uintptr_t)a[0].u, (const float*)(uintptr_t)a[1].u, (const float*)(uintptr_t)a[2].u, (int)a[3].i, (int64_t)a[4].i, (float*)(uintptr_t)a[5].u, (float*)(uintptr_t)a[6].u, (float*)(uintptr_t)a[7].u, (float*)(uintptr_t)a[8].u, (float*)(uintptr_t)a[9].u, (float*)(uintptr_t)a[10].u, (float*)(uintptr_t)a[11].u, (const float*)(uintptr_t)a[12].u, (const float*)(uintptr_t)a[13].u, (float*)(uintptr_t)a[14].u, (int)a[15].i, (int)a[16].i, (int)a[17].i, (int)a[18].i, stream);
+    case 59: return atmvfi_warp_blend_planes((const float*)(uintptr_t)a[0].u, (const float*)(uintptr_t)a[1].u, (const float*)(uintptr_t)a[2].u, (int)a[3].i, (int64_t)a[4].i, (float*)(uintptr_t)a[5].u, (float*)(uintptr_t)a[6].u, (float*)(uintptr_t)a[7].u, (float*)(uintptr_t)a[8].u, (float*)(uintptr_t)a[9].u, (float*)(uintptr_t)a[10].u, (float*)(uintptr_t)a[11].u, (const float*)(uintptr_t)a[12].u, (const float*)(uintptr_t)a[13].u, (float*)(uintptr_t)a[14].u, (int)a[15].i, (void*)(uintptr_t)a[16].u, (void*)(uintptr_t)a[17].u, (int64_t)a[18].i, (int)a[19].i, (int)a[20].i, (int)a[21].i, (int)a[22].i, stream);
+    case 60: return atmvfi_warp_blend_tiled((const float*)(uintptr_t)a[0].u, (const float*)(uintptr_t)a[1].u, (const float*)(uintptr_t)a[2].u, (int)a[3].i, (int64_t)a[4].i, (float*)(uintptr_t)a[5].u, (float*)(uintptr_t)a[6].u, (float*)(uintptr_t)a[7].u, (float*)(uintptr_t)a[8].u, (float*)(uintptr_t)a[9].u, (float*)(uintptr_t)a[10].u, (float*)(uintptr_t)a[11].u, (const float*)(uintptr_t)a[12].u, (const float*)(uintptr_t)a[13].u, (float*)(uintptr_t)a[14].u, (int)a[15].i, (void*)(uintptr_t)a[16].u, (void*)(uintptr_t)a[17].u, (int64_t)a[18].i, (int)a[19].i, (int)a[20].i, (int)a[21].i, (int)a[22].i, stream);
+    case 61: return atmvfi_window_attention((const float*)(uintptr_t)a[0].u, (float*)(uintptr_t)a[1].u, (float*)(uintptr_t)a[2].u, (const int32_t*)(uintptr_t)a[3].u, (int)a[4].i, (int)a[5].i, (int)a[6].i, (int)a[7].i, (int)a[8].i, (int)a[9].i, (void*)(uintptr_t)a[10].u, (void*)(uintptr_t)a[11].u, (int)a[12].i, stream);
+    case 62: return atmvfi_window_attention_f16x3((const float*)(uintptr_t)a[0].u, (float*)(uintptr_t)a[1].u, (float*)(uintptr_t)a[2].u, (const int32_t*)(uintptr_t)a[3].u, (int)a[4].i, (int)a[5].i, (int)a[6].i, (int)a[7].i, (int)a[8].i, (int)a[9].i, (void*)(uintptr_t)a[10].u, (void*)(uintptr_t)a[11].u, (int)a[12].i, stream);
+    case 63: return atmvfi_window_attn_cross_motion((const float*)(uintptr_t)a[0].u, (float*)(uintptr_t)a[1].u, (float*)(uintptr_t)a[2].u, (const int32_t*)(uintptr_t)a[3].u, (int)a[4].i, (int)a[5].i, (int)a[6].i, (int)a[7].i, (int)a[8].i, stream);
+    case 64: return atmvfi_window_attn_self((const float*)(uintptr_t)a[0].u, (float*)(uintptr_t)a[1].u, (const int32_t*)(uintptr_t)a[2].u, (int)a[3].i, (int)a[4].i, (int)a[5].i, (int)a[6].i, (int)a[7].i, stream);
+    case 65: return atmvfi_yuv420_to_rgb((const void*)(uintptr_t)a[0].u, (int)a[1].i, (int)a[2].i, (int)a[3].i, (int)a[4].i, (int)a[5].i, (int)a[6].i, (void*)(uintptr_t)a[7].u, (int)a[8].i, (float*)(uintptr_t)a[9].u, (int)a[10].i, (int)a[11].i, (int)a[12].i, (int)a[13].i, stream);
+    case 66: return atmvfi_yuv420_window((const void*)(uintptr_t)a[0].u, (int)a[1].i, (int)a[2].i, (int)a[3].i, (int)a[4].i, (int)a[5].i, (int)a[6].i, (int)a[7].i, (int)a[8].i, (int)a[9].i, (int)a[10].i, (int)a[11].i, (float*)(uintptr_t)a[12].u, (int)a[13].i, (int)a[14].i, (int)a[15].i, (int)a[16].i, (void*)(uintptr_t)a[17].u, stream);
+    case 67: return atmvfi_yuv420p10_to_f32((const void*)(uintptr_t)a[0].u, (int)a[1].i, (int)a[2].i, (int)a[3].i, (int)a[4].i, (int)a[5].i, (int)a[6].i, (int)a[7].i, (int)a[8].i, (float*)(uintptr_t)a[9].u, (int)a[10].i, (int)a[11].i, (int)a[12].i, (int)a[13].i, stream);
+    case 68: return atmvfi_yuv_borders((const void*)(uintptr_t)a[0].u, (int)a[1].i, (int)a[2].i, (int)a[3].i, (int)a[4].i, (int64_t)a[5].i, (int32_t*)(uintptr_t)a[6].u, (int32_t*)(uintptr_t)a[7].u, (int64_t)a[8].i, stream);
+    case 69: return atmvfi_yuv_compose((void*)(uintptr_t)a[0].u, (const void*)(uintptr_t)a[1].u, (int)a[2].i, (int)a[3].i, (int)a[4].i, (int)a[5].i, (int)a[6].i, (int)a[7].i, (int)a[8].i, (int)a[9].i, (int)a[10].i, (int64_t)a[11].i, (int64_t)a[12].i, (int64_t)a[13].i, (int)a[14].i, (int)a[15].i, (int)a[16].i, (int)a[17].i, (const float*)(uintptr_t)a[18].u, (int)a[19].i, (int)a[20].i, (int)a[21].i, (int)a[22].i, (const void*)(uintptr_t)a[23].u, stream);
+    case 70: return atmvfi_yuv_pack((const void*)(uintptr_t)a[0].u, (int)a[1].i, (int)a[2].i, (int)a[3].i, (void*)(uintptr_t)a[4].u, stream);
+    case 71: return atmvfi_yuv_sub_decode((const void*)(uintptr_t)a[0].u, (int)a[1].i, (int)a[2].i, (int)a[3].i, (int)a[4].i, (int)a[5].i, (int)a[6].i, (int)a[7].i, (int)a[8].i, (int)a[9].i, (int64_t)a[10].i, (int64_t)a[11].i, (int64_t)a[12].i, (int)a[13].i, (int)a[14].i, (int)a[15].i, (int)a[16].i, (int)a[17].i, (void*)(uintptr_t)a[18].u, (int)a[19].i, (float*)(uintptr_t)a[20].u, (int)a[21].i, (int)a[22].i, (int)a[23].i, (int)a[24].i, stream);
+    case 72: return atmvfi_yuv_sub_encode((const void*)(uintptr_t)a[0].u, (int)a[1].i, (const float*)(uintptr_t)a[2].u, (int)a[3].i, (int)a[4].i, (int)a[5].i, (int)a[6].i, (int)a[7].i, (int)a[8].i, (int)a[9].i, (int)a[10].i, (int)a[11].i, (int)a[12].i, (int)a[13].i, (int)a[14].i, (int)a[15].i, (void*)(uintptr_t)a[16].u, stream);
+    case 73: return atmvfi_yuv_surface_decode((const void*)(uintptr_t)a[0].u, (int)a[1].i, (int)a[2].i, (int)a[3].i, (int)a[4].i, (int)a[5].i, (int)a[6].i, (int)a[7].i, (int)a[8].i, (int64_t)a[9].i, (int64_t)a[10].i, (int64_t)a[11].i, (int)a[12].i, (int)a[13].i, (int)a[14].i, (int)a[15].i, (int)a[16].i, (void*)(uintptr_t)a[17].u, (int)a[18].i, (float*)(uintptr_t)a[19].u, (int)a[20].i, (int)a[21].i, (int)a[22].i, (int)a[23].i, stream);
+    case 74: return atmvfi_yuv_surface_encode((const void*)(uintptr_t)a[0].u, (int)a[1].i, (const float*)(uintptr_t)a[2].u, (int)a[3].i, (int)a[4].i, (int)a[5].i, (int)a[6].i, (int)a[7].i, (int)a[8].i, (int)a[9].i, (int)a[10].i, (int)a[11].i, (int)a[12].i, (int)a[13].i, (int)a[14].i, (void*)(uintptr_t)a[15].u, stream);
+    case 75: return atmvfi_yuv_unpack((const void*)(uintptr_t)a[0].u, (int)a[1].i, (int)a[2].i, (int)a[3].i, (int64_t)a[4].i, (void*)(uintptr_t)a[5].u, stream);
     default: break;
     }
     atmvfi::set_error("plan_run: unknown function id %d", op->fn);
diff --git a/atm-vfi_amd/hip_ops.py b/atm-vfi_amd/hip_ops.py
--- a/atm-vfi_amd/hip_ops.py
+++ b/atm-vfi_amd/hip_ops.py
@@ -47,6 +47,7 @@
         ("out_plane_gc", ctypes.c_int32), ("tile_wn", ctypes.c_int32),
         ("in_hi2", c_f), ("in_lo2", c_f), ("in_ld2", ctypes.c_int32), ("in_split_chunks", ctypes.c_int32),
         ("workspace", c_f), ("workspace_floats", ctypes.c_int64),
+        ("weight_order", ctypes.c_int32),
     ]
 
 
@@ -83,6 +84,10 @@
     "atmvfi_pack_weight": (c_i, [c_i, c_f, c_f, c_i, c_i, c_i, c_i, c_f]),
     "atmvfi_split_weight_halves": (c_l, [c_i, c_i, c_i, c_i, c_i]),
     "atmvfi_pack_weight_split": (c_i, [c_i, c_f, c_f, c_f, c_i, c_i, c_i, c_i, c_f]),
+    "atmvfi_split_weight_halves_deconv_il": (c_l, [c_i, c_i]),
+    "atmvfi_pack_weight_split_deconv_il": (c_i, [c_f, c_f, c_f, c_i, c_i, c_f]),
+    "atmvfi_deconv_il_column": (c_i, [c_i, c_i]),
+    "atmvfi_deconv_direct_ok": (c_i, [ctypes.POINTER(GemmParams)]),
     "atmvfi_conv3x3_weight_halves": (c_l, [c_i, c_i]),
     "atmvfi_pack_weight_conv3x3": (c_i, [c_f, c_f, c_f, c_i, c_i, c_f]),
     "atmvfi_conv3x3_f16x3": (c_i, [c_f, c_i, c_i, c_i, c_i, c_i, c_f, c_f, c_i, c_f, c_i, c_f, c_f, c_f, c_f, c_l, c_f, c_i, c_i, c_f]),
@@ -205,6 +210,8 @@
     lo: Optional[torch.Tensor] = None
     hi3: Optional[torch.Tensor] = None
     lo3: Optional[torch.Tensor] = None
+    hi_il: Optional[torch.Tensor] = None
+    lo_il: Optional[torch.Tensor] = None
 
 
 @dataclass
@@ -570,6 +577,7 @@
         self.attention_f16x3 = True
         self.conv3_instance = None
         self.gemm_tile_wn = 0
+        self.deconv_direct_launches = 0
         self.warp_tiles = True
         self.recording: Optional[LaunchPlan] = None
         self.gemm_workspace = None
@@ -641,6 +649,12 @@
             pw.lo = torch.empty(nh, dtype=torch.float16, device=self.device)
             self._check(self.lib.atmvfi_pack_weight_split(mode, _ptr(w), _ptr(pw.hi), _ptr(pw.lo), cout, cin, kh, kw, self._stream()),
                         "pack_weight_split")
+            if mode == GEMM_DECONV:
+                ni = self.lib.atmvfi_split_weight_halves_deconv_il(cout, cin)
+                pw.hi_il = torch.empty(ni, dtype=torch.float16, device=self.device)
+                pw.lo_il = torch.empty(ni, dtype=torch.float16, device=self.device)
+                self._check(self.lib.atmvfi_pack_weight_split_deconv_il(_ptr(w), _ptr(pw.hi_il), _ptr(pw.lo_il), cout, cin, self._stream()),
+                            "pack_weight_split_deconv_il")
             if mode == GEMM_CONV and kh == 3 and kw == 3:
                 n3 = self.lib.atmvfi_conv3x3_weight_halves(cout, cin)
                 pw.hi3 = torch.empty(n3, dtype=torch.float16, device=self.device)
@@ -962,9 +976,14 @@
         ws = self._gemm_splitk(p, n * h * wd, 4 * ((cout + 3) // 4 * 4), (cin + 31) // 32) if use_planes else None
         p._srcs = (x, out, bias, prelu, in_prelu, ws)
         self._plane_prec(p)
+        direct = bool(use_planes and self.deconv_direct and w.hi_il is not None and self.lib.atmvfi_deconv_direct_ok(ctypes.byref(p)))
+        if direct:
+            p.weight_hi, p.weight_lo, p.weight_order = w.hi_il.data_ptr(), w.lo_il.data_ptr(), 1
+        self.deconv_direct_launches += direct
         self._run("deconv2x2_split" if use_planes else "deconv2x2_f16x3" if p.precision else "deconv2x2", meta, self.lib.atmvfi_deconv2x2,
                   ctypes.byref(p), self._stream())
 
+    deconv_direct = True
     split_planes_ok = True
     pyramid_packs = True
     motion_head_sink = True
diff --git a/atm-vfi_amd/network.py b/atm-vfi_amd/network.py
--- a/atm-vfi_amd/network.py
+++ b/atm-vfi_amd/network.py
@@ -745,7 +745,7 @@
     def _mode_fields(self, ops) -> Tuple:
         return (self.global_motion, self.ensemble_global_motion, self._precision, self._checked, getattr(ops, "attention_f16x3", None),
                 self.local_motion_args["window_size"], self.global_motion_args["window_size"], getattr(ops, "warp_tiles", None),
-                getattr(ops, "conv3_instance", None), getattr(ops, "gemm_tile_wn", None))
+                getattr(ops, "conv3_instance", None), getattr(ops, "gemm_tile_wn", None), getattr(ops, "deconv_direct", None))
 
     def _pool_validity_key(self, ops, glob: bool, target) -> Tuple:
         return (self._prepared_sig, glob, self._precision, self._checked, getattr(ops, "attention_f16x3", None), self._rows_fit_planes, target)
diff --git a/include/atmvfi.h b/include/atmvfi.h
--- a/include/atmvfi.h
+++ b/include/atmvfi.h
@@ -55,7 +55,11 @@
     int32_t in_ld2, in_split_chunks;
     float* workspace;
     int64_t workspace_floats;
+    int32_t weight_order;
 } atmvfi_gemm_params;
+
+#define ATMVFI_WEIGHTS_STANDARD  0
+#define ATMVFI_WEIGHTS_DECONV_IL 1
 
 #define ATMVFI_PREC_F32   0
 #define ATMVFI_PREC_F16X3 1
@@ -74,6 +78,11 @@
 int atmvfi_conv2d(const atmvfi_gemm_params* p, void* stream);
 int atmvfi_linear(const atmvfi_gemm_params* p, void* stream);
 int atmvfi_deconv2x2(const atmvfi_gemm_params* p, void* stream);
+
+int64_t atmvfi_split_weight_halves_deconv_il(int Cout, int Cin);
+int atmvfi_pack_weight_split_deconv_il(const float* src, void* dst_hi, void* dst_lo, int Cout, int Cin, void* stream);
+int atmvfi_deconv_il_column(int Cout, int n);
+int atmvfi_deconv_direct_ok(const atmvfi_gemm_params* p);
 
 int64_t atmvfi_packed_weight_floats(int mode, int Cout, int Cin, int kh, int kw);
 int atmvfi_pack_weight(int mode, const float* src, float* dst, int Cout, int Cin, int kh, int kw, void* stream);
```

Result: no change. 51.97, median of 4 (+0.0%).
